# Insomnia34/charon

Hardware: AMD Instinct MI355X
Metric: verified BLS partial sigs/sec (node) + threshold aggregates/sec, 1/2/4/8 GPU (higher is better)
Workload: dtype u32

## Files before the change

charon_amd/csrc/hipbls.hip:

```cpp
#include <hip/hip_runtime.h>
#include <hsa/hsa.h>
#include <hsa/hsa_ext_amd.h>

#include <algorithm>
#include <array>
#include <atomic>
#include <chrono>
#include <condition_variable>
#include <cstdio>
#include <cstdlib>
#include <cstring>
#include <deque>
#include <map>
#include <memory>
#include <mutex>
#include <string>
#include <thread>
#include <unordered_map>
#include <vector>

#include <sys/random.h>

#include "fav_split.h"
#include "hcache_assign.h"
#include "kernels.h"
#include "ranges.h"

extern "C" {
__global__ void k_rlc_items(uint64_t i0, uint64_t i1, const uint8_t* pks, const uint8_t* sigs, const uint32_t* msg_idx,
                            uint64_t n, uint64_t n_msgs, bls::rlc_seed seed, uint32_t* rpk, uint32_t* rsig,
                            int32_t* status, const uint32_t* key_idx, uint64_t T, const int32_t* tcode,
                            const uint32_t* tab, bls::keycache kc);
__global__ void k_rlc_hash(const uint8_t* msgs, const uint64_t* offs, uint64_t n_hash, const uint32_t* mlist, uint32_t* H,
                           uint64_t hstride, const uint32_t* hslot);
__global__ void k_rlcb_items(uint64_t n, const uint8_t* pks, const uint8_t* sigs, const uint32_t* msg_idx,
                             uint64_t n_msgs, bls::rlc_seed seed, uint32_t* rpk, uint32_t* pts, uint32_t* sc,
                             int32_t* status, const uint32_t* key_idx, uint64_t T, const int32_t* tcode,
                             const uint32_t* tab, const uint32_t* g1pos, uint32_t* gpts, uint32_t* gsc,
                             bls::keycache kc);
}

extern "C" {
__global__ void k_sign_ct_hash(const uint8_t* msgs, const uint64_t* offs, uint64_t n, uint32_t* H);
__global__ void k_sign_ct_mul(const uint8_t* sks, const uint32_t* H, uint64_t n, uint8_t* out, int32_t* status);
__global__ void k_sk_to_pk_ct(const uint8_t* sks, uint64_t n, uint8_t* out, int32_t* status);
}

extern "C" {
__global__ void k_g1_comb_build(uint32_t* T);
__global__ void k_deal_ct(const uint8_t* secrets, const uint8_t* tails, uint32_t n, uint32_t total, uint32_t threshold,
                          const uint32_t* T, uint8_t* out_shares, int32_t* status, uint8_t* out_pubs,
                          int32_t* pub_status, uint8_t* sink);
__global__ void k_recover_plan(const uint64_t* offs, uint32_t n_groups, uint32_t* m_max);
__global__ void k_recover_ct(const uint8_t* shares, const int64_t* ids, const uint64_t* offs, uint32_t n_groups,
                             uint32_t n_parts, const uint32_t* m_max, const uint32_t* T, uint8_t* out_secrets,
                             int32_t* status, uint8_t* out_pubkeys, int32_t* pk_status, uint8_t* sink);
}

namespace bls_fp2p {
__global__ void k_verify_prep8(const uint8_t* pks, const uint8_t* msgs, const uint64_t* offs, const uint8_t* sigs,
                               uint64_t n, uint32_t* ws, int32_t* status, uint32_t replicas, uint32_t* race,
                               uint32_t epoch);
__global__ void k_verify_pair_lq8(const uint32_t* ws, uint64_t n, int32_t* status, uint32_t replicas, uint32_t* race,
                                  uint32_t epoch);
__global__ void k_rlcb_sfactor8(const uint32_t* W, uint32_t* Fs);
__global__ void k_rlcb_final8(const uint32_t* Ftot, const uint32_t* Fs, int32_t* flag);
__global__ void k_g1m_miller8(uint64_t nl_max, const uint32_t* meta, const uint32_t* lmsg, const uint32_t* Wv,
                              const uint32_t* H, uint64_t hstride, const uint32_t* hslot, uint32_t* F, uint64_t col0,
                              uint64_t fstride);
__global__ void k_fav_prep8(const uint8_t* pks, uint64_t nkeys, const uint8_t* sigs, const uint8_t* msgs,
                            const uint64_t* moffs, uint64_t G, uint32_t* pts, int32_t* kcode, uint32_t* ws);
__global__ void k_tv_prep8(const uint8_t* pks, const uint8_t* msgs, const uint64_t* moffs, uint64_t G,
                           const int64_t* ids, const uint64_t* goffs, uint32_t* ws, int32_t* vstatus,
                           const uint8_t* sigs, uint64_t n_parts, uint32_t* pts, int32_t* pstat, uint32_t with_keys);
__global__ void k_tagg_sum8(const uint32_t* pts, const int32_t* pstat, const int64_t* ids, const uint64_t* goffs,
                            uint64_t n_parts, uint8_t* out, int32_t* status);
__global__ void k_tv_prep8_keys(const uint32_t* key_idx, uint64_t T, const int32_t* tcode, const uint32_t* tab,
                                const uint8_t* msgs, const uint64_t* moffs, const uint32_t* mlist, uint64_t n_hash,
                                uint64_t n_msgs, uint32_t* Hc, uint64_t G, const int64_t* ids, const uint64_t* goffs,
                                uint32_t* ws, int32_t* vstatus, const uint8_t* sigs, uint64_t n_parts, uint32_t* pts,
                                int32_t* pstat);
__global__ void k_verify_prep8_keys(const uint8_t* msgs, const uint64_t* moffs, const uint32_t* mlist, uint64_t n_hash,
                                    const uint32_t* hslot, uint32_t* H, uint64_t hstride, const uint8_t* sigs,
                                    uint64_t n, uint32_t* ws);
__global__ void k_hcache_fill8(const uint8_t* msgs, const uint64_t* moffs, const uint32_t* mlist, uint64_t n_hash,
                               const uint32_t* hslot, uint32_t* H, uint64_t hstride);
}
namespace bls_hex {
__global__ void k_verify_pair_lq16(const uint32_t* ws, uint64_t n, int32_t* status, uint32_t replicas, uint32_t* race,
                                   uint32_t epoch);
__global__ void k_tv_pair_lq16(const uint32_t* pts, const int32_t* pstat, const int64_t* ids, const uint64_t* goffs,
                               uint64_t G, uint64_t n_parts, const uint32_t* ws, int32_t* astatus, int32_t* vstatus,
                               uint8_t* out);
}
namespace bls_hexw {
__global__ void k_fav_pair_lq16(const uint32_t* pts, const int32_t* kcode, uint64_t nkeys, const uint64_t* goff,
                                const uint32_t* ws, uint64_t G, int32_t* status);
__global__ void k_fav_pair_lq16_keys(const uint32_t* key_idx, uint64_t T, const int32_t* tcode, const uint32_t* tab,
                                     const uint64_t* poff, const uint32_t* parts, const int32_t* pflags,
                                     uint64_t n_slices, const uint64_t* goff, const uint32_t* hcol,
                                     const uint32_t* Hcache, uint64_t cstride, const uint32_t* Hc, uint64_t hstride,
                                     const uint32_t* ws, uint64_t G, int32_t* status);
}
namespace bls_fp2p {
constexpr uint32_t kSfactorLds = 36 * 1024;
}

namespace {

thread_local std::string g_last_error;

constexpr int kStreamsPerDevice = 4;

struct DevBuf {
  void* p = nullptr;
  size_t cap = 0;
  hipError_t ensure(size_t n) {
    if (n <= cap) return hipSuccess;
    if (p) (void)hipFree(p);
    p = nullptr;
    cap = 0;
    const size_t want = ((n < 4096 ? 4096 : n + n / 4) + 255) & ~(size_t)255;
    hipError_t e = hipMalloc(&p, want);
    if (e == hipSuccess) cap = want;
    return e;
  }
};

struct TimingSlot {
  std::vector<std::pair<hipEvent_t, hipEvent_t>> pending;
  double total_ms = 0;
  uint64_t launches = 0;
};

struct HCache : HCacheState {
  DevBuf table;
};

struct KeyCache {
  std::mutex mu;
  uint64_t slots = 0;
  uint32_t* entries = nullptr;
  uint32_t* claim = nullptr;
  unsigned long long* ctr = nullptr;
  bls::keycache dev() const {
    bls::keycache k{};
    if (slots) {
      k.entries = entries;
      k.claim = claim;
      k.ctr = ctr;
      k.mask = (uint32_t)(slots - 1);
    }
    return k;
  }
};
constexpr uint64_t kKeyCacheDefaultSlots = 65536;
constexpr uint64_t kKeyCacheMaxSlots = 1ull << 24;

struct RootCache {
  std::mutex mu;
  uint64_t slots = 0;
  uint32_t* entries = nullptr;
  uint32_t* claim = nullptr;
  unsigned long long* ctr = nullptr;
  unsigned long long* h_ins = nullptr;
  uint64_t gen_base = 0;
  uint64_t rollovers = 0;
  bool partition = true;
  bls::rootcache dev() const {
    bls::rootcache r{};
    if (slots) {
      r.entries = entries;
      r.claim = claim;
      r.ctr = ctr;
      r.mask = (uint32_t)(slots - 1);
    }
    return r;
  }
};
constexpr uint64_t kRootCacheDefaultSlots = 262144;
constexpr uint64_t kRootCacheMaxSlots = 1ull << 22;

struct VBatch {
  std::vector<uint8_t> pk, sig, msg;
  std::vector<uint64_t> off{0};
  std::vector<int32_t> status;
  int rc = HIPBLS_OK;
  bool done = false;
  uint64_t n() const { return off.size() - 1; }
};

struct QSlot {
  hipStream_t stream = nullptr;
  hipEvent_t done_ev = nullptr;
  DevBuf d_pk, d_sig, d_msg, d_off, d_st, d_ws;
  int32_t* h_st = nullptr;
  uint64_t h_cap = 0;
  std::shared_ptr<VBatch> b;
  int rc = HIPBLS_OK;
  std::chrono::steady_clock::time_point launched;
};

struct VerifyQueue {
  static constexpr int kSlots = 2;
  std::mutex mu;
  std::condition_variable cv_work, cv_done;
  std::deque<std::shared_ptr<VBatch>> open;
  std::unordered_map<uint64_t, std::pair<std::shared_ptr<VBatch>, uint32_t>> tickets;
  uint64_t next_ticket = 1;
  std::thread worker;
  bool started = false, stop = false;
  uint64_t batches = 0, items = 0, keyed = 0, overlapped = 0;
  uint64_t wakeups = 0;
  double batch_us[26] = {};
  double batch_mean = 2.0;
  hipStream_t stream = nullptr;
  QSlot slot[kSlots];
  std::deque<int> inflight;
  DevBuf d_pk, d_sig, d_msg, d_off, d_kidx, d_midx, d_slot, d_mlist, d_rlc_st;
  DevBuf d_vk_h, d_vk_ws;
  std::vector<uint32_t> kidx, midx, order, slotv, miss;
  std::vector<uint8_t> sig_sorted, umsg;
  std::vector<uint64_t> uoff;
  std::vector<int32_t> st_sorted;
};

struct Context {
  int device = -1;
  int slot = 0;
  hipStream_t stream = nullptr;
  std::mutex mu;
  DevBuf b_pk, b_msg, b_off, b_sig, b_st, b_out, b_ids, b_pts, b_pst, b_aux, b_part, b_bad;
  DevBuf r_pk, r_sig, r_h, r_win, r_midx, r_list, r_cnt, r_slot, r_mlist;
  DevBuf t_code, t_tab, b_kidx;
  DevBuf f_ws;
  DevBuf fk_h, fk_hcol, fk_mlist;
  DevBuf fk_slices, fk_poff, fk_parts, fk_pflags;
  DevBuf v_ws;
  DevBuf ct_h;
  DevBuf ct_comb, ct_sink, ct_plan, dl_pub, dl_pst;
  int comb_state = 0;
  hipEvent_t comb_ev = nullptr;
  DevBuf vk_midx, vk_slot, vk_mlist, vk_h, vk_ws;
  DevBuf pf_msg, pf_off, pf_slot, pf_mlist;
  DevBuf tv_pts[2], tv_pst[2], tv_ws[2], tv_aux[2];
  DevBuf tv_h[2];
  struct TvHostSlot {
    std::mutex mu;
    DevBuf sig, ids, off, pk, msg, moff, out, st;
    DevBuf kidx, midx, hsrc, mlist;
    uint8_t* h_out = nullptr;
    int32_t* h_st = nullptr;
    uint64_t h_groups = 0;
    hipEvent_t done = nullptr;
  } tvh[2];
  std::atomic<uint64_t> tvh_seq{0};
  hipEvent_t tv_done[2] = {}, tv_phase = nullptr;
  hipEvent_t tv_hread = nullptr;
  uint64_t tv_seq = 0;
  uint64_t t_size = 0;
  std::unordered_map<std::string, uint32_t> t_index;
  static constexpr int kSub = 2;
  hipStream_t sub[kSub] = {};
  hipEvent_t ev_fork = nullptr, ev_hash = nullptr, ev_join[kSub] = {};
  hipEvent_t ws_done = nullptr, ws_done_rlc = nullptr;
  hipEvent_t ev_join_in = nullptr, ev_join_out = nullptr;
  int stream_prio = 0;
  std::vector<uint32_t> cu_mask;
  uint64_t joined = 0;
  uint64_t r_windows = 0;
  uint64_t r_call = 0;
  DevBuf m_pts, m_sc, m_cnt, m_off, m_cur, m_list, m_B, m_P, m_Sg, m_Wp, m_W, m_F, m_F2, m_flag, m_Fs;
  DevBuf g1_ws;
  hipEvent_t rlcb_ev_sf = nullptr;
  uint64_t slots = 0;
  static constexpr int kRlcbSlots = 8;
  int32_t* rlcb_host_flag = nullptr;
  hipEvent_t rlcb_ev[kRlcbSlots] = {};
  hipEvent_t rlcb_ev_items = nullptr, rlcb_ev_msm = nullptr;
  bool rlcb_pending[kRlcbSlots] = {};
  uint64_t rlcb_seq[kRlcbSlots] = {};
  uint64_t rlcb_call[kRlcbSlots] = {};
  uint64_t rlcb_next_seq = 0, rlcb_last_seq = 0;
  int rlcb_last = -1;
  uint64_t rlcb_last_call = 0;
  int rlcb_skipped = 0;
  uint64_t rlcb_attempted = 0, rlcb_passed = 0;
  HCache hcache;
  KeyCache kcache;
  RootCache rcache;
  std::mutex tmu;
  std::map<std::string, TimingSlot> timing;
  VerifyQueue q;
};

std::vector<Context*> g_ctxs;
std::map<int, int> g_streams_per_device;
std::atomic<int> g_nctx{0};
std::mutex g_init_mu;
std::atomic<bool> g_timing{false};
std::atomic<uint64_t> g_rr{0};
std::atomic<uint64_t> g_call_seq{0};
constexpr int kMaxContexts = 64;

int set_err(const char* what, hipError_t e) {
  g_last_error = std::string(what) + ": " + hipGetErrorString(e);
  return HIPBLS_ERR_DEVICE;
}
int arg_err(const char* what) {
  g_last_error = what;
  return HIPBLS_ERR_ARG;
}

#define HIP_TRY(expr)                                \
  do {                                               \
    hipError_t _e = (expr);                          \
    if (_e != hipSuccess) return set_err(#expr, _e); \
  } while (0)

int keycache_setup(KeyCache& kc, uint64_t slots, hipStream_t s) {
  if (slots > kKeyCacheMaxSlots) return arg_err("key cache above 2^24 slots");
  uint64_t want = 0;
  if (slots) {
    want = bls::KC_MIN_SLOTS;
    while (want < slots) want <<= 1;
  }
  if (want != kc.slots) {
    if (kc.entries) (void)hipFree(kc.entries);
    if (kc.claim) (void)hipFree(kc.claim);
    kc.entries = kc.claim = nullptr;
    kc.slots = 0;
    if (want) {
      HIP_TRY(hipMalloc((void**)&kc.entries, want * bls::KC_WORDS * 4));
      HIP_TRY(hipMalloc((void**)&kc.claim, want * 4));
      kc.slots = want;
    }
  }
  if (!kc.ctr) HIP_TRY(hipMalloc((void**)&kc.ctr, 3 * sizeof(unsigned long long)));
  HIP_TRY(hipMemsetAsync(kc.ctr, 0, 3 * sizeof(unsigned long long), s));
  if (kc.slots) {
    HIP_TRY(hipMemsetAsync(kc.claim, 0, kc.slots * 4, s));
    HIP_TRY(hipMemsetAsync(kc.entries, 0, kc.slots * bls::KC_WORDS * 4, s));
  }
  HIP_TRY(hipStreamSynchronize(s));
  return HIPBLS_OK;
}
uint64_t keycache_default_slots() {
  const char* e = getenv("HIPBLS_KEYCACHE_SLOTS");
  if (!e || !e[0]) return kKeyCacheDefaultSlots;
  char* end = nullptr;
  const unsigned long long v = strtoull(e, &end, 10);
  if (end == e || *end || v > kKeyCacheMaxSlots) {
    fprintf(stderr, "hipbls: HIPBLS_KEYCACHE_SLOTS=%s ignored (expected 0 .. 2^24)\n", e);
    return kKeyCacheDefaultSlots;
  }
  return (uint64_t)v;
}

int rootcache_setup(RootCache& rc, uint64_t slots, hipStream_t s) {
  if (slots > kRootCacheMaxSlots) return arg_err("root cache above 2^22 slots");
  uint64_t want = 0;
  if (slots) {
    want = bls::KC_MIN_SLOTS;
    while (want < slots) want <<= 1;
  }
  if (want != rc.slots) {
    if (rc.entries) (void)hipFree(rc.entries);
    if (rc.claim) (void)hipFree(rc.claim);
    rc.entries = rc.claim = nullptr;
    rc.slots = 0;
    if (want) {
      HIP_TRY(hipMalloc((void**)&rc.entries, want * bls::RC_WORDS * 4));
      HIP_TRY(hipMalloc((void**)&rc.claim, want * 4));
      rc.slots = want;
    }
  }
  if (!rc.ctr) HIP_TRY(hipMalloc((void**)&rc.ctr, 3 * sizeof(unsigned long long)));
  if (!rc.h_ins) HIP_TRY(hipHostMalloc((void**)&rc.h_ins, sizeof(unsigned long long), hipHostMallocDefault));
  HIP_TRY(hipMemsetAsync(rc.ctr, 0, 3 * sizeof(unsigned long long), s));
  if (rc.slots) {
    HIP_TRY(hipMemsetAsync(rc.claim, 0, rc.slots * 4, s));
    HIP_TRY(hipMemsetAsync(rc.entries, 0, rc.slots * bls::RC_WORDS * 4, s));
  }
  HIP_TRY(hipStreamSynchronize(s));
  *rc.h_ins = 0;
  rc.gen_base = 0;
  rc.rollovers = 0;
  return HIPBLS_OK;
}
uint64_t rootcache_default_slots() {
  const char* e = getenv("HIPBLS_ROOTCACHE_SLOTS");
  if (!e || !e[0]) return kRootCacheDefaultSlots;
  char* end = nullptr;
  const unsigned long long v = strtoull(e, &end, 10);
  if (end == e || *end || v > kRootCacheMaxSlots) {
    fprintf(stderr, "hipbls: HIPBLS_ROOTCACHE_SLOTS=%s ignored (expected 0 .. 2^22)\n", e);
    return kRootCacheDefaultSlots;
  }
  return (uint64_t)v;
}

#define KC_LAUNCH_GUARD(c) std::lock_guard<std::mutex> _kcl((c).kcache.mu)

int nctx() { return g_nctx.load(std::memory_order_acquire); }
Context& ctx(int k) { return *g_ctxs[k]; }

constexpr uint32_t kCuMaskWords = 16;
constexpr uint64_t kScratchAlign = 2ull << 20;
constexpr uint32_t kLaneBytes = 64;

struct Scratch {
  uint64_t per_lane = 0;
  uint64_t per_queue = 0;
  uint64_t limit = 0;
  uint32_t slots = 0;
  uint32_t cus = 0;
  uint32_t queues = 0;
  std::string deepest;
};
std::map<int, Scratch> g_scratch;
std::atomic<bool> g_join_all{false};

template <int S>
__global__ void k_scratch_reserve(uint32_t* out, uint32_t n) {
  constexpr int W = (S - 16) / 4;
  volatile uint32_t frame[W];
  if (n) {
    frame[n % W] = n;
    out[threadIdx.x] = frame[(n * 7u) % W];
  }
}

struct KernelRef {
  const char* name;
  const void* fn;
};
#define KREF(k) {#k, reinterpret_cast<const void*>(&k)}
#define KREF8(k) {#k, reinterpret_cast<const void*>(&bls_fp2p::k)}
#define KREF16(k) {#k, reinterpret_cast<const void*>(&bls_hex::k)}
#define KREF16W(k) {#k, reinterpret_cast<const void*>(&bls_hexw::k)}
const KernelRef kKernels[] = {
    KREF(k_fav_batch), KREF(k_fp12_prod64), KREF(k_g1_decode), KREF(k_g1m_count), KREF(k_g1m_fix), KREF(k_g1m_fold),
    KREF(k_g1m_hist), KREF(k_g1m_plan), KREF(k_g1m_rank), KREF(k_g1m_run), KREF(k_g1m_scatter), KREF(k_g2_decode),
    KREF(k_g2_sum_final), KREF(k_g2_sum_partial), KREF(k_msm_fix), KREF(k_msm_hist), KREF(k_msm_run), KREF(k_msm_scan),
    KREF(k_msm_scatter), KREF(k_msm_segment), KREF(k_msm_window), KREF(k_msm_wsum), KREF(k_pubtab_load),
    KREF(k_rlc_fallback), KREF(k_rlc_fallback_lg2), KREF(k_rlc_hash), KREF(k_rlc_items),
    KREF(k_rlc_window), KREF(k_rlc_window_lg2), KREF(k_rlcb_chunks), KREF(k_rlcb_items), KREF(k_rlcb_mark),
    KREF(k_scan_apply), KREF(k_scan_part), KREF(k_scan_top), KREF(k_sign), KREF(k_signing_roots), KREF(k_sk_to_pk),
    KREF(k_tagg_scale), KREF(k_tagg_sum), KREF(k_tagg_sum_s), KREF(k_tagg_unscale),
    KREF(k_tv_check_unscale), KREF(k_tv_join), KREF(k_tv_phase_a), KREF(k_tv_prep_pk), KREF(k_tv_prep_pk2),
    KREF(k_verify_fused), KREF(k_verify_keys), KREF(k_verify_pair_lg2), KREF(k_verify_pair_lq4),
    KREF(k_verify_pair_single), KREF(k_verify_prep), KREF(k_zero_sig_status), KREF8(k_g1m_miller8),
    KREF8(k_rlcb_final8), KREF8(k_rlcb_sfactor8), KREF8(k_verify_pair_lq8), KREF8(k_verify_prep8),
    KREF16(k_verify_pair_lq16), KREF8(k_fav_prep8), KREF16W(k_fav_pair_lq16),
    KREF8(k_tv_prep8), KREF8(k_tagg_sum8), KREF16(k_tv_pair_lq16),
    KREF(k_tv_phase_a_keys), KREF(k_tv_join_keys), KREF(k_tv_gather_keys), KREF8(k_tv_prep8_keys),
    KREF(k_verify_gather_keys), KREF8(k_verify_prep8_keys), KREF8(k_hcache_fill8),
    KREF(k_fav_batch_keys), KREF16W(k_fav_pair_lq16_keys), KREF(k_fav_sum_keys),
    KREF(k_root_lookup),
    KREF(k_sign_ct_hash), KREF(k_sign_ct_mul), KREF(k_sk_to_pk_ct),
    KREF(k_g1_comb_build), KREF(k_deal_ct), KREF(k_recover_plan), KREF(k_recover_ct),
};
#define RES(s) reinterpret_cast<const void*>(&k_scratch_reserve<s>)
const void* const kReserve[] = {
    RES(8192), RES(8448), RES(8704), RES(8960), RES(9216), RES(9472), RES(9728), RES(9984), RES(10240), RES(10496),
    RES(10752), RES(11008), RES(11264), RES(11520), RES(11776), RES(12032), RES(12288), RES(12544), RES(12800),
    RES(13056), RES(13104),
};
#undef RES
#undef KREF
#undef KREF8
#undef KREF16
#undef KREF16W

std::string kernel_names() {
  std::string s;
  for (const KernelRef& k : kKernels) {
    if (!s.empty()) s += ' ';
    s += k.name;
  }
  return s;
}

uint64_t scratch_limit(int device) {
  int bus = -1, dev = -1, dom = -1;
  if (hipDeviceGetAttribute(&bus, hipDeviceAttributePciBusId, device) != hipSuccess ||
      hipDeviceGetAttribute(&dev, hipDeviceAttributePciDeviceId, device) != hipSuccess ||
      hipDeviceGetAttribute(&dom, hipDeviceAttributePciDomainId, device) != hipSuccess) {
    (void)hipGetLastError();
    return 0;
  }
  struct Find {
    uint32_t bdf, dom;
    hsa_agent_t agent;
    bool found;
  } f{(uint32_t)((bus << 8) | (dev << 3)), (uint32_t)dom, {}, false};
  if (hsa_init() != HSA_STATUS_SUCCESS) return 0;
  hsa_iterate_agents(
      [](hsa_agent_t a, void* p) -> hsa_status_t {
        Find& f = *(Find*)p;
        hsa_device_type_t t;
        uint32_t bdf = 0, dom = 0;
        if (hsa_agent_get_info(a, HSA_AGENT_INFO_DEVICE, &t) != HSA_STATUS_SUCCESS || t != HSA_DEVICE_TYPE_GPU)
          return HSA_STATUS_SUCCESS;
        if (hsa_agent_get_info(a, (hsa_agent_info_t)HSA_AMD_AGENT_INFO_BDFID, &bdf) != HSA_STATUS_SUCCESS ||
            hsa_agent_get_info(a, (hsa_agent_info_t)HSA_AMD_AGENT_INFO_DOMAIN, &dom) != HSA_STATUS_SUCCESS)
          return HSA_STATUS_SUCCESS;
        if ((bdf & ~7u) == f.bdf && dom == f.dom) {
          f.agent = a;
          f.found = true;
          return HSA_STATUS_INFO_BREAK;
        }
        return HSA_STATUS_SUCCESS;
      },
      &f);
  uint64_t lim = 0;
  if (!f.found ||
      hsa_agent_get_info(f.agent, (hsa_agent_info_t)HSA_AMD_AGENT_INFO_SCRATCH_LIMIT_MAX, &lim) != HSA_STATUS_SUCCESS)
    lim = 0;
  return lim;
}

int scratch_budget(int device, Scratch& s) {
  s = Scratch();
  for (const KernelRef& k : kKernels) {
    hipFuncAttributes fa;
    HIP_TRY(hipFuncGetAttributes(&fa, k.fn));
    if ((uint64_t)fa.localSizeBytes > s.per_lane) {
      s.per_lane = fa.localSizeBytes;
      s.deepest = k.name;
    }
  }
  int threads = 0, warp = 0, cus = 0;
  HIP_TRY(hipDeviceGetAttribute(&threads, hipDeviceAttributeMaxThreadsPerMultiProcessor, device));
  HIP_TRY(hipDeviceGetAttribute(&warp, hipDeviceAttributeWarpSize, device));
  HIP_TRY(hipDeviceGetAttribute(&cus, hipDeviceAttributeMultiprocessorCount, device));
  s.slots = warp > 0 ? (uint32_t)(threads / warp) : 32;
  s.cus = (uint32_t)cus;
  const uint64_t raw = s.per_lane * kLaneBytes * s.slots * s.cus;
  s.per_queue = (raw + kScratchAlign - 1) / kScratchAlign * kScratchAlign;
  const char* q = getenv("GPU_MAX_HW_QUEUES");
  s.queues = q && atoi(q) > 0 ? (uint32_t)atoi(q) : 4u;
  s.limit = scratch_limit(device);
  return HIPBLS_OK;
}

int scratch_reserve(const hipStream_t* ss, int n, uint64_t per_lane) {
  const void* fn = nullptr;
  for (const void* r : kReserve) {
    hipFuncAttributes fa;
    HIP_TRY(hipFuncGetAttributes(&fa, r));
    if ((uint64_t)fa.localSizeBytes >= per_lane) {
      fn = r;
      break;
    }
  }
  if (!fn) {
    g_last_error = "scratch: the deepest kernel needs " + std::to_string(per_lane) +
                   " B per lane, more than the largest reserve kernel";
    return HIPBLS_ERR_DEVICE;
  }
  void* args[2];
  uint32_t* none = nullptr;
  uint32_t zero = 0;
  args[0] = &none;
  args[1] = &zero;
  for (int k = 0; k < n; ++k) {
    HIP_TRY(hipLaunchKernel(fn, dim3(1), dim3(64), args, 0, ss[k]));
    HIP_TRY(hipStreamSynchronize(ss[k]));
  }
  return HIPBLS_OK;
}

int init_locked(const std::vector<int>& ids) {
  int ndev = 0;
  hipError_t e = hipGetDeviceCount(&ndev);
  if (e != hipSuccess || ndev == 0) return set_err("hipGetDeviceCount (no GPU)", e == hipSuccess ? hipErrorNoDevice : e);
  if (ids.empty() || ids.size() > (size_t)kMaxContexts) return arg_err("device list empty or longer than 64");
  for (int d : ids)
    if (d < 0 || d >= ndev) return arg_err("device index out of range");
  std::vector<Context*> made;
  std::map<int, std::array<hipStream_t, kStreamsPerDevice>> dev_streams;
  for (size_t k = 0; k < ids.size(); ++k) {
    Context* c = new Context();
    c->device = ids[k];
    c->slot = (int)k;
    HIP_TRY(hipSetDevice(c->device));
    auto it = dev_streams.find(c->device);
    if (it == dev_streams.end()) {
      std::array<hipStream_t, kStreamsPerDevice> ss{};
      for (auto& x : ss) HIP_TRY(hipStreamCreateWithFlags(&x, hipStreamNonBlocking));
      it = dev_streams.emplace(c->device, ss).first;
    }
    c->stream = it->second[0];
    c->sub[0] = it->second[1];
    c->sub[1] = it->second[2];
    c->q.stream = it->second[3];
    HIP_TRY(hipEventCreateWithFlags(&c->ws_done, hipEventDisableTiming));
    HIP_TRY(hipEventCreateWithFlags(&c->ws_done_rlc, hipEventDisableTiming));
    HIP_TRY(hipEventCreateWithFlags(&c->ev_join_in, hipEventDisableTiming));
    HIP_TRY(hipEventCreateWithFlags(&c->ev_join_out, hipEventDisableTiming));
    HIP_TRY(hipStreamGetPriority(c->stream, &c->stream_prio));
    c->cu_mask.assign(kCuMaskWords, 0);
    if (hipExtStreamGetCUMask(c->stream, kCuMaskWords, c->cu_mask.data()) != hipSuccess) {
      (void)hipGetLastError();
      c->cu_mask.clear();
    }
    {
      const int krc = keycache_setup(c->kcache, keycache_default_slots(), c->stream);
      if (krc) return krc;
      const char* part = getenv("HIPBLS_ROOTCACHE_PARTITION");
      c->rcache.partition = !(part && part[0] == '0');
      const int rrc = rootcache_setup(c->rcache, rootcache_default_slots(), c->stream);
      if (rrc) return rrc;
    }
    made.push_back(c);
  }
  for (auto& kv : dev_streams) {
    HIP_TRY(hipSetDevice(kv.first));
    Scratch sb;
    int rc = scratch_budget(kv.first, sb);
    if (rc) return rc;
    if (sb.limit && (uint64_t)kStreamsPerDevice * sb.per_queue > sb.limit) {
      g_last_error = "scratch: " + std::to_string(kStreamsPerDevice) + " hardware queues x " +
                     std::to_string(sb.per_queue) + " B (" + std::to_string(sb.per_lane) + " B per lane, " + sb.deepest +
                     ") exceed device " + std::to_string(kv.first) + "'s scratch limit of " + std::to_string(sb.limit) +
                     " B";
      return HIPBLS_ERR_DEVICE;
    }
    if (sb.limit && (uint64_t)sb.queues * sb.per_queue > sb.limit) g_join_all = true;
    if (!sb.limit) {
      g_join_all = true;
      g_last_error = "scratch: device " + std::to_string(kv.first) +
                     " reports no scratch limit; every *_device call runs on the library's streams";
      fprintf(stderr, "hipbls: %s\n", g_last_error.c_str());
    }
    const char* rs = getenv("HIPBLS_SCRATCH_RESERVE");
    if (!(rs && rs[0] == '0')) {
      rc = scratch_reserve(kv.second.data(), kStreamsPerDevice, sb.per_lane);
      if (rc) return rc;
    }
    g_scratch[kv.first] = sb;
  }
  const char* t = getenv("HIPBLS_TIMING");
  if (t && t[0] == '1') g_timing = true;
  for (auto& kv : dev_streams) g_streams_per_device[kv.first] = (int)kv.second.size();
  g_ctxs = made;
  g_nctx.store((int)made.size(), std::memory_order_release);
  return HIPBLS_OK;
}

int default_devices(std::vector<int>& ids) {
  int ndev = 0;
  if (hipGetDeviceCount(&ndev) != hipSuccess) ndev = 0;
  const char* env = getenv("HIPBLS_DEVICES");
  if (env && env[0]) {
    if (!strcmp(env, "all")) {
      for (int d = 0; d < ndev; ++d) ids.push_back(d);
    } else {
      const char* p = env;
      while (*p) {
        char* end = nullptr;
        const long v = strtol(p, &end, 10);
        if (end == p) return arg_err("HIPBLS_DEVICES: expected 'all' or a comma-separated device list");
        ids.push_back((int)v);
        p = *end == ',' ? end + 1 : end;
        if (*end && *end != ',') return arg_err("HIPBLS_DEVICES: expected 'all' or a comma-separated device list");
      }
    }
    return HIPBLS_OK;
  }
  int d = 0;
  HIP_TRY(hipGetDevice(&d));
  ids.push_back(d);
  return HIPBLS_OK;
}

int ensure_init() {
  if (nctx()) return HIPBLS_OK;
  std::lock_guard<std::mutex> lk(g_init_mu);
  if (nctx()) return HIPBLS_OK;
  std::vector<int> ids;
  const int rc = default_devices(ids);
  if (rc) return rc;
  return init_locked(ids);
}

int bind(Context& c) {
  HIP_TRY(hipSetDevice(c.device));
  return HIPBLS_OK;
}

#define ENTER_CTX(c)          \
  int _brc = bind(c);         \
  if (_brc) return _brc;      \
  std::lock_guard<std::mutex> _lk((c).mu)

#define ENSURE_INIT()              \
  do {                             \
    int _irc = ensure_init();      \
    if (_irc) return _irc;         \
  } while (0)

Context& ctx_of(const void* p) {
  const int n = nctx();
  if (n > 1 && p) {
    hipPointerAttribute_t a;
    if (hipPointerGetAttributes(&a, p) == hipSuccess)
      for (int k = 0; k < n; ++k)
        if (ctx(k).device == a.device) return ctx(k);
    (void)hipGetLastError();
  }
  return ctx(0);
}

bool shares_library_queues(Context& c, hipStream_t st) {
  if (g_join_all.load()) return false;
  int prio = 0;
  if (hipStreamGetPriority(st, &prio) != hipSuccess) {
    (void)hipGetLastError();
    return false;
  }
  if (prio != c.stream_prio) return false;
  if (c.cu_mask.empty()) return true;
  uint32_t m[kCuMaskWords] = {};
  if (hipExtStreamGetCUMask(st, kCuMaskWords, m) != hipSuccess) {
    (void)hipGetLastError();
    return false;
  }
  return std::equal(c.cu_mask.begin(), c.cu_mask.end(), m);
}

struct StreamJoin {
  Context& c;
  hipStream_t user = nullptr, s = nullptr;
  bool joined = false;
  StreamJoin(Context& cc, void* stream) : c(cc), user((hipStream_t)stream), s(stream ? (hipStream_t)stream : cc.stream) {}
  int begin() {
    if (!user || user == c.stream || shares_library_queues(c, user)) return HIPBLS_OK;
    HIP_TRY(hipEventRecord(c.ev_join_in, user));
    HIP_TRY(hipStreamWaitEvent(c.stream, c.ev_join_in, 0));
    s = c.stream;
    joined = true;
    c.joined += 1;
    return HIPBLS_OK;
  }
  ~StreamJoin() {
    if (joined && hipEventRecord(c.ev_join_out, c.stream) == hipSuccess) (void)hipStreamWaitEvent(user, c.ev_join_out, 0);
  }
};
#define ON_STREAM(c, stream, s)        \
  StreamJoin _sj((c), (stream));       \
  {                                    \
    const int _jrc = _sj.begin();      \
    if (_jrc) return _jrc;             \
  }                                    \
  const hipStream_t s = _sj.s

enum { WS_GEN = 0, WS_RLC = 1 };
int ws_begin(Context& c, hipStream_t s, int group = WS_GEN) {
  HIP_TRY(hipStreamWaitEvent(s, group == WS_RLC ? c.ws_done_rlc : c.ws_done, 0));
  return HIPBLS_OK;
}
int ws_end(Context& c, hipStream_t s, int group = WS_GEN) {
  HIP_TRY(hipEventRecord(group == WS_RLC ? c.ws_done_rlc : c.ws_done, s));
// ... 106 lines not shown
  return c.slots;
}
constexpr uint64_t kPairHashMaxVerify = 16384;

void drain_timing(TimingSlot& t, bool wait) {
  std::vector<std::pair<hipEvent_t, hipEvent_t>> keep;
  for (auto& pr : t.pending) {
    if (!wait && hipEventQuery(pr.second) != hipSuccess) {
      keep.push_back(pr);
      continue;
    }
    float ms = 0;
    if ((!wait || hipEventSynchronize(pr.second) == hipSuccess) &&
        hipEventElapsedTime(&ms, pr.first, pr.second) == hipSuccess) {
      t.total_ms += ms;
      t.launches += 1;
    }
    (void)hipEventDestroy(pr.first);
    (void)hipEventDestroy(pr.second);
  }
  t.pending.swap(keep);
}

template <class Launch>
int timed(Context& c, const char* name, hipStream_t s, Launch launch) {
  hipEvent_t e0 = nullptr, e1 = nullptr;
  const bool on = g_timing.load();
  if (on) {
    HIP_TRY(hipEventCreate(&e0));
    HIP_TRY(hipEventCreate(&e1));
    HIP_TRY(hipEventRecord(e0, s));
  }
  launch();
  HIP_TRY(hipGetLastError());
  if (on) {
    HIP_TRY(hipEventRecord(e1, s));
    std::lock_guard<std::mutex> lk(c.tmu);
    TimingSlot& t = c.timing[name];
    t.pending.emplace_back(e0, e1);
    if (t.pending.size() > 256) drain_timing(t, false);
  }
  return HIPBLS_OK;
}

int initial_pair_mode() {
  const char* pm = getenv("HIPBLS_PAIR_MODE");
  if (pm && pm[0] >= '0' && pm[0] <= '4' && pm[1] == 0) return pm[0] - '0';
  return HIPBLS_PAIR_AUTO;
}
std::atomic<int> g_pair_mode{initial_pair_mode()};
constexpr uint64_t kLg2MaxVerify = 32768;
constexpr uint64_t kLg2MaxWindows = 32768;

#ifndef BLS_LQ4_MAX_VERIFY
#define BLS_LQ4_MAX_VERIFY 16384
#endif
constexpr uint64_t kLq4MaxVerify = BLS_LQ4_MAX_VERIFY;

#ifndef BLS_LQ8_MAX_VERIFY
#define BLS_LQ8_MAX_VERIFY 4096
#endif
constexpr uint64_t kLq8MaxVerify = BLS_LQ8_MAX_VERIFY;

uint32_t initial_lat_replicas() {
  const char* r = getenv("HIPBLS_LAT_REPLICAS");
  const int v = r ? atoi(r) : 8;
  return v < 1 ? 1u : (v > 32 ? 32u : (uint32_t)v);
}
std::atomic<uint32_t> g_lat_replicas{initial_lat_replicas()};
std::atomic<uint32_t> g_race_epoch{0};

bool use_pairs(uint64_t units, uint64_t auto_max) {
  const int mode = g_pair_mode.load();
  if (mode == HIPBLS_PAIR_SINGLE) return false;
  if (mode == HIPBLS_PAIR_LANES || mode == HIPBLS_PAIR_QUADS || mode == HIPBLS_PAIR_OCTETS) return true;
  return units <= auto_max;
}
bool use_quads(uint64_t n) {
  const int mode = g_pair_mode.load();
  if (mode == HIPBLS_PAIR_QUADS || mode == HIPBLS_PAIR_OCTETS) return true;
  return mode == HIPBLS_PAIR_AUTO && n <= kLq4MaxVerify;
}
constexpr uint64_t kLq16MaxVerify = 4;
bool initial_lat_hex() {
  const char* e = getenv("HIPBLS_LAT_HEX");
  return !(e && e[0] == '0');
}
const bool g_lat_hex = initial_lat_hex();
bool use_hex(uint64_t n) { return g_lat_hex && g_pair_mode.load() == HIPBLS_PAIR_AUTO && n <= kLq16MaxVerify; }
bool use_octets(uint64_t n) {
  const int mode = g_pair_mode.load();
  if (mode == HIPBLS_PAIR_OCTETS) return true;
  return mode == HIPBLS_PAIR_AUTO && n <= kLq8MaxVerify;
}

int verify_ws_ensure_bytes(DevBuf& ws, uint64_t bytes, hipStream_t s) {
  void* const before = ws.p;
  HIP_TRY(ws.ensure(bytes + 128));
  if (ws.p != before) HIP_TRY(hipMemsetAsync((uint8_t*)ws.p + ws.cap - 64, 0, 64, s));
  return HIPBLS_OK;
}
int verify_ws_ensure(DevBuf& ws, uint64_t n, hipStream_t s) { return verify_ws_ensure_bytes(ws, n * 122 * 4, s); }

struct OctRace {
  unsigned g8;
  uint32_t* race;
  uint32_t reps, epoch;
};
OctRace oct_race(const DevBuf& ws, uint64_t n) {
  OctRace R;
  R.g8 = (unsigned)((8 * n + 63) / 64);
  R.race = (uint32_t*)((uint8_t*)ws.p + ws.cap - 64);
  R.reps = R.g8 == 1 && ((uintptr_t)R.race & 63) == 0 ? g_lat_replicas.load() : 1u;
  R.epoch = R.reps > 1 ? g_race_epoch.fetch_add(1) + 1u : 0u;
  if (R.reps > 1 && R.epoch == 0) R.epoch = g_race_epoch.fetch_add(1) + 1u;
  return R;
}

int launch_oct_check(Context& c, const DevBuf& ws, uint64_t n, int32_t* d_status, hipStream_t s, const OctRace& R) {
  return timed(c, use_hex(n) ? "verify_pair_lq16" : "verify_pair_lq8", s, [&] {
#if defined(BLS_LQ8_XCD_PROBE) && BLS_LQ8_XCD_PROBE
    hipLaunchKernelGGL(bls_fp2p::k_verify_pair_lq8, dim3(8 * R.g8), dim3(kBlock), 0, s, (const uint32_t*)ws.p, n,
                       d_status, 1u, R.race, 0u);
#else
    if (use_hex(n))
      hipLaunchKernelGGL(bls_hex::k_verify_pair_lq16, dim3(R.g8 * R.reps), dim3(kBlock), 0, s, (const uint32_t*)ws.p,
                         n, d_status, R.reps, R.race, R.epoch);
    else
      hipLaunchKernelGGL(bls_fp2p::k_verify_pair_lq8, dim3(R.g8 * R.reps), dim3(kBlock), 0, s, (const uint32_t*)ws.p,
                         n, d_status, R.reps, R.race, R.epoch);
#endif
  });
}

bool rootcache_due(const RootCache& R) {
  return R.slots && *(volatile unsigned long long*)R.h_ins - R.gen_base >= R.slots / 2;
}

int rootcache_roll_if_due(Context& c, bool ctx_locked) {
  RootCache& R = c.rcache;
  {
    std::lock_guard<std::mutex> g(R.mu);
    if (!rootcache_due(R)) return HIPBLS_OK;
  }
  std::unique_lock<std::mutex> cl(c.mu, std::defer_lock);
  if (!ctx_locked) cl.lock();
  std::lock_guard<std::mutex> g(R.mu);
  if (!rootcache_due(R)) return HIPBLS_OK;
  HIP_TRY(hipDeviceSynchronize());
  unsigned long long ins = 0;
  HIP_TRY(hipMemcpyAsync(&ins, R.ctr + 2, sizeof(ins), hipMemcpyDeviceToHost, c.stream));
  HIP_TRY(hipMemsetAsync(R.claim, 0, R.slots * 4, c.stream));
  HIP_TRY(hipMemsetAsync(R.entries, 0, R.slots * bls::RC_WORDS * 4, c.stream));
  HIP_TRY(hipStreamSynchronize(c.stream));
  *R.h_ins = ins;
  R.gen_base = ins;
  R.rollovers += 1;
  return HIPBLS_OK;
}

int launch_verify_fused(Context& c, const uint8_t* d_pks, const uint8_t* d_msgs, const uint64_t* d_offs,
                        const uint8_t* d_sigs, uint64_t n, int32_t* d_status, hipStream_t s, DevBuf& ws,
                        bool ctx_locked) {
  RootCache& R = c.rcache;
  int rc = rootcache_roll_if_due(c, ctx_locked);
  if (rc) return rc;
  std::lock_guard<std::mutex> rg(R.mu);
  const bls::rootcache rcd = n <= 0xffffffffull ? R.dev() : bls::rootcache{};
  uint32_t *perm = nullptr, *pslot = nullptr;
  if (rcd.entries) {
    rc = verify_ws_ensure_bytes(ws, (2 * n + 2) * 4, s);
    if (rc) return rc;
    perm = (uint32_t*)ws.p;
    pslot = perm + n;
    uint32_t* const cnt = pslot + n;
    HIP_TRY(hipMemsetAsync(cnt, 0, 2 * sizeof(uint32_t), s));
    rc = timed(c, "root_lookup", s, [&] {
      hipLaunchKernelGGL(k_root_lookup, dim3((unsigned)grid_for(n)), dim3(kBlock), 0, s, d_msgs, d_offs, n, rcd, perm,
                         pslot, cnt, R.partition ? 1 : 0);
    });
    if (rc) return rc;
  }
  rc = timed(c, "verify", s, [&] {
    KC_LAUNCH_GUARD(c);
    hipLaunchKernelGGL(k_verify_fused, dim3((unsigned)grid_for(n)), dim3(kBlock), 0, s, d_pks, d_msgs, d_offs, d_sigs,
                       n, d_status, c.kcache.dev(), rcd, (const uint32_t*)perm, (const uint32_t*)pslot);
  });
  if (rc) return rc;
  if (rcd.entries) HIP_TRY(hipMemcpyAsync(R.h_ins, rcd.ctr + 2, sizeof(unsigned long long), hipMemcpyDeviceToHost, s));
  return HIPBLS_OK;
}

int launch_verify(Context& c, const uint8_t* d_pks, const uint8_t* d_msgs, const uint64_t* d_offs,
                  const uint8_t* d_sigs, uint64_t n, int32_t* d_status, hipStream_t s, DevBuf& ws,
                  bool ctx_locked = true) {
  if (n == 0) return HIPBLS_OK;
  if (!use_pairs(n, kLg2MaxVerify))
    return launch_verify_fused(c, d_pks, d_msgs, d_offs, d_sigs, n, d_status, s, ws, ctx_locked);
  int rc = verify_ws_ensure(ws, n, s);
  if (rc) return rc;
  if (use_octets(n)) {
    const OctRace R = oct_race(ws, n);
    rc = timed(c, "verify_prep8", s, [&] {
      hipLaunchKernelGGL(bls_fp2p::k_verify_prep8, dim3(3 * R.g8 * R.reps), dim3(kBlock), 0, s, d_pks, d_msgs, d_offs,
                         d_sigs, n, (uint32_t*)ws.p, d_status, R.reps, R.race, R.epoch);
    });
    if (rc) return rc;
    return launch_oct_check(c, ws, n, d_status, s, R);
  }
  rc = timed(c, "verify_prep", s, [&] {
    const int pair_hash = n <= kPairHashMaxVerify ? 1 : 0;
    KC_LAUNCH_GUARD(c);
    hipLaunchKernelGGL(k_verify_prep, dim3((unsigned)((pair_hash ? 3 : 2) * grid_for(n))), dim3(kBlock), 0, s, d_pks,
                       d_msgs, d_offs, d_sigs, n, (uint32_t*)ws.p, d_status, pair_hash, c.kcache.dev());
  });
  if (rc) return rc;
  if (use_quads(n))
    return timed(c, "verify_pair_lq4", s, [&] {
      hipLaunchKernelGGL(k_verify_pair_lq4, dim3((unsigned)grid_for(4 * n)), dim3(kBlock), 0, s,
                         (const uint32_t*)ws.p, n, d_status);
    });
  return timed(c, "verify_pair_lg2", s, [&] {
    hipLaunchKernelGGL(k_verify_pair_lg2, dim3((unsigned)grid_for(2 * n)), dim3(kBlock), 0, s,
                       (const uint32_t*)ws.p, n, d_status);
  });
}

bool use_rlc_batch(Context& c, uint64_t n);
int launch_rlc_batch(Context& c, const uint8_t* d_pks, const uint8_t* d_sigs, const uint32_t* d_midx, uint64_t n,
                     const uint8_t* d_msgs, const uint64_t* d_offs, uint64_t n_msgs, const rlc_seed& seed,
                     int32_t* d_status, hipStream_t s, const uint32_t* d_kidx, uint32_t* d_H, uint64_t hstride,
                     const uint32_t* d_hslot, const uint32_t* d_mlist, uint64_t n_hash);

int ensure_rlc_streams(Context& c) {
  if (c.ev_fork) return HIPBLS_OK;
  HIP_TRY(hipEventCreateWithFlags(&c.ev_hash, hipEventDisableTiming));
  for (int k = 0; k < Context::kSub; ++k) HIP_TRY(hipEventCreateWithFlags(&c.ev_join[k], hipEventDisableTiming));
  HIP_TRY(hipEventCreateWithFlags(&c.ev_fork, hipEventDisableTiming));
  return HIPBLS_OK;
}

rlc_seed parse_seed(const uint8_t* seed32) {
  rlc_seed seed;
  for (int k = 0; k < 8; ++k)
    seed.w[k] = (uint32_t)seed32[4 * k] << 24 | (uint32_t)seed32[4 * k + 1] << 16 | (uint32_t)seed32[4 * k + 2] << 8 |
                (uint32_t)seed32[4 * k + 3];
  return seed;
}

constexpr uint64_t kLg2FallbackLanes = 32768;
int launch_fallback(Context& c, hipStream_t s, const uint32_t* list, const uint32_t* cnt, uint64_t cap,
                    uint64_t concurrent, const uint8_t* d_pks, const uint8_t* d_sigs, const uint32_t* d_midx,
                    const uint32_t* d_H, uint64_t hstride, const uint32_t* d_hslot, int32_t* d_status,
                    const uint32_t* d_kidx, uint64_t T, const uint32_t* tab, const uint32_t* rpk,
                    const uint32_t* rsig, uint64_t n) {
  const int mode = g_pair_mode.load();
  const uint64_t pair_upto = mode == HIPBLS_PAIR_SINGLE ? 0
                             : (mode == HIPBLS_PAIR_AUTO ? kLg2FallbackLanes / (concurrent ? concurrent : 1)
                                                         : ~(uint64_t)0);
  const uint64_t pairs = cap < pair_upto ? cap : pair_upto;
  int rc = HIPBLS_OK;
  if (pairs > 0)
    rc = timed(c, "rlc_fallback_lg2", s, [&] {
      hipLaunchKernelGGL(k_rlc_fallback_lg2, dim3((unsigned)grid_for(2 * pairs)), dim3(kBlock), 0, s, list, cnt, cap,
                         d_pks, d_sigs, d_midx, d_H, hstride, d_hslot, d_status, d_kidx, T, tab, pair_upto, rpk, rsig,
                         n);
    });
  if (rc) return rc;
  if (pair_upto < cap)
    rc = timed(c, "rlc_fallback", s, [&] {
      hipLaunchKernelGGL(k_rlc_fallback, dim3((unsigned)grid_for(cap)), dim3(kBlock), 0, s, list, cnt, cap, d_pks,
                         d_sigs, d_midx, d_H, hstride, d_hslot, d_status, d_kidx, T, tab, pair_upto, rpk, rsig, n);
    });
  return rc;
}

int launch_rlc(Context& c, const uint8_t* d_pks, const uint8_t* d_sigs, const uint32_t* d_midx, uint64_t n,
               const uint8_t* d_msgs, const uint64_t* d_offs, uint64_t n_msgs, const rlc_seed& seed,
               int32_t* d_status, hipStream_t s, uint64_t call, const uint32_t* d_kidx = nullptr,
               uint32_t* d_H = nullptr, uint64_t hstride = 0, const uint32_t* d_hslot = nullptr,
               const uint32_t* d_mlist = nullptr, uint64_t n_hash = 0) {
  const uint64_t T = c.t_size;
  const int32_t* tcode = (const int32_t*)c.t_code.p;
  const uint32_t* tab = (const uint32_t*)c.t_tab.p;
  c.r_windows = 0;
  c.r_call = call;
  if (n == 0) return HIPBLS_OK;
  if (n > 0xffffffffull) return arg_err("RLC batch larger than 2^32 items");
  int rc = ensure_rlc_streams(c);
  if (rc) return rc;
  const uint64_t n_win = (n + RLC_W - 1) / RLC_W;
  HIP_TRY(c.r_pk.ensure(n * 36 * 4));
  HIP_TRY(c.r_sig.ensure(n * 72 * 4));
  if (!d_H) {
    HIP_TRY(c.r_h.ensure((n_msgs ? n_msgs : 1) * 48 * 4));
    d_H = (uint32_t*)c.r_h.p;
    hstride = n_msgs;
    d_hslot = nullptr;
    d_mlist = nullptr;
    n_hash = n_msgs;
  }
  HIP_TRY(c.r_win.ensure(n_win * 4));
  HIP_TRY(c.r_list.ensure(n * 4));
  HIP_TRY(c.r_cnt.ensure(Context::kSub * 4));
  if (use_rlc_batch(c, n))
    return launch_rlc_batch(c, d_pks, d_sigs, d_midx, n, d_msgs, d_offs, n_msgs, seed, d_status, s, d_kidx, d_H,
                            hstride, d_hslot, d_mlist, n_hash);
  uint32_t* rpk = (uint32_t*)c.r_pk.p;
  uint32_t* rsig = (uint32_t*)c.r_sig.p;
  int32_t* win = (int32_t*)c.r_win.p;
  uint32_t* list = (uint32_t*)c.r_list.p;
  uint32_t* cnt = (uint32_t*)c.r_cnt.p;
  const uint64_t min_win = 2048;
  int nsub = (int)((n_win + min_win - 1) / min_win);
  if (nsub > Context::kSub) nsub = Context::kSub;
  if (nsub < 1) nsub = 1;
  const uint64_t win_per = (n_win + nsub - 1) / nsub;
  bool direct = false;
  {
    uint64_t full = 0, all = 0;
    for (int k = 0; k < nsub; ++k) {
      const uint64_t w0 = win_per * k, w1 = w0 + win_per < n_win ? w0 + win_per : n_win;
      if (w0 >= w1 || use_pairs(w1 - w0, kLg2MaxWindows)) continue;
      full += (w1 - w0) / kBlock;
      all += grid_for(w1 - w0);
    }
    const uint64_t S = wave_slots(c);
    direct = all > S && (full + S - 1) / S < (all + S - 1) / S;
  }

  rc = ws_begin(c, s, WS_RLC);
  if (rc) return rc;
  HIP_TRY(hipMemsetAsync(cnt, 0, Context::kSub * 4, s));
  HIP_TRY(hipEventRecord(c.ev_fork, s));
  if (n_hash) {
    rc = timed(c, "rlc_hash", s, [&] {
      hipLaunchKernelGGL(k_rlc_hash, dim3((unsigned)grid_for(n_hash)), dim3(kBlock), 0, s, d_msgs, d_offs, n_hash,
                         d_mlist, d_H, hstride, d_hslot);
    });
// ... 2545 lines not shown
}

int hipbls_kernel_timing(const char* name, double* avg_ms, uint64_t* launches) {
  if (!name || !avg_ms || !launches) return arg_err("null argument");
  ENSURE_INIT();
  double total = 0;
  uint64_t cnt = 0;
  const int n = nctx();
  for (int k = 0; k < n; ++k) {
    Context& c = ctx(k);
    int rc = bind(c);
    if (rc) return rc;
    std::lock_guard<std::mutex> lk(c.tmu);
    auto it = c.timing.find(name);
    if (it == c.timing.end()) continue;
    drain_timing(it->second, true);
    total += it->second.total_ms;
    cnt += it->second.launches;
  }
  *launches = cnt;
  *avg_ms = cnt ? total / cnt : 0.0;
  return HIPBLS_OK;
}

int hipbls_kernel_timing_reset(void) {
  ENSURE_INIT();
  const int n = nctx();
  for (int k = 0; k < n; ++k) {
    Context& c = ctx(k);
    int rc = bind(c);
    if (rc) return rc;
    std::lock_guard<std::mutex> lk(c.tmu);
    for (auto& kv : c.timing) {
      drain_timing(kv.second, true);
      kv.second.total_ms = 0;
      kv.second.launches = 0;
    }
  }
  return HIPBLS_OK;
}

int rlc_entry(const uint8_t* pks, const uint32_t* key_idx, const uint8_t* sigs, const uint32_t* msg_idx, uint64_t n,
              const uint8_t* msgs, const uint64_t* msg_offsets, uint64_t n_msgs, const uint8_t* seed32,
              int32_t* status) {
  const uint64_t call = g_call_seq.fetch_add(1) + 1;
  const std::vector<uint64_t> b = plan_ranges(n, parts_for(n, kSplitRlc), msg_idx);
  const bool whole = b.size() == 2;
  return run_ranges(b, [&](Context& c, uint64_t lo, uint64_t hi) {
    return rlc_range(c, pks, key_idx, sigs, msg_idx, lo, hi, msgs, msg_offsets, n_msgs, seed32, status, call, whole);
  });
}

int hipbls_batch_verify_rlc(const uint8_t* pks, const uint8_t* sigs, const uint32_t* msg_idx, uint64_t n,
                            const uint8_t* msgs, const uint64_t* msg_offsets, uint64_t n_msgs, const uint8_t* seed32,
                            int32_t* status) {
  if (n == 0) return HIPBLS_OK;
  if (!pks || !sigs || !msg_idx || !msg_offsets || !seed32 || !status || mul_overflows(n, 288))
    return arg_err("bad RLC arguments");
  for (uint64_t i = 0; i < n; ++i)
    if (msg_idx[i] >= n_msgs) return arg_err("message index out of range");
  if (!offsets_ok(msg_offsets, n_msgs)) return arg_err("bad message offsets");
  if (msg_offsets[n_msgs] && !msgs) return arg_err("null messages");
  ENSURE_INIT();
  return rlc_entry(pks, nullptr, sigs, msg_idx, n, msgs, msg_offsets, n_msgs, seed32, status);
}

int hipbls_batch_verify_rlc_device(const uint8_t* d_pks, const uint8_t* d_sigs, const uint32_t* d_msg_idx, uint64_t n,
                                   const uint8_t* d_msgs, const uint64_t* d_msg_offsets, uint64_t n_msgs,
                                   const uint8_t* seed32, int32_t* d_status, void* stream) {
  if (n == 0) return HIPBLS_OK;
  if (!seed32 || mul_overflows(n, 288)) return arg_err("bad RLC arguments");
  ENSURE_INIT();
  Context& c = ctx_of(d_status);
  ENTER_CTX(c);
  ON_STREAM(c, stream, s);
  return launch_rlc(c, d_pks, d_sigs, d_msg_idx, n, d_msgs, d_msg_offsets, n_msgs, parse_seed(seed32), d_status,
                    s, g_call_seq.fetch_add(1) + 1);
}

int hipbls_hcache_config(uint64_t capacity) {
  if (capacity > (1ull << 24)) return arg_err("H(m) cache capacity above 2^24");
  ENSURE_INIT();
  return run_all([&](Context& c) -> int {
    HCache& hc = c.hcache;
    HIP_TRY(hipDeviceSynchronize());
    hcache_reset(hc, capacity);
    if (capacity) HIP_TRY(hc.table.ensure(capacity * 48 * 4));
    return HIPBLS_OK;
  });
}

int hipbls_keycache_config(uint64_t slots) {
  if (slots > kKeyCacheMaxSlots) return arg_err("key cache above 2^24 slots");
  ENSURE_INIT();
  return run_all([&](Context& c) -> int {
    KC_LAUNCH_GUARD(c);
    HIP_TRY(hipDeviceSynchronize());
    return keycache_setup(c.kcache, slots, c.stream);
  });
}

int hipbls_keycache_stats(uint64_t* hits, uint64_t* misses, uint64_t* inserts) {
  if (!hits || !misses || !inserts) return arg_err("null output");
  *hits = *misses = *inserts = 0;
  ENSURE_INIT();
  const int n = nctx();
  for (int k = 0; k < n; ++k) {
    Context& c = ctx(k);
    ENTER_CTX(c);
    if (!c.kcache.ctr) continue;
    unsigned long long v[3] = {0, 0, 0};
    HIP_TRY(hipDeviceSynchronize());
    HIP_TRY(hipMemcpyAsync(v, c.kcache.ctr, sizeof(v), hipMemcpyDeviceToHost, c.stream));
    HIP_TRY(hipStreamSynchronize(c.stream));
    *hits += v[0];
    *misses += v[1];
    *inserts += v[2];
  }
  return HIPBLS_OK;
}

int hipbls_rootcache_config(uint64_t slots) {
  if (slots > kRootCacheMaxSlots) return arg_err("root cache above 2^22 slots");
  ENSURE_INIT();
  return run_all([&](Context& c) -> int {
    std::lock_guard<std::mutex> g(c.rcache.mu);
    HIP_TRY(hipDeviceSynchronize());
    return rootcache_setup(c.rcache, slots, c.stream);
  });
}

int hipbls_rootcache_stats(uint64_t* hits, uint64_t* misses, uint64_t* inserts, uint64_t* rollovers) {
  if (!hits || !misses || !inserts || !rollovers) return arg_err("null output");
  *hits = *misses = *inserts = *rollovers = 0;
  ENSURE_INIT();
  const int n = nctx();
  for (int k = 0; k < n; ++k) {
    Context& c = ctx(k);
    ENTER_CTX(c);
    std::lock_guard<std::mutex> g(c.rcache.mu);
    if (!c.rcache.ctr) continue;
    unsigned long long v[3] = {0, 0, 0};
    HIP_TRY(hipDeviceSynchronize());
    HIP_TRY(hipMemcpyAsync(v, c.rcache.ctr, sizeof(v), hipMemcpyDeviceToHost, c.stream));
    HIP_TRY(hipStreamSynchronize(c.stream));
    *hits += v[0];
    *misses += v[1];
    *inserts += v[2];
    *rollovers += c.rcache.rollovers;
  }
  return HIPBLS_OK;
}

int hipbls_hcache_stats(uint64_t* hits, uint64_t* misses, uint64_t* entries) {
  if (!hits || !misses || !entries) return arg_err("null output");
  *hits = *misses = *entries = 0;
  const int n = nctx();
  for (int k = 0; k < n; ++k) {
    Context& c = ctx(k);
    std::lock_guard<std::mutex> lk(c.mu);
    *hits += c.hcache.hits;
    *misses += c.hcache.misses;
    *entries += c.hcache.map.size();
  }
  return HIPBLS_OK;
}

int hipbls_hcache_prefetch(const uint8_t* msgs, const uint64_t* msg_offsets, uint64_t n_msgs, uint64_t* hashed,
                           uint64_t* present) {
  if (hashed) *hashed = 0;
  if (present) *present = 0;
  if (n_msgs == 0) return HIPBLS_OK;
  if (!msg_offsets || !offsets_ok(msg_offsets, n_msgs)) return arg_err("bad message offsets");
  if (msg_offsets[n_msgs] && !msgs) return arg_err("null messages");
  ENSURE_INIT();
  std::vector<uint8_t> umsg;
  std::vector<uint64_t> uoff;
  std::vector<uint32_t> mid;
  distinct_messages(msgs, msg_offsets, n_msgs, umsg, uoff, mid);
  const int nc = nctx();
  std::vector<uint64_t> h(nc, 0), p(nc, 0);
  int rc = run_all([&](Context& c) -> int {
    return hcache_prefetch_on(c, umsg.data(), uoff.data(), uoff.size() - 1, h[c.slot], p[c.slot]);
  });
  if (rc) return rc;
  for (int k = 0; k < nc; ++k) {
    if (hashed) *hashed += h[k];
    if (present) *present += p[k];
  }
  return HIPBLS_OK;
}

int hipbls_pubshare_table_load(const uint8_t* pks, uint64_t n, int32_t* status) {
  if ((n && (!pks || !status)) || mul_overflows(n, 240) || n > 0xffffffffull) return arg_err("bad table arguments");
  ENSURE_INIT();
  const int nc = nctx();
  std::vector<std::vector<int32_t>> st(nc, std::vector<int32_t>(n ? n : 1));
  int rc = run_all([&](Context& c) -> int { return table_load_host(c, pks, n, st[c.slot].data()); });
  if (rc) return rc;
  if (n) memcpy(status, st[0].data(), n * 4);
  return HIPBLS_OK;
}

int hipbls_pubshare_table_size(uint64_t* n) {
  if (!n) return arg_err("null output");
  ENSURE_INIT();
  Context& c = ctx(0);
  std::lock_guard<std::mutex> lk(c.mu);
  *n = c.t_size;
  return HIPBLS_OK;
}

int hipbls_verify_batch_keys(const uint32_t* key_idx, const uint8_t* msgs, const uint64_t* msg_offsets,
                             const uint8_t* sigs, uint64_t n, int32_t* status) {
  if (n == 0) return HIPBLS_OK;
  if (!key_idx || !msg_offsets || !sigs || !status || mul_overflows(n, 96)) return arg_err("bad arguments");
  if (!offsets_ok(msg_offsets, n)) return arg_err("bad message offsets");
  if (msg_offsets[n] && !msgs) return arg_err("null messages");
  ENSURE_INIT();
  uint64_t T = 0;
  {
    std::lock_guard<std::mutex> lk(ctx(0).mu);
    T = ctx(0).t_size;
  }
  for (uint64_t i = 0; i < n; ++i)
    if (key_idx[i] >= T) return arg_err("key index outside the pubshare table");
  return run_ranges(plan_ranges(n, parts_for(n, kSplitVerify), nullptr), [&](Context& c, uint64_t lo, uint64_t hi) {
    std::vector<uint64_t> tmp;
    return verify_keys_host(c, key_idx + lo, msgs ? msgs + msg_offsets[lo] : msgs, rebase(msg_offsets, lo, hi, tmp),
                            sigs + 96 * lo, hi - lo, status + lo);
  });
}

int hipbls_verify_batch_keys_device(const uint32_t* d_key_idx, const uint8_t* d_msgs, const uint64_t* d_msg_offsets,
                                    const uint8_t* d_sigs, uint64_t n, int32_t* d_status, void* stream) {
  if (n == 0) return HIPBLS_OK;
  ENSURE_INIT();
  Context& c = ctx_of(d_status);
  ENTER_CTX(c);
  ON_STREAM(c, stream, s);
  return timed(c, "verify_keys", s, [&] {
    hipLaunchKernelGGL(k_verify_keys, dim3((unsigned)grid_for(n)), dim3(kBlock), 0, s, d_key_idx, c.t_size,
                       (const int32_t*)c.t_code.p, (const uint32_t*)c.t_tab.p, d_msgs, d_msg_offsets, d_sigs, n,
                       d_status);
  });
}

int hipbls_batch_verify_rlc_keys(const uint32_t* key_idx, const uint8_t* sigs, const uint32_t* msg_idx, uint64_t n,
                                 const uint8_t* msgs, const uint64_t* msg_offsets, uint64_t n_msgs,
                                 const uint8_t* seed32, int32_t* status) {
  if (n == 0) return HIPBLS_OK;
  if (!key_idx || !sigs || !msg_idx || !msg_offsets || !seed32 || !status || mul_overflows(n, 288))
    return arg_err("bad RLC arguments");
  for (uint64_t i = 0; i < n; ++i)
    if (msg_idx[i] >= n_msgs) return arg_err("message index out of range");
  if (!offsets_ok(msg_offsets, n_msgs)) return arg_err("bad message offsets");
  if (msg_offsets[n_msgs] && !msgs) return arg_err("null messages");
  ENSURE_INIT();
  uint64_t T = 0;
  {
    std::lock_guard<std::mutex> lk(ctx(0).mu);
    T = ctx(0).t_size;
  }
  for (uint64_t i = 0; i < n; ++i)
    if (key_idx[i] >= T) return arg_err("key index outside the pubshare table");
  return rlc_entry(nullptr, key_idx, sigs, msg_idx, n, msgs, msg_offsets, n_msgs, seed32, status);
}

int hipbls_batch_verify_rlc_keys_device(const uint32_t* d_key_idx, const uint8_t* d_sigs, const uint32_t* d_msg_idx,
                                        uint64_t n, const uint8_t* d_msgs, const uint64_t* d_msg_offsets,
                                        uint64_t n_msgs, const uint8_t* seed32, int32_t* d_status, void* stream) {
  if (n == 0) return HIPBLS_OK;
  if (!seed32 || !d_key_idx || mul_overflows(n, 288)) return arg_err("bad RLC arguments");
  ENSURE_INIT();
  Context& c = ctx_of(d_status);
  ENTER_CTX(c);
  ON_STREAM(c, stream, s);
  return launch_rlc(c, nullptr, d_sigs, d_msg_idx, n, d_msgs, d_msg_offsets, n_msgs, parse_seed(seed32), d_status,
                    s, g_call_seq.fetch_add(1) + 1, d_key_idx);
}

int hipbls_rlc_stats(uint64_t* windows, uint64_t* windows_failed, uint64_t* items_fallback) {
  if (!windows || !windows_failed || !items_fallback) return arg_err("null output");
  ENSURE_INIT();
  *windows = *windows_failed = *items_fallback = 0;
  const int n = nctx();
  uint64_t newest = 0;
  for (int k = 0; k < n; ++k) {
    std::lock_guard<std::mutex> lk(ctx(k).mu);
    if (ctx(k).r_call > newest) newest = ctx(k).r_call;
  }
  for (int k = 0; k < n; ++k) {
    Context& c = ctx(k);
    ENTER_CTX(c);
    if (c.r_call != newest || c.r_windows == 0) continue;
    std::vector<int32_t> v(c.r_windows);
    HIP_TRY(hipDeviceSynchronize());
    HIP_TRY(hipMemcpy(v.data(), c.r_win.p, v.size() * 4, hipMemcpyDeviceToHost));
    *windows += c.r_windows;
    for (int32_t x : v)
      if (x > 0) {
        *windows_failed += 1;
        *items_fallback += (uint64_t)x;
      } else if (x < 0) {
        *items_fallback += (uint64_t)-x;
      }
// ... 6 lines not shown
```

charon_amd/csrc/kernels.h:

```cpp
#pragma once
#include <hip/hip_runtime.h>

#include "fav_keys.h"
#include "lg2.h"
#include "ops.h"
#include "rlc.h"
#include "rlcb.h"

using namespace bls;

namespace {

#ifndef BLS_VERIFY_LDS
#define BLS_VERIFY_LDS 1
#endif
constexpr int kBlock = 64;
#define BLS_LANE_F12(F)                      \
  __shared__ u32x4 s_f12_[36 * kBlock];      \
  const f12l<kBlock> F { (BLS_LDS u32x4*)&s_f12_[threadIdx.x] }

__global__ void __launch_bounds__(kBlock) k_verify_fused(const uint8_t* __restrict__ pks,
                                                         const uint8_t* __restrict__ msgs,
                                                         const uint64_t* __restrict__ offs,
                                                         const uint8_t* __restrict__ sigs, uint64_t n,
                                                         int32_t* __restrict__ status, keycache kc, rootcache rc,
                                                         const uint32_t* __restrict__ perm,
                                                         const uint32_t* __restrict__ pslot) {
  const uint64_t j = blockIdx.x * (uint64_t)blockDim.x + threadIdx.x;
  if (j >= n) return;
  const uint64_t i = perm ? perm[j] : j;
  if (i >= n) return;
  const uint64_t o0 = offs[i], o1 = offs[i + 1];
#if BLS_VERIFY_LDS
  BLS_LANE_F12(F);
  if (!perm) rc.entries = nullptr;
  status[i] = op_verify_l_kernel_rc(pks + 48 * i, msgs + o0, (uint32_t)(o1 - o0), sigs + 96 * i, F, kc, rc,
                                    perm ? pslot[j] : RC_NONE);
#else
  status[i] = op_verify(pks + 48 * i, msgs + o0, (uint32_t)(o1 - o0), sigs + 96 * i);
#endif
}

__global__ void __launch_bounds__(kBlock) k_root_lookup(const uint8_t* __restrict__ msgs,
                                                        const uint64_t* __restrict__ offs, uint64_t n, rootcache rc,
                                                        uint32_t* __restrict__ perm, uint32_t* __restrict__ pslot,
                                                        uint32_t* __restrict__ cnt, int partition) {
  const uint64_t i = blockIdx.x * (uint64_t)blockDim.x + threadIdx.x;
  if (i >= n) return;
  const uint64_t o0 = offs[i], o1 = offs[i + 1];
  const bool eligible = o1 - o0 == RC_MSG_BYTES;
  uint32_t slot = RC_NONE;
  if (eligible) {
    uint32_t tag[8];
    rc_tag_from_msg(tag, msgs + o0);
    slot = rc_find(rc, tag);
  }
  const bool hit = slot != RC_NONE;
  rc_count(rc, 0, hit);
  rc_count(rc, 1, eligible && !hit);
  uint64_t pos = i;
  if (partition) {
    const uint64_t act = __ballot(1), mh = __ballot(hit), mr = act & ~mh;
    const uint32_t lane = __builtin_amdgcn_mbcnt_hi(~0u, __builtin_amdgcn_mbcnt_lo(~0u, 0u));
    uint32_t bh = 0, br = 0;
    if (lane == (uint32_t)(__ffsll((unsigned long long)act) - 1)) {
      if (mh) bh = atomicAdd(cnt + 0, (uint32_t)__popcll(mh));
      if (mr) br = atomicAdd(cnt + 1, (uint32_t)__popcll(mr));
    }
    bh = __builtin_amdgcn_readfirstlane(bh);
    br = __builtin_amdgcn_readfirstlane(br);
    const uint64_t below = ((uint64_t)1 << lane) - 1;
    pos = hit ? (uint64_t)bh + __popcll(mh & below) : n - 1 - ((uint64_t)br + __popcll(mr & below));
  }
  if (pos >= n) return;
  perm[pos] = (uint32_t)i;
  pslot[pos] = slot;
}

__global__ void __launch_bounds__(kBlock) k_verify_prep(const uint8_t* __restrict__ pks,
                                                        const uint8_t* __restrict__ msgs,
                                                        const uint64_t* __restrict__ offs,
                                                        const uint8_t* __restrict__ sigs, uint64_t n,
                                                        uint32_t* __restrict__ ws, int32_t* __restrict__ status,
                                                        int pair_hash, keycache kc) {
  const uint64_t nb = (n + kBlock - 1) / kBlock;
  const bool hash_role = blockIdx.x >= nb;
  if (hash_role && pair_hash) {
    const uint64_t t = (blockIdx.x - nb) * (uint64_t)blockDim.x + threadIdx.x;
    const uint64_t i = t >> 1;
    if (i >= n) return;
    const uint32_t m = (t & 1) ? ~0u : 0u;
    const uint64_t o0 = offs[i], o1 = offs[i + 1];
    g2j hj;
    hash_to_g2_pair(hj, msgs + o0, (uint32_t)(o1 - o0), DST_POP, 43, m);
    if (!m) {
      g2a hm;
      jac_to_aff(hm, hj);
      soa_store<48>(ws + 24 * n, n, i, &hm.x.c0.v[0]);
    }
    return;
  }
  const uint64_t i = (blockIdx.x - (hash_role ? nb : 0)) * (uint64_t)blockDim.x + threadIdx.x;
  if (i >= n) return;
  if (hash_role) {
    const uint64_t o0 = offs[i], o1 = offs[i + 1];
    g2j hj;
    hash_to_g2(hj, msgs + o0, (uint32_t)(o1 - o0), DST_POP, 43);
    g2a hm;
    jac_to_aff(hm, hj);
    soa_store<48>(ws + 24 * n, n, i, &hm.x.c0.v[0]);
    return;
  }
  g1a pk;
  g2a sig;
  int st = RLC_PENDING;
  const int dp = g1_decode_kc_pk(pk, pks + 48 * i, kc);
  if (dp == DEC_BAD) {
    st = HIPBLS_ERR_PUBKEY;
  } else {
    const int ds = g2_decompress(sig, sigs + 96 * i, false);
    if (ds == DEC_BAD)
      st = HIPBLS_ERR_SIGNATURE;
    else if (dp == DEC_INF || ds == DEC_INF)
      st = verify_inf_status(ds, sig);
  }
  if (st == RLC_PENDING) {
    soa_store<24>(ws, n, i, &pk.x.v[0]);
    soa_store<48>(ws + 72 * n, n, i, &sig.x.c0.v[0]);
  }
  status[i] = st;
}

__global__ void __launch_bounds__(kBlock) k_verify_pair_lg2(const uint32_t* __restrict__ ws, uint64_t n,
                                                            int32_t* __restrict__ status) {
  const uint64_t t = blockIdx.x * (uint64_t)blockDim.x + threadIdx.x;
  const uint64_t i = t >> 1;
  const uint32_t m = (t & 1) ? ~0u : 0u;
  if (i >= n || status[i] != RLC_PENDING) return;
  g1a P[1];
  g2a Q[1];
  if (!m) {
    soa_load<24>(&P[0].x.v[0], ws, n, i);
    soa_load<48>(&Q[0].x.c0.v[0], ws + 24 * n, n, i);
  } else {
    P[0].x = G1_GEN_X;
    P[0].y = G1_NEG_GEN_Y;
    soa_load<48>(&Q[0].x.c0.v[0], ws + 72 * n, n, i);
  }
  fp12 f;
  g2j T;
  miller_loop_multi<1>(f, P, Q, 1, &T);
  const uint32_t in_g2 = g2_subgroup_from_miller(T, Q[0]) ? 1u : 0u;
  const uint32_t other = pair_swap(in_g2);
  const uint32_t sig_in_g2 = m ? in_g2 : other;
  const bool ok = lg2_finish(f, m);
  if (!m) status[i] = !sig_in_g2 ? HIPBLS_ERR_SIGNATURE : (ok ? HIPBLS_OK : HIPBLS_ERR_VERIFY);
}

__device__ __forceinline__ void verify_pair_lq4_lane(uint64_t t, const uint32_t* __restrict__ ws, uint64_t n,
                                                     int32_t* __restrict__ status) {
  const uint64_t i = t >> 2;
  const int q = (int)(t & 3);
  if (i >= n || status[i] != RLC_PENDING) return;
  g1a pk;
  g2a hm, sig;
  soa_load<24>(&pk.x.v[0], ws, n, i);
  soa_load<48>(&hm.x.c0.v[0], ws + 24 * n, n, i);
  soa_load<48>(&sig.x.c0.v[0], ws + 72 * n, n, i);
  const int st = lq4_verify(pk, hm, sig, q);
  if (q == 0) status[i] = st;
}
__global__ void __launch_bounds__(kBlock) k_verify_pair_lq4(const uint32_t* __restrict__ ws, uint64_t n,
                                                            int32_t* __restrict__ status) {
  verify_pair_lq4_lane(blockIdx.x * (uint64_t)blockDim.x + threadIdx.x, ws, n, status);
}

__global__ void __launch_bounds__(kBlock) k_sign(const uint8_t* __restrict__ sks, const uint8_t* __restrict__ msgs,
                                                 const uint64_t* __restrict__ offs, uint64_t n,
                                                 uint8_t* __restrict__ out, int32_t* __restrict__ status) {
  const uint64_t i = blockIdx.x * (uint64_t)blockDim.x + threadIdx.x;
  if (i >= n) return;
  const uint64_t o0 = offs[i], o1 = offs[i + 1];
  uint8_t sig[96];
  const int st = op_sign(sig, sks + 32 * i, msgs + o0, (uint32_t)(o1 - o0));
  for (int k = 0; k < 96; ++k) out[96 * i + k] = st == HIPBLS_OK ? sig[k] : (uint8_t)0;
  status[i] = st;
}

__global__ void __launch_bounds__(kBlock) k_sk_to_pk(const uint8_t* __restrict__ sks, uint64_t n,
                                                     uint8_t* __restrict__ out, int32_t* __restrict__ status) {
  const uint64_t i = blockIdx.x * (uint64_t)blockDim.x + threadIdx.x;
  if (i >= n) return;
  uint8_t pk[48];
  const int st = op_sk_to_pk(pk, sks + 32 * i);
  for (int k = 0; k < 48; ++k) out[48 * i + k] = st == HIPBLS_OK ? pk[k] : (uint8_t)0;
  status[i] = st;
}

#ifndef BLS_TAGG_WAVES
#define BLS_TAGG_WAVES 1
#endif
__device__ __forceinline__ void tagg_scale_lane(uint64_t k, const uint8_t* __restrict__ sigs,
                                                const int64_t* __restrict__ ids, const uint64_t* __restrict__ goffs,
                                                uint64_t n_groups, uint64_t n_parts, uint32_t* __restrict__ pts,
                                                int32_t* __restrict__ pstat) {
  if (k >= n_parts) return;
  uint64_t lo = 0, hi = n_groups;
  while (hi - lo > 1) {
    const uint64_t mid = (lo + hi) / 2;
    if (goffs[mid] <= k)
      lo = mid;
    else
      hi = mid;
  }
  const uint64_t g0 = goffs[lo], g1 = goffs[lo + 1];
  const int t = (int)(g1 - g0);
  const int me = (int)(k - g0);
  g2j acc;
  jac_set_inf(acc);
  int st = HIPBLS_OK;
  for (int a = 0; a < t; ++a) {
    if (ids[g0 + a] == 0) st = HIPBLS_ERR_COMBINE;
    for (int b = a + 1; b < t; ++b)
      if (ids[g0 + a] == ids[g0 + b]) st = HIPBLS_ERR_COMBINE;
  }
// ... 1101 lines not shown
```

charon_amd/csrc/ops.h:

```cpp
#pragma once
#include "../../include/hipbls.h"
#include "fr.h"
#include "h2c.h"
#include "pairing.h"
#include "pairing_lds.h"

namespace bls {

BLS_HD BLS_CALL bool pairing_check_verify(const g1a& pk, const g2a& hm, const g2a& sig) {
  g1a P[2];
  g2a Q[2];
  bool skip[2] = {false, false};
  P[0] = pk;
  Q[0] = hm;
  P[1].x = G1_GEN_X;
  P[1].y = G1_NEG_GEN_Y;
  Q[1] = sig;
  fp12 f, e;
  miller_loop_n(f, P, Q, skip, 2);
  final_exponentiation(e, f);
  return fp12_is_one(e);
}

BLS_HD BLS_CALL int pairing_check_verify_sig(const g1a& pk, const g2a& hm, const g2a& sig) {
  g1a P1;
  P1.x = G1_GEN_X;
  P1.y = G1_NEG_GEN_Y;
  fp12 f, e;
  g2j T1;
  miller_loop_2(f, pk, hm, P1, sig, &T1);
  const bool in_g2 = g2_subgroup_from_miller(T1, sig);
  final_exponentiation(e, f);
  if (!in_g2) return HIPBLS_ERR_SIGNATURE;
  return fp12_is_one(e) ? HIPBLS_OK : HIPBLS_ERR_VERIFY;
}

#ifndef BLS_VERIFY_L_CALL
#define BLS_VERIFY_L_CALL BLS_CALL
#endif
template <int S, bool INL>
BLS_HD BLS_INLINE int pairing_check_verify_sig_l_body(const g1a& pk, const g2a& hm, const g2a& sig, const f12l<S> F) {
  g1a P1;
  P1.x = G1_GEN_X;
  P1.y = G1_NEG_GEN_Y;
  fp12 f;
  bool in_g2;
  {
    g2j T1;
    if (INL)
      miller_loop_2_l_body<S, true>(f, F, pk, hm, P1, sig, &T1);
    else
      miller_loop_2_l<S, true>(f, F, pk, hm, P1, sig, &T1);
    in_g2 = g2_subgroup_from_miller(T1, sig);
  }
  final_exp_l(f, f, F);
  if (!in_g2) return HIPBLS_ERR_SIGNATURE;
  return fp12_is_one(f) ? HIPBLS_OK : HIPBLS_ERR_VERIFY;
}
template <int S>
BLS_HD BLS_VERIFY_L_CALL int pairing_check_verify_sig_l(const g1a& pk, const g2a& hm, const g2a& sig, const f12l<S> F) {
  return pairing_check_verify_sig_l_body<S, false>(pk, hm, sig, F);
}

BLS_HD BLS_INLINE int verify_inf_status(int ds, const g2a& sig) {
  if (ds == DEC_OK) {
    g2j sj;
    jac_from_aff(sj, sig);
    if (!g2_in_subgroup(sj)) return HIPBLS_ERR_SIGNATURE;
  }
  return HIPBLS_ERR_VERIFY;
}




BLS_HD BLS_CALL void lagrange_at_zero(fr& out_plain, const int64_t* ids, int n, int i) {
  fr num, den, t, xi, xj;
  fr_from_u32(num, 1);
  fr_from_u32(den, 1);
  fr_from_i64(xi, ids[i]);
  for (int j = 0; j < n; ++j) {
    if (j == i) continue;
    fr_from_i64(xj, ids[j]);
    fr_mul(num, num, xj);
    fr_sub(t, xj, xi);
    fr_mul(den, den, t);
  }
  fr_inv(den, den);
  fr_mul(t, num, den);
  fr_to_plain(out_plain, t);
}

BLS_HD BLS_INLINE uint64_t gcd_u64(uint64_t a, uint64_t b) {
  while (b) {
    const uint64_t t = a % b;
    a = b;
    b = t;
  }
  return a;
}
BLS_HD BLS_CALL bool lagrange_small(const int64_t* ids, int t, int me, int64_t& c_me, uint64_t& L) {
  if (t < 1 || t > 16) return false;
  for (int a = 0; a < t; ++a)
    if (ids[a] > (1 << 20) || ids[a] < -(1 << 20) || ids[a] == 0) return false;
  int64_t D[16];
  uint64_t l = 1;
  for (int k = 0; k < t; ++k) {
    int64_t d = 1;
    for (int j = 0; j < t; ++j) {
      if (j == k) continue;
      if (__builtin_mul_overflow(d, ids[j] - ids[k], &d)) return false;
    }
    if (d == 0 || d == INT64_MIN) return false;
    D[k] = d;
    const uint64_t ad = d < 0 ? (uint64_t)(-d) : (uint64_t)d;
    if (__builtin_mul_overflow(l, ad / gcd_u64(l, ad), &l) || l > (uint64_t)INT64_MAX) return false;
  }
  for (int k = 0; k < t; ++k) {
    int64_t n = 1;
    for (int j = 0; j < t; ++j)
      if (j != k && __builtin_mul_overflow(n, ids[j], &n)) return false;
    const uint64_t ad = D[k] < 0 ? (uint64_t)(-D[k]) : (uint64_t)D[k];
    const int64_t f = D[k] < 0 ? -(int64_t)(l / ad) : (int64_t)(l / ad);
    int64_t c;
    if (__builtin_mul_overflow(n, f, &c) || c == INT64_MIN) return false;
    if (k == me) c_me = c;
  }
  L = l;
  return true;
}

BLS_HD BLS_INLINE void g2_mul_i64(g2j& r, const g2j& p, int64_t c) {
  jac_mul_u64(r, p, c < 0 ? (uint64_t)0 - (uint64_t)c : (uint64_t)c);
  if (c < 0) {
    g2j t = r;
    jac_neg(r, t);
  }
}

BLS_HD BLS_CALL void tagg_scale_point(g2j& out, const g2j& sj, const int64_t* ids, int t, int me) {
  int64_t c;
  uint64_t L;
  if (lagrange_small(ids, t, me, c, L)) {
    g2_mul_i64(out, sj, c);
  } else {
    fr lam;
    lagrange_at_zero(lam, ids, t, me);
    g2_mul_glv4(out, sj, lam.v);
  }
}

BLS_HD BLS_CALL bool g2_subgroup_and_mul_i64(g2j& out, const g2j& sj, int64_t c) {
  const uint64_t k = c < 0 ? (uint64_t)0 - (uint64_t)c : (uint64_t)c;
  g2j pw = sj, ax, ac;
  jac_set_inf(ax);
  jac_set_inf(ac);
  for (int i = 0; i < 64; ++i) {
    if ((X_ABS >> i) & 1ull) {
      g2j t = ax;
      jac_add(ax, t, pw);
    }
    if ((k >> i) & 1ull) {
      g2j t = ac;
      jac_add_body(ac, t, pw);
    }
    if (i < 63 && ((X_ABS | k) >> (i + 1)) != 0) {
      g2j t;
      jac_dbl_body(t, pw);
      pw = t;
    }
  }
  if (c < 0) {
    g2j t = ac;
    jac_neg(ac, t);
  }
  out = ac;
  g2j q, ps;
  jac_neg(q, ax);
  g2_psi(ps, sj);
  return jac_eq(q, ps);
}

BLS_HD BLS_CALL void tagg_unscale(g2j& acc, const int64_t* ids, int t) {
  int64_t c;
  uint64_t L;
  if (!lagrange_small(ids, t, 0, c, L) || jac_is_inf(acc)) return;
  fr lf, li, plain;
  fr_from_i64(lf, (int64_t)L);
  fr_inv(li, lf);
  fr_to_plain(plain, li);
  g2j x = acc;
  g2_mul_glv4(acc, x, plain.v);
}

BLS_HD BLS_INLINE uint64_t tagg_group_L(const int64_t* ids, int t) {
  int64_t c;
  uint64_t L;
  return lagrange_small(ids, t, 0, c, L) ? L : 1;
}
BLS_HD BLS_CALL void g1_scale_affine(g1a& pk, uint64_t L) {
  if (L <= 1) return;
  g1j pj, q;
// ... 103 lines not shown
```

charon_amd/csrc/pairing.h:

```cpp
#pragma once
#include "curve.h"

namespace bls {

struct g1_pair_in {
  fp x, y;
  bool is_inf;
};




BLS_HD BLS_INLINE void miller_dbl_step_inl(g2j& T_in, fp2& g0, fp2& g1, fp2& h1, const fp& xp_in, const fp& yp_in) {
  const fp xp = xp_in;
  const fp yp = yp_in;
  g2j T = T_in;
  fp2 A, B, C, E, H, t;
  fp2_sqr(t, T.x);
  {
    fp2 J3;
    fp2_add(J3, t, t);
    fp2_add(J3, J3, t);
    fp2_mul_fp(g1, J3, xp);
  }
  fp2_mul(A, T.x, T.y);
  fp2_half(A, A);
  fp2_sqr(C, T.z);
  fp2_mul_3b2(E, C);
  fp2_add(H, T.y, T.z);
  fp2_sqr(H, H);
  fp2_sqr(B, T.y);
  fp2_sub(H, H, B);
  fp2_sub(H, H, C);
  fp2_sub(g0, E, B);
  fp2_mul_fp(h1, H, yp);
  fp2_neg(h1, h1);
  fp2_mul(T.z, B, H);
  fp2 F;
  fp2_add(F, E, E);
  fp2_add(F, F, E);
  fp2_sub(t, B, F);
  fp2_mul(T.x, A, t);
  fp2_add(t, B, F);
  fp2_half(t, t);
  fp2_sqr(t, t);
  fp2 E2;
  fp2_sqr(E2, E);
  fp2_add(C, E2, E2);
  fp2_add(C, C, E2);
  fp2_sub(T.y, t, C);
  T_in = T;
}
BLS_HD BLS_MILLER_CALL void miller_dbl_step(g2j& T_in, fp2& g0, fp2& g1, fp2& h1, const fp& xp_in, const fp& yp_in) { miller_dbl_step_inl(T_in, g0, g1, h1, xp_in, yp_in); }

BLS_HD BLS_INLINE void miller_add_step_inl(g2j& T_in, fp2& g0, fp2& g1, fp2& h1, const g2a& Q_in, const fp& xp_in,
                                         const fp& yp_in) {
  const fp xp = xp_in;
  const fp yp = yp_in;
  g2j T = T_in;
  fp2 theta, lambda, t, u;
  fp2_mul(t, Q_in.y, T.z);
  fp2_sub(theta, T.y, t);
  fp2_mul(t, Q_in.x, T.z);
  fp2_sub(lambda, T.x, t);
  fp2_mul(t, theta, Q_in.x);
  fp2_mul(u, lambda, Q_in.y);
  fp2_sub(g0, t, u);
  fp2_mul_fp(g1, theta, xp);
  fp2_neg(g1, g1);
  fp2_mul_fp(h1, lambda, yp);
  fp2 C, D, E, G;
  fp2_sqr(C, theta);
  fp2_mul(C, T.z, C);
  fp2_sqr(D, lambda);
  fp2_mul(G, T.x, D);
  fp2_mul(E, lambda, D);
  fp2_mul(T.z, T.z, E);
  fp2_mul(t, T.y, E);
  fp2_add(u, E, C);
  fp2_sub(u, u, G);
  fp2_sub(u, u, G);
  fp2_mul(T.x, lambda, u);
  fp2_sub(u, G, u);
  fp2_mul(u, theta, u);
  fp2_sub(T.y, u, t);
  T_in = T;
}
BLS_HD BLS_MILLER_CALL void miller_add_step(g2j& T_in, fp2& g0, fp2& g1, fp2& h1, const g2a& Q_in, const fp& xp_in,
                                         const fp& yp_in) { miller_add_step_inl(T_in, g0, g1, h1, Q_in, xp_in, yp_in); }

#ifndef BLS_MILLER_FUSE
#define BLS_MILLER_FUSE 0
#endif
BLS_HD BLS_CALL void miller_dbl2_line2(fp12& f_io, g2j& T0_io, g2j& T1_io, const g1a& P0_in, const g1a& P1_in,
                                       bool square) {
  fp12 f = f_io;
  g2j T0 = T0_io, T1 = T1_io;
  const g1a P0 = P0_in, P1 = P1_in;
  if (square) {
    fp12 s;
    fp12_sqr_inl(s, f);
    f = s;
  }
  fp2 a0, a1, ah, g0, g1, h1;
  miller_dbl_step_inl(T0, a0, a1, ah, P0.x, P0.y);
  miller_dbl_step_inl(T1, g0, g1, h1, P1.x, P1.y);
  fp12_mul_line2_inl(f, a0, a1, ah, g0, g1, h1);
  f_io = f;
  T0_io = T0;
  T1_io = T1;
}

BLS_HD BLS_CALL void miller_loop_2(fp12& f_out, const g1a& P0_in, const g2a& Q0, const g1a& P1_in, const g2a& Q1,
                                   g2j* T1_out = nullptr) {
  const g1a P0 = P0_in, P1 = P1_in;
  g2j T0, T1;
  T0.x = Q0.x;
  T0.y = Q0.y;
  fp2_set_one(T0.z);
  T1.x = Q1.x;
  T1.y = Q1.y;
  fp2_set_one(T1.z);
  fp12 f;
  {
    fp2 a0, a1, ah, g0, g1, h1;
    miller_dbl_step_inl(T0, a0, a1, ah, P0.x, P0.y);
    miller_dbl_step_inl(T1, g0, g1, h1, P1.x, P1.y);
    fp12_line_pair(f, a0, a1, ah, g0, g1, h1);
    miller_add_step_inl(T0, a0, a1, ah, Q0, P0.x, P0.y);
    miller_add_step_inl(T1, g0, g1, h1, Q1, P1.x, P1.y);
    fp12_mul_line2_inl(f, a0, a1, ah, g0, g1, h1);
  }
  for (int bit = 61; bit >= 0; --bit) {
    fp12_sqr_inl(f, f);
    fp2 a0, a1, ah, g0, g1, h1;
    miller_dbl_step_inl(T0, a0, a1, ah, P0.x, P0.y);
    miller_dbl_step_inl(T1, g0, g1, h1, P1.x, P1.y);
    fp12_mul_line2_inl(f, a0, a1, ah, g0, g1, h1);
    if ((X_ABS >> bit) & 1ull) {
      miller_add_step_inl(T0, a0, a1, ah, Q0, P0.x, P0.y);
      miller_add_step_inl(T1, g0, g1, h1, Q1, P1.x, P1.y);
      fp12_mul_line2_inl(f, a0, a1, ah, g0, g1, h1);
    }
  }
  fp12_conj(f_out, f);
  if (T1_out) *T1_out = T1;
}

BLS_HD BLS_INLINE bool g2_subgroup_from_miller(const g2j& T, const g2a& Q) {
  g2j q, ps;
  jac_from_aff(q, Q);
  g2_psi(ps, q);
  fp2 t;
  bool ok = !fp2_is_zero(T.z);
  fp2_mul(t, ps.x, T.z);
  ok = ok && fp2_eq(t, T.x);
  fp2_mul(t, ps.y, T.z);
  fp2_add(t, t, T.y);
  return ok && fp2_is_zero(t);
}

BLS_HD BLS_CALL void miller_loop_n(fp12& f, const g1a* P, const g2a* Q, const bool* skip, int n) {
  static_assert((X_ABS >> 62) & 1ull, "miller_loop_2 folds the top bit below |x|'s leading one into its first step");
  if (n == 2 && !skip[0] && !skip[1]) {
    miller_loop_2(f, P[0], Q[0], P[1], Q[1]);
    return;
  }
  constexpr int MAXN = 2;
  g2j T[MAXN];
  for (int i = 0; i < n; ++i) {
    T[i].x = Q[i].x;
    T[i].y = Q[i].y;
    fp2_set_one(T[i].z);
  }
  fp12_set_one(f);
  fp2 g0, g1, h1;
  bool first = true;
  for (int bit = 62; bit >= 0; --bit) {
    if (n == 2 && !skip[0] && !skip[1]) {
      fp2 a0, a1, ah;
#if BLS_MILLER_FUSE == 1
      miller_dbl2_line2(f, T[0], T[1], P[0], P[1], !first);
#elif BLS_MILLER_FUSE == 2
      if (!first) fp12_sqr(f, f);
      miller_dbl2_line2(f, T[0], T[1], P[0], P[1], false);
#else
      if (!first) fp12_sqr(f, f);
      miller_dbl_step(T[0], a0, a1, ah, P[0].x, P[0].y);
      miller_dbl_step(T[1], g0, g1, h1, P[1].x, P[1].y);
      fp12_mul_line2(f, a0, a1, ah, g0, g1, h1);
#endif
      first = false;
      if ((X_ABS >> bit) & 1ull) {
        miller_add_step(T[0], a0, a1, ah, Q[0], P[0].x, P[0].y);
        miller_add_step(T[1], g0, g1, h1, Q[1], P[1].x, P[1].y);
        fp12_mul_line2(f, a0, a1, ah, g0, g1, h1);
      }
      continue;
    }
    if (!first) fp12_sqr(f, f);
    first = false;
    for (int i = 0; i < n; ++i) {
      miller_dbl_step(T[i], g0, g1, h1, P[i].x, P[i].y);
      if (!skip[i]) fp12_mul_line(f, g0, g1, h1);
    }
    if ((X_ABS >> bit) & 1ull) {
      for (int i = 0; i < n; ++i) {
        miller_add_step(T[i], g0, g1, h1, Q[i], P[i].x, P[i].y);
        if (!skip[i]) fp12_mul_line(f, g0, g1, h1);
      }
    }
  }
  fp12_conj(f, f);
}

#ifndef BLS_EXP_MUL
#define BLS_EXP_MUL fp12_mul
#endif

struct cyc_c {
// ... 223 lines not shown
```

charon_amd/csrc/pairing_lds.h:

```cpp
#pragma once
#include "pairing.h"

namespace bls {

#if defined(__HIP_DEVICE_COMPILE__)
#define BLS_LDS __attribute__((address_space(3)))
#else
#define BLS_LDS
#endif

typedef uint32_t u32x4 __attribute__((vector_size(16)));

#if defined(__HIPCC__)
#define BLS_MEMBER __forceinline__
#else
#define BLS_MEMBER inline
#endif

template <int S>
struct f12l {
  BLS_LDS u32x4* p;

  BLS_HD BLS_MEMBER void ld_fp(fp& r, int g) const {
    for (int j = 0; j < 3; ++j) {
      const u32x4 q = p[(g + j) * S];
      r.v[4 * j] = q[0];
      r.v[4 * j + 1] = q[1];
      r.v[4 * j + 2] = q[2];
      r.v[4 * j + 3] = q[3];
    }
  }
  BLS_HD BLS_MEMBER void st_fp(int g, const fp& a) const {
    for (int j = 0; j < 3; ++j) {
      const u32x4 q = {a.v[4 * j], a.v[4 * j + 1], a.v[4 * j + 2], a.v[4 * j + 3]};
      p[(g + j) * S] = q;
    }
  }
  BLS_HD BLS_MEMBER fp2 ld(int k) const {
    fp2 r;
    ld_fp(r.c0, 6 * k);
    ld_fp(r.c1, 6 * k + 3);
    return r;
  }
  BLS_HD BLS_MEMBER void st(int k, const fp2& a) const {
    st_fp(6 * k, a.c0);
    st_fp(6 * k + 3, a.c1);
  }
  BLS_HD BLS_MEMBER void ld12(fp12& r) const {
    r.c0.c0 = ld(0);
    r.c0.c1 = ld(1);
    r.c0.c2 = ld(2);
    r.c1.c0 = ld(3);
    r.c1.c1 = ld(4);
    r.c1.c2 = ld(5);
  }
  BLS_HD BLS_MEMBER void st12(const fp12& a) const {
    st(0, a.c0.c0);
    st(1, a.c0.c1);
    st(2, a.c0.c2);
    st(3, a.c1.c0);
    st(4, a.c1.c1);
    st(5, a.c1.c2);
  }
};

#if BLS_LAZY_FP6
template <class A, class B>
BLS_HD BLS_INLINE void fp6_mul_fetch(fp6& r, const A& a, const B& b) {
  fp2 xa1, xa2, c0, c1, c2;
  fp2_mul_xi(xa1, a(1));
  fp2_mul_xi(xa2, a(2));
  fp2_mul3(c0, a(0), b(0), xa1, b(2), xa2, b(1));
  fp2_mul3(c1, a(0), b(1), a(1), b(0), xa2, b(2));
  fp2_mul3(c2, a(0), b(2), a(1), b(1), a(2), b(0));
  r.c0 = c0;
  r.c1 = c1;
  r.c2 = c2;
}
#else
template <class A, class B>
BLS_HD BLS_INLINE void fp6_mul_fetch(fp6& r, const A& a, const B& b) {
  fp2 t0, t1, t2, s0, s1, u0, u1, u2;
  fp2_mul(t0, a(0), b(0));
  fp2_mul(t1, a(1), b(1));
  fp2_mul(t2, a(2), b(2));
  fp2_add_lazy(s0, a(1), a(2));
  fp2_add_lazy(s1, b(1), b(2));
  fp2_mul(u0, s0, s1);
  fp2_sub(u0, u0, t1);
  fp2_sub(u0, u0, t2);
  fp2_mul_xi(u0, u0);
  fp2_add(u0, u0, t0);
  fp2_add_lazy(s0, a(0), a(1));
  fp2_add_lazy(s1, b(0), b(1));
  fp2_mul(u1, s0, s1);
  fp2_sub(u1, u1, t0);
  fp2_sub(u1, u1, t1);
  fp2 x2;
  fp2_mul_xi(x2, t2);
  fp2_add(u1, u1, x2);
  fp2_add_lazy(s0, a(0), a(2));
  fp2_add_lazy(s1, b(0), b(2));
  fp2_mul(u2, s0, s1);
  fp2_sub(u2, u2, t0);
  fp2_sub(u2, u2, t2);
  fp2_add(u2, u2, t1);
  r.c0 = u0;
  r.c1 = u1;
  r.c2 = u2;
}
#endif

template <int S>
BLS_HD BLS_INLINE void fp12_sqr_l(const f12l<S>& F) {
  fp6 t;
  fp6_mul_fetch(t, [&](int i) { return F.ld(i); }, [&](int i) { return F.ld(3 + i); });
  {
    const fp2 b0 = F.ld(3), b1 = F.ld(4), b2 = F.ld(5);
    fp2 vb0, s, u;
    fp2_mul_xi(vb0, b2);
    fp2 a = F.ld(0);
    fp2_add(s, a, b0);
    fp2_add(u, a, vb0);
    F.st(0, s);
    F.st(3, u);
    a = F.ld(1);
    fp2_add(s, a, b1);
    fp2_add(u, a, b0);
    F.st(1, s);
    F.st(4, u);
    a = F.ld(2);
    fp2_add(s, a, b2);
    fp2_add(u, a, b1);
    F.st(2, s);
    F.st(5, u);
  }
  fp6 s;
  fp6_mul_fetch(s, [&](int i) { return F.ld(i); }, [&](int i) { return F.ld(3 + i); });
  fp6 vt;
  fp6_mul_v(vt, t);
  fp2 c;
  fp2_sub(c, s.c0, t.c0);
  fp2_sub(c, c, vt.c0);
  F.st(0, c);
  fp2_sub(c, s.c1, t.c1);
  fp2_sub(c, c, vt.c1);
  F.st(1, c);
  fp2_sub(c, s.c2, t.c2);
  fp2_sub(c, c, vt.c2);
  F.st(2, c);
  fp2_add(c, t.c0, t.c0);
  F.st(3, c);
  fp2_add(c, t.c1, t.c1);
  F.st(4, c);
  fp2_add(c, t.c2, t.c2);
  F.st(5, c);
}

template <int S>
BLS_HD BLS_INLINE void fp12_mul_line2_l(const f12l<S>& F, const fp2& ga0_in, const fp2& ga1_in, const fp2& ha1_in,
                                        const fp2& gb0_in, const fp2& gb1_in, const fp2& hb1_in) {
  const fp2 ga0 = ga0_in;
  const fp2 ga1 = ga1_in;
  const fp2 ha1 = ha1_in;
  const fp2 gb0 = gb0_in;
  const fp2 gb1 = gb1_in;
  const fp2 hb1 = hb1_in;
  fp2 p00, p11, phh, sa, sb, t;
  fp6 L0;
  fp2 x, y;
// ... 21 lines not shown
  fp6 t0, t1;
  fp6_mul_fetch(t0, [&](int i) { return F.ld(i); }, [&](int i) { return i == 0 ? L0.c0 : (i == 1 ? L0.c1 : L0.c2); });
#if BLS_LAZY_FP6
  {
    fp2 u, xa2;
    fp2_mul2(u, F.ld(4), y, F.ld(5), x);
    fp2_mul_xi(t1.c0, u);
    fp2_mul_xi(xa2, F.ld(5));
    fp2_mul2(t1.c1, F.ld(3), x, xa2, y);
    fp2_mul2(t1.c2, F.ld(3), y, F.ld(4), x);
  }
#else
  {
    fp2 m1, m2, m0, u, w2;
    fp2_mul(m1, F.ld(4), x);
    fp2_mul(m2, F.ld(5), y);
    fp2_mul(m0, F.ld(3), x);
    fp2_add_lazy(u, F.ld(4), F.ld(5));
    fp2_add_lazy(w2, x, y);
    fp2_mul(u, u, w2);
    fp2_sub(u, u, m1);
    fp2_sub(u, u, m2);
    fp2_mul_xi(t1.c0, u);
    fp2_mul_xi(u, m2);
    fp2_add(t1.c1, m0, u);
    fp2_mul(u, F.ld(3), y);
    fp2_add(t1.c2, u, m1);
  }
#endif
  fp2 c;
  for (int i = 0; i < 3; ++i) {
    fp2_add(c, F.ld(i), F.ld(3 + i));
    F.st(3 + i, c);
  }
  fp6 d;
  {
    fp6 vt1;
    fp6_mul_v(vt1, t1);
    fp2_add(c, t0.c0, vt1.c0);
    F.st(0, c);
    fp2_add(c, t0.c1, vt1.c1);
    F.st(1, c);
    fp2_add(c, t0.c2, vt1.c2);
    F.st(2, c);
    fp6_add(d, t0, t1);
  }
  fp6 l, s;
  l.c0 = L0.c0;
  fp2_add(l.c1, L0.c1, x);
  fp2_add(l.c2, L0.c2, y);
  fp6_mul_fetch(s, [&](int i) { return F.ld(3 + i); }, [&](int i) { return i == 0 ? l.c0 : (i == 1 ? l.c1 : l.c2); });
  fp2_sub(c, s.c0, d.c0);
  F.st(3, c);
  fp2_sub(c, s.c1, d.c1);
  F.st(4, c);
  fp2_sub(c, s.c2, d.c2);
  F.st(5, c);
}

template <class A>
BLS_HD BLS_INLINE void fp6_mul_01_fetch(fp6& r, const A& a, const fp2& b0, const fp2& b1) {
#if BLS_LAZY_FP6
  fp2 xa2, c0, c1, c2;
  fp2_mul_xi(xa2, a(2));
  fp2_mul2(c0, a(0), b0, xa2, b1);
  fp2_mul2(c1, a(0), b1, a(1), b0);
  fp2_mul2(c2, a(2), b0, a(1), b1);
  r.c0 = c0;
  r.c1 = c1;
  r.c2 = c2;
#else
  fp2 t0, t1, s0, s1, u, c0, c1, c2;
  fp2_mul(t0, a(0), b0);
  fp2_mul(t1, a(1), b1);
  fp2_mul(u, a(2), b1);
  fp2_mul_xi(u, u);
  fp2_add(c0, u, t0);
  fp2_add_lazy(s0, a(0), a(1));
  fp2_add(s1, b0, b1);
  fp2_mul(c1, s0, s1);
  fp2_sub(c1, c1, t0);
  fp2_sub(c1, c1, t1);
  fp2_mul(c2, a(2), b0);
  fp2_add(c2, c2, t1);
  r.c0 = c0;
  r.c1 = c1;
  r.c2 = c2;
#endif
}
template <class A>
BLS_HD BLS_INLINE void fp6_mul_1_fetch(fp6& r, const A& a, const fp2& b1) {
  fp2 c0;
  fp2_mul(c0, a(2), b1);
  fp2_mul_xi(r.c0, c0);
  fp2_mul(r.c1, a(0), b1);
  fp2_mul(r.c2, a(1), b1);
}

template <int S>
BLS_HD BLS_INLINE void fp12_mul_line_l(const f12l<S>& F, const fp2& g0_in, const fp2& g1_in, const fp2& h1_in) {
  const fp2 g0 = g0_in;
  const fp2 g1 = g1_in;
  const fp2 h1 = h1_in;
  fp6 t0, t1;
  fp6_mul_01_fetch(t0, [&](int i) { return F.ld(i); }, g0, g1);
  fp6_mul_1_fetch(t1, [&](int i) { return F.ld(3 + i); }, h1);
  fp2 c;
  for (int i = 0; i < 3; ++i) {
    fp2_add(c, F.ld(i), F.ld(3 + i));
    F.st(3 + i, c);
  }
  fp6 d;
  {
    fp6 vt1;
    fp6_mul_v(vt1, t1);
    fp2_add(c, t0.c0, vt1.c0);
    F.st(0, c);
    fp2_add(c, t0.c1, vt1.c1);
    F.st(1, c);
    fp2_add(c, t0.c2, vt1.c2);
    F.st(2, c);
    fp6_add(d, t0, t1);
  }
  fp2 gh1;
  fp2_add(gh1, g1, h1);
  fp6 s;
  fp6_mul_01_fetch(s, [&](int i) { return F.ld(3 + i); }, g0, gh1);
  fp2_sub(c, s.c0, d.c0);
  F.st(3, c);
  fp2_sub(c, s.c1, d.c1);
  F.st(4, c);
  fp2_sub(c, s.c2, d.c2);
  F.st(5, c);
}

#ifndef BLS_ML_PARK
#define BLS_ML_PARK 6
#endif
template <class T>
BLS_HD BLS_INLINE void park_agpr(T& x) {
#if defined(__HIP_DEVICE_COMPILE__)
  uint32_t* w = reinterpret_cast<uint32_t*>(&x);
#pragma unroll
  for (int i = 0; i < (int)(sizeof(T) / 4); ++i) asm("" : "+a"(w[i]));
#endif
}

#ifndef BLS_ML_DBL
#define BLS_ML_DBL miller_dbl_step_inl
#endif
#ifndef BLS_MILLER_L_CALL
#define BLS_MILLER_L_CALL BLS_CALL
#endif
template <int S, bool P1_NEG_GEN = false>
BLS_HD BLS_INLINE void miller_loop_2_l_body(fp12& f_out, const f12l<S> F, const g1a& P0_in, const g2a& Q0,
                                          const g1a& P1_in, const g2a& Q1, g2j* T1_out) {
  g1a P0 = P0_in;
  g1a P1;
  if (P1_NEG_GEN) {
    P1.x = G1_GEN_X;
    P1.y = G1_NEG_GEN_Y;
  } else {
    P1 = P1_in;
  }
  g2j T0, T1;
  T0.x = Q0.x;
  T0.y = Q0.y;
  fp2_set_one(T0.z);
  T1.x = Q1.x;
  T1.y = Q1.y;
  fp2_set_one(T1.z);
  {
    fp12 f;
    fp2 a0, a1, ah, g0, g1, h1;
    miller_dbl_step_inl(T0, a0, a1, ah, P0.x, P0.y);
    miller_dbl_step_inl(T1, g0, g1, h1, P1.x, P1.y);
    fp12_line_pair(f, a0, a1, ah, g0, g1, h1);
    F.st12(f);
    miller_add_step_inl(T0, a0, a1, ah, Q0, P0.x, P0.y);
    miller_add_step_inl(T1, g0, g1, h1, Q1, P1.x, P1.y);
    fp12_mul_line2_l(F, a0, a1, ah, g0, g1, h1);
  }
  for (int bit = 61; bit >= 0; --bit) {
#if BLS_ML_PARK & 1
    park_agpr(T0);
    park_agpr(T1);
#endif
#if BLS_ML_PARK & 4
    park_agpr(P0);
#endif
    fp12_sqr_l(F);
    fp2 a0, a1, ah, g0, g1, h1;
    BLS_ML_DBL(T0, a0, a1, ah, P0.x, P0.y);
#if BLS_ML_PARK & 2
    park_agpr(T0);
    park_agpr(a0);
    park_agpr(a1);
    park_agpr(ah);
#endif
    BLS_ML_DBL(T1, g0, g1, h1, P1.x, P1.y);
    fp12_mul_line2_l(F, a0, a1, ah, g0, g1, h1);
    if ((X_ABS >> bit) & 1ull) {
      miller_add_step_inl(T0, a0, a1, ah, Q0, P0.x, P0.y);
      miller_add_step_inl(T1, g0, g1, h1, Q1, P1.x, P1.y);
      fp12_mul_line2_l(F, a0, a1, ah, g0, g1, h1);
    }
  }
  fp12 f;
  F.ld12(f);
  fp12_conj(f_out, f);
  if (T1_out) *T1_out = T1;
}
template <int S, bool P1_NEG_GEN = false>
BLS_HD BLS_MILLER_L_CALL void miller_loop_2_l(fp12& f_out, const f12l<S> F, const g1a& P0_in, const g2a& Q0, const g1a& P1_in,
                                     const g2a& Q1, g2j* T1_out) {
  miller_loop_2_l_body<S, P1_NEG_GEN>(f_out, F, P0_in, Q0, P1_in, Q1, T1_out);
}

template <int S>
BLS_HD BLS_INLINE void fp12_mul_l(const f12l<S>& F, const fp12& b) {
  fp6 t0, t1;
  fp6_mul_fetch(t0, [&](int i) { return F.ld(i); }, [&](int i) { return i == 0 ? b.c0.c0 : (i == 1 ? b.c0.c1 : b.c0.c2); });
  fp6_mul_fetch(t1, [&](int i) { return F.ld(3 + i); }, [&](int i) { return i == 0 ? b.c1.c0 : (i == 1 ? b.c1.c1 : b.c1.c2); });
  fp2 c;
  for (int i = 0; i < 3; ++i) {
    fp2_add(c, F.ld(i), F.ld(3 + i));
    F.st(3 + i, c);
  }
  fp6 d, sb;
  {
    fp6 vt1;
    fp6_mul_v(vt1, t1);
    fp2_add(c, t0.c0, vt1.c0);
    F.st(0, c);
    fp2_add(c, t0.c1, vt1.c1);
    F.st(1, c);
    fp2_add(c, t0.c2, vt1.c2);
    F.st(2, c);
    fp6_add(d, t0, t1);
  }
  fp6_add(sb, b.c0, b.c1);
  fp6 s;
  fp6_mul_fetch(s, [&](int i) { return F.ld(3 + i); }, [&](int i) { return i == 0 ? sb.c0 : (i == 1 ? sb.c1 : sb.c2); });
  fp2_sub(c, s.c0, d.c0);
  F.st(3, c);
  fp2_sub(c, s.c1, d.c1);
  F.st(4, c);
  fp2_sub(c, s.c2, d.c2);
  F.st(5, c);
}

template <int S>
BLS_HD BLS_CALL bool fp12_cyc_exp_xabs_karabina_l(fp12& r, const fp12& a_in, const f12l<S> F) {
  static_assert(X_ABS == 0xd201000000010000ull, "the squaring counts below are |x|'s set bits");
  cyc_c st[6];
  cyc_c c;
  c.z2 = a_in.c1.c0;
  c.z3 = a_in.c0.c2;
  c.z4 = a_in.c0.c1;
  c.z5 = a_in.c1.c2;
  cyc_sqr_run(c, 16);
  st[0] = c;
  cyc_sqr_run(c, 32);
  st[1] = c;
  cyc_sqr_run(c, 9);
  st[2] = c;
  cyc_sqr_run(c, 3);
  st[3] = c;
  cyc_sqr_run(c, 2);
  st[4] = c;
  cyc_sqr_run(c, 1);
  st[5] = c;
  fp2 num[6], den[6], pre[6];
  int s;
#pragma unroll 1
  for (s = 0; s < 6; ++s) cyc_z1_parts(num[s], den[s], st[s]);
  pre[0] = den[0];
#pragma unroll 1
  for (s = 1; s < 6; ++s) fp2_mul(pre[s], pre[s - 1], den[s]);
  if (fp2_is_zero(pre[5])) return true;
  fp2 inv;
  fp2_inv(inv, pre[5]);
#pragma unroll 1
  for (s = 5; s >= 0; --s) {
    fp2 is, z1;
    if (s > 0) {
      fp2_mul(is, inv, pre[s - 1]);
      fp2_mul(inv, inv, den[s]);
    } else {
      is = inv;
    }
    fp2_mul(z1, num[s], is);
    fp12 d;
    cyc_decompress(d, st[s], z1);
    if (s == 5)
      F.st12(d);
    else
      fp12_mul_l(F, d);
  }
  F.ld12(r);
  return false;
}
template <int S>
BLS_HD BLS_INLINE void fp12_cyc_exp_xabs_l(fp12& r, const fp12& a_in, const f12l<S>& F) {
  if (fp12_cyc_exp_xabs_karabina_l(r, a_in, F)) fp12_cyc_exp_xabs_gs(r, a_in);
}

template <int S>
BLS_HD BLS_CALL void final_exponentiation_l(fp12& r, const fp12& f_in, const f12l<S> F) {
  fp12 m;
  {
    fp12 t, fi;
    fp12_conj(t, f_in);
    fp12_inv(fi, f_in);
    BLS_FE_MUL(m, t, fi);
    fp12_frobenius(t, m, 2);
    BLS_FE_MUL(m, t, m);
  }
  fp12 t1;
  {
    fp12 t0, u;
    fp12_cyc_exp_xabs_l(t0, m, F);
    BLS_FE_MUL(t0, t0, m);
    fp12_conj(t0, t0);
    fp12_cyc_exp_xabs_l(u, t0, F);
    BLS_FE_MUL(u, u, t0);
    fp12_conj(t0, u);
    fp12_cyc_exp_xabs_l(u, t0, F);
    fp12_conj(u, u);
    fp12_frobenius(t1, t0, 1);
    BLS_FE_MUL(t1, t1, u);
  }
  fp12 t2;
  {
    fp12 u;
    fp12_cyc_exp_xabs_l(u, t1, F);
    fp12_cyc_exp_xabs_l(u, u, F);
    fp12_frobenius(t2, t1, 2);
    BLS_FE_MUL(t2, t2, u);
    fp12_conj(u, t1);
    BLS_FE_MUL(t2, t2, u);
  }
  {
    fp12 u;
    fp12_cyclotomic_sqr(u, m);
    BLS_FE_MUL(u, u, m);
    BLS_FE_MUL(r, t2, u);
  }
}
#ifndef BLS_FE_LDS
#define BLS_FE_LDS 1
#endif
template <int S>
BLS_HD BLS_INLINE void final_exp_l(fp12& r, const fp12& f, const f12l<S>& F) {
#if BLS_FE_LDS
  final_exponentiation_l(r, f, F);
#else
  final_exponentiation(r, f);
#endif
}

template <int S>
BLS_HD BLS_CALL bool pairing_check_verify_l(const g1a& pk, const g2a& hm, const g2a& sig, const f12l<S> F) {
  g1a P1;
// ... 10 lines not shown
```

charon_amd/csrc/rlc.h:

```cpp
#pragma once
#include "keycache.h"
#include "rootcache.h"
#include "ops.h"

namespace bls {

#ifndef RLC_W
#define RLC_W 8
#endif
constexpr int RLC_PENDING = -1;

struct rlc_seed {
  uint32_t w[8];
};

BLS_HD BLS_INLINE void rlc_scalars(uint32_t& a, uint32_t& b, const rlc_seed& seed, uint64_t i) {
  uint32_t w[16];
  for (int k = 0; k < 8; ++k) w[k] = seed.w[k];
  w[8] = (uint32_t)(i >> 32);
  w[9] = (uint32_t)i;
  w[10] = 0x80000000u;
  for (int k = 11; k < 15; ++k) w[k] = 0;
  w[15] = 40 * 8;
  sha256_state s;
// ... 69 lines not shown
    jac_from_aff(pj, P);
    jac_add_aff(pq, pj, Q);
    jac_to_aff(PQ, pq);
  }
  jac<F> acc;
  jac_set_inf(acc);
  for (int bit = 31; bit >= 0; --bit) {
    jac<F> t;
    jac_dbl_body(t, acc);
    acc = t;
    const uint32_t d = ((a >> bit) & 1u) | (((b >> bit) & 1u) << 1);
    const aff<F> addend = d == 1 ? P : (d == 2 ? Q : PQ);
    if (d) {
      jac<F> x = acc, y;
      jac_add_aff_body(y, x, addend);
      acc = y;
    }
  }
  r = acc;
}

BLS_HD BLS_CALL int g1_decompress_keep_x(g1a& out, g1j& xP, const uint8_t* b) {
  const int st = g1_decompress(out, b, false);
  if (st != DEC_OK) return st;
  g1j p, q, q2, phi;
  jac_from_aff(p, out);
  jac_mul_u64(q, p, X_ABS);
  jac_mul_u64(q2, q, X_ABS);
  fp_mul(phi.x, p.x, FP_BETA);
  fp_neg(phi.y, p.y);
  phi.z = p.z;
  if (!jac_eq(q2, phi)) return DEC_BAD;
  jac_neg(xP, q);
  return DEC_OK;
}

template <bool WANT_X>
BLS_HD BLS_INLINE int g1_decode_kc_body(g1a& out, g1j& xP, const uint8_t* b, const keycache& kc) {
  uint32_t tag[12];
  kc_tag_from_wire(tag, b);
  int st;
  bool ins = false;
  const bool hit = kc_lookup(kc, tag, out.y.v, WANT_X ? &xP.x.v[0] : nullptr);
  if (hit) {
    uint8_t buf[48];
    for (int i = 0; i < 48; ++i) buf[i] = b[i];
    buf[0] &= 0x1f;
    fp_plain_from_be48(out.x, buf);
    fp_to_mont(out.x, out.x);
    st = DEC_OK;
  } else {
    st = g1_decompress_keep_x(out, xP, b);
    if (st == DEC_OK) ins = kc_insert(kc, tag, out.y.v, &xP.x.v[0]);
  }
  kc_count(kc, hit, ins);
  return st;
}
BLS_HD BLS_CALL int g1_decode_kc_x(g1a& out, g1j& xP, const uint8_t* b, const keycache& kc) {
  if (!kc.entries) return g1_decompress_keep_x(out, xP, b);
  return g1_decode_kc_body<true>(out, xP, b, kc);
}
BLS_HD BLS_CALL int g1_decode_kc_pk(g1a& out, const uint8_t* b, const keycache& kc) {
  if (!kc.entries) return g1_decompress(out, b, true);
  g1j xP;
  return g1_decode_kc_body<false>(out, xP, b, kc);
}

BLS_HD BLS_CALL int rlc_item_decoded(int dp, const g1a& pk, const g1j& xpk, const uint8_t* sig96, const rlc_seed& seed,
                                     uint64_t i, uint32_t* rpk36, uint32_t* rsig72) {
  g1j rp;
  g2j rs;
  jac_set_inf(rp);
  jac_set_inf(rs);
  int st = RLC_PENDING;
  if (dp == DEC_BAD) st = HIPBLS_ERR_PUBKEY;
  g2a sig;
  if (st == RLC_PENDING) {
    const int ds = g2_decompress(sig, sig96, true);
    if (ds == DEC_BAD)
      st = HIPBLS_ERR_SIGNATURE;
    else if (dp == DEC_INF || ds == DEC_INF)
      st = HIPBLS_ERR_VERIFY;
  }
  if (st == RLC_PENDING) {
    uint32_t a, b;
    rlc_scalars(a, b, seed, i);
    g1j pj;
    jac_from_aff(pj, pk);
    jac_mul2_u32(rp, pj, xpk, a, b);
    g2j sj, psj;
    jac_from_aff(sj, sig);
    g2_psi(psj, sj);
    g2a psa;
    psa.x = psj.x;
    psa.y = psj.y;
    jac_mul2_u32_aff(rs, sig, psa, a, b);
  }
  const uint32_t* p = &rp.x.v[0];
  for (int k = 0; k < 36; ++k) rpk36[k] = p[k];
  const uint32_t* s = &rs.x.c0.v[0];
  for (int k = 0; k < 72; ++k) rsig72[k] = s[k];
  return st;
}

BLS_HD BLS_CALL int rlc_item(const uint8_t* pk48, const uint8_t* sig96, const rlc_seed& seed, uint64_t i,
                             uint32_t* rpk36, uint32_t* rsig72) {
  g1a pk;
  g1j xpk;
  const int dp = g1_decompress_keep_x(pk, xpk, pk48);
  return rlc_item_decoded(dp, pk, xpk, sig96, seed, i, rpk36, rsig72);
}
BLS_HD BLS_CALL int rlc_item_kc(const uint8_t* pk48, const uint8_t* sig96, const rlc_seed& seed, uint64_t i,
                                uint32_t* rpk36, uint32_t* rsig72, const keycache& kc) {
  g1a pk;
  g1j xpk;
  const int dp = g1_decode_kc_x(pk, xpk, pk48, kc);
  return rlc_item_decoded(dp, pk, xpk, sig96, seed, i, rpk36, rsig72);
}

constexpr int PUBTAB_WORDS = 24 + 36;

BLS_HD BLS_INLINE int pubtab_load_lane(uint64_t k, const uint8_t* pks, uint64_t T, int32_t* code, uint32_t* tab) {
  g1a pk;
  g1j xpk;
  const int dp = g1_decompress_keep_x(pk, xpk, pks + 48 * k);
  if (dp != DEC_OK) {
    fp_set_zero(pk.x);
    fp_set_zero(pk.y);
    jac_set_inf(xpk);
  }
  soa_store<24>(tab, T, k, &pk.x.v[0]);
  soa_store<36>(tab + 24 * T, T, k, &xpk.x.v[0]);
  code[k] = dp;
  return dp == DEC_BAD ? HIPBLS_ERR_PUBKEY : HIPBLS_OK;
}

BLS_HD BLS_INLINE int pubtab_get(g1a& pk, g1j& xpk, uint64_t k, uint64_t T, const int32_t* code, const uint32_t* tab) {
  soa_load<24>(&pk.x.v[0], tab, T, k);
  soa_load<36>(&xpk.x.v[0], tab + 24 * T, T, k);
  return code[k];
}

BLS_HD BLS_INLINE int tv_key_lane(g1a& lpk, uint64_t k, uint64_t T, const int32_t* code, const uint32_t* tab,
                                  const int64_t* ids, int t) {
  if (k >= T) return HIPBLS_ERR_ARG;
  g1j xpk;
  const int dp = pubtab_get(lpk, xpk, k, T, code, tab);
  if (dp == DEC_BAD) return HIPBLS_ERR_PUBKEY;
  if (dp == DEC_INF) return HIPBLS_ERR_VERIFY;
  g1_scale_affine(lpk, tagg_group_L(ids, t));
  return RLC_PENDING;
}

BLS_HD BLS_CALL void verify_hm_rc(g2a& hm, const uint8_t* msg, uint32_t msg_len, const rootcache& rc, uint32_t slot) {
  const bool eligible = rc.entries && msg_len == RC_MSG_BYTES;
  uint32_t tag[8];
  if (eligible) rc_tag_from_msg(tag, msg);
  bool ins = false;
  if (!(eligible && slot != RC_NONE && rc_get_slot(rc, slot, tag, &hm.x.c0.v[0]))) {
    g2j hj;
    hash_to_g2(hj, msg, msg_len, DST_POP, 43);
    const bool inf = jac_is_inf(hj);
    jac_to_aff(hm, hj);
    if (eligible && !inf) ins = rc_insert(rc, tag, &hm.x.c0.v[0]);
  }
  if (rc.entries) rc_count(rc, 2, ins);
}

template <int S>
BLS_HD BLS_INLINE int op_verify_l_kernel_rc(const uint8_t* pk48, const uint8_t* msg, uint32_t msg_len,
                                            const uint8_t* sig96, const f12l<S> F, const keycache& kc,
                                            const rootcache& rc, uint32_t slot) {
  g1a pk;
  const int dp = g1_decode_kc_pk(pk, pk48, kc);
  if (dp == DEC_BAD) return HIPBLS_ERR_PUBKEY;
  g2a sig;
  const int ds = g2_decompress(sig, sig96, false);
  if (ds == DEC_BAD) return HIPBLS_ERR_SIGNATURE;
  if (dp == DEC_INF || ds == DEC_INF) return verify_inf_status(ds, sig);
  g2a hm;
  verify_hm_rc(hm, msg, msg_len, rc, slot);
  return pairing_check_verify_sig_l_body<S, true>(pk, hm, sig, F);
}

template <int S>
BLS_HD BLS_CALL int op_verify_decoded_pk(int dp, const g1a& pk, const uint8_t* msg, uint32_t msg_len,
                                         const uint8_t* sig96, const f12l<S> F) {
  if (dp == DEC_BAD) return HIPBLS_ERR_PUBKEY;
  g2a sig;
  const int ds = g2_decompress(sig, sig96, false);
  if (ds == DEC_BAD) return HIPBLS_ERR_SIGNATURE;
  if (dp == DEC_INF || ds == DEC_INF) return verify_inf_status(ds, sig);
  g2j hj;
  hash_to_g2(hj, msg, msg_len, DST_POP, 43);
  g2a hm;
  jac_to_aff(hm, hj);
  return pairing_check_verify_sig_l(pk, hm, sig, F);
}

template <int MAXN>
BLS_HD BLS_CALL void miller_loop_multi(fp12& f, const g1a* P, const g2a* Q, int n, g2j* T0_out = nullptr) {
  g2j T[MAXN];
  for (int k = 0; k < n; ++k) {
    T[k].x = Q[k].x;
    T[k].y = Q[k].y;
    fp2_set_one(T[k].z);
  }
  fp12_set_one(f);
  fp2 g0, g1, h1;
  for (int bit = 62; bit >= 0; --bit) {
    if (bit != 62) fp12_sqr(f, f);
    for (int k = 0; k < n; k += 2) {
      if (k + 1 < n) {
        fp2 a0, a1, ah;
        miller_dbl_step(T[k], a0, a1, ah, P[k].x, P[k].y);
        miller_dbl_step(T[k + 1], g0, g1, h1, P[k + 1].x, P[k + 1].y);
        fp12_mul_line2(f, a0, a1, ah, g0, g1, h1);
      } else {
        miller_dbl_step(T[k], g0, g1, h1, P[k].x, P[k].y);
        fp12_mul_line(f, g0, g1, h1);
      }
    }
    if ((X_ABS >> bit) & 1ull) {
      for (int k = 0; k < n; k += 2) {
        if (k + 1 < n) {
          fp2 a0, a1, ah;
          miller_add_step(T[k], a0, a1, ah, Q[k], P[k].x, P[k].y);
          miller_add_step(T[k + 1], g0, g1, h1, Q[k + 1], P[k + 1].x, P[k + 1].y);
          fp12_mul_line2(f, a0, a1, ah, g0, g1, h1);
        } else {
          miller_add_step(T[k], g0, g1, h1, Q[k], P[k].x, P[k].y);
          fp12_mul_line(f, g0, g1, h1);
        }
      }
    }
  }
  fp12_conj(f, f);
  if (T0_out) *T0_out = T[0];
}

template <int MAXN, int S>
BLS_HD BLS_CALL void miller_loop_multi_l(fp12& f_out, const f12l<S> F, const g1a* P, const g2a* Q, int n) {
  g2j T[MAXN];
  for (int k = 0; k < n; ++k) {
    T[k].x = Q[k].x;
    T[k].y = Q[k].y;
    fp2_set_one(T[k].z);
  }
  {
    fp12 one;
    fp12_set_one(one);
    F.st12(one);
  }
  fp2 g0, g1, h1;
  for (int bit = 62; bit >= 0; --bit) {
    if (bit != 62) fp12_sqr_l(F);
    for (int k = 0; k < n; k += 2) {
      if (k + 1 < n) {
        fp2 a0, a1, ah;
        miller_dbl_step(T[k], a0, a1, ah, P[k].x, P[k].y);
        miller_dbl_step(T[k + 1], g0, g1, h1, P[k + 1].x, P[k + 1].y);
        fp12_mul_line2_l(F, a0, a1, ah, g0, g1, h1);
      } else {
        miller_dbl_step(T[k], g0, g1, h1, P[k].x, P[k].y);
        fp12_mul_line_l(F, g0, g1, h1);
      }
    }
    if ((X_ABS >> bit) & 1ull) {
      for (int k = 0; k < n; k += 2) {
        if (k + 1 < n) {
          fp2 a0, a1, ah;
          miller_add_step(T[k], a0, a1, ah, Q[k], P[k].x, P[k].y);
          miller_add_step(T[k + 1], g0, g1, h1, Q[k + 1], P[k + 1].x, P[k + 1].y);
          fp12_mul_line2_l(F, a0, a1, ah, g0, g1, h1);
        } else {
          miller_add_step(T[k], g0, g1, h1, Q[k], P[k].x, P[k].y);
          fp12_mul_line_l(F, g0, g1, h1);
        }
      }
    }
  }
  fp12 f;
  F.ld12(f);
  fp12_conj(f_out, f);
}

template <int LS, class LoadPk, class LoadSig, class LoadH>
BLS_HD BLS_INLINE bool rlc_window(const f12l<LS>& F, uint64_t i0, uint64_t i1, const int32_t* status, const uint32_t* msg_idx,
                                  LoadPk load_pk, LoadSig load_sig, LoadH load_h) {
  g1a P[RLC_W + 1];
  g2a Q[RLC_W + 1];
  int np = 0;
  g2j S;
  jac_set_inf(S);
  g1j run;
  uint32_t run_msg = 0xffffffffu;
  bool any = false;
  for (uint64_t i = i0; i < i1; ++i) {
    if (status[i] != RLC_PENDING) continue;
    any = true;
    g1j qp;
    g2j qs;
    load_pk(qp, i);
    load_sig(qs, i);
    jac_add(S, S, qs);
    const uint32_t m = msg_idx[i];
    if (m != run_msg) {
      if (run_msg != 0xffffffffu && !jac_is_inf(run)) {
        jac_to_aff(P[np], run);
        load_h(Q[np], run_msg);
        ++np;
      }
      run = qp;
      run_msg = m;
    } else {
      jac_add(run, run, qp);
    }
  }
  if (!any) return true;
  if (!jac_is_inf(run)) {
    jac_to_aff(P[np], run);
    load_h(Q[np], run_msg);
    ++np;
  }
  if (!jac_is_inf(S)) {
    P[np].x = G1_GEN_X;
    P[np].y = G1_NEG_GEN_Y;
    jac_to_aff(Q[np], S);
    ++np;
  }
  if (np == 0) return true;
  fp12 f;
  miller_loop_multi_l<RLC_W + 1>(f, F, P, Q, np);
  final_exp_l(f, f, F);
  return fp12_is_one(f);
// ... 100 lines not shown
```

charon_amd/csrc/rootcache.h:

```cpp
#pragma once
#include "keycache.h"

namespace bls {

constexpr int RC_WORDS = 64;
constexpr int RC_TAG = 0, RC_H = 8, RC_CHK = 56, RC_USED = 60;
constexpr uint32_t RC_MSG_BYTES = 32;
constexpr uint32_t RC_NONE = 0xffffffffu;

struct rootcache {
  uint32_t* entries;
  uint32_t* claim;
  unsigned long long* ctr;
  uint32_t mask;
  uint32_t pad_;
};

KC_HD void rc_tag_from_msg(uint32_t tag[8], const uint8_t* m32) {
  for (int k = 0; k < 8; ++k)
    tag[k] = (uint32_t)m32[4 * k] | ((uint32_t)m32[4 * k + 1] << 8) | ((uint32_t)m32[4 * k + 2] << 16) |
             ((uint32_t)m32[4 * k + 3] << 24);
}
KC_HD uint64_t rc_tag_hash(const uint32_t tag[8]) { return kc_fold(0x452821E638D01377ull, tag, 8); }
KC_HD uint64_t rc_check(uint64_t tag_hash, const uint32_t h[48]) {
  return kc_check_final(kc_fold(tag_hash ^ 0xBE5466CF34E90C6Cull, h, 48));
}

KC_HD void rc_pack(uint32_t e[RC_WORDS], const uint32_t tag[8], const uint32_t h[48]) {
  for (int k = 0; k < 8; ++k) e[RC_TAG + k] = tag[k];
  for (int k = 0; k < 48; ++k) e[RC_H + k] = h[k];
  const uint64_t c = rc_check(rc_tag_hash(tag), h);
  e[RC_CHK] = (uint32_t)c;
  e[RC_CHK + 1] = (uint32_t)(c >> 32);
  for (int k = RC_CHK + 2; k < RC_WORDS; ++k) e[k] = 0;
}

KC_HD bool rc_entry_get(const uint32_t* e, const uint32_t tag[8], uint32_t* h ) {
  uint32_t diff = 0;
  for (int k = 0; k < 8; ++k) diff |= e[RC_TAG + k] ^ tag[k];
  if (diff) return false;
  const uint64_t c = rc_check(rc_tag_hash(tag), e + RC_H);
  if (e[RC_CHK] != (uint32_t)c || e[RC_CHK + 1] != (uint32_t)(c >> 32)) return false;
  if (h)
    for (int k = 0; k < 48; ++k) h[k] = e[RC_H + k];
  return true;
}

constexpr int RC_PROBES = 4;
constexpr int RC_SEQ = RC_PROBES * KC_WINDOW;
KC_HD uint32_t rc_seq_slot(uint64_t tag_hash, int j, uint32_t mask) {
  const int p = j / KC_WINDOW;
  const uint32_t home = p ? (uint32_t)(kc_mix(tag_hash, (uint32_t)p) >> 20) : kc_home(tag_hash, mask);
  return (home + (uint32_t)(j % KC_WINDOW)) & mask;
}

KC_HD uint32_t rc_find(const rootcache& rc, const uint32_t tag[8]) {
  const uint64_t th = rc_tag_hash(tag);
  const uint32_t fpr = kc_fingerprint(th);
  for (int j = 0; j < RC_SEQ; ++j) {
    const uint32_t s = rc_seq_slot(th, j, rc.mask);
    const uint32_t c = kc_load_claim(rc.claim + s);
    if (!c) return RC_NONE;
    if (c != fpr) continue;
    uint32_t e[RC_WORDS];
    kc_load_words(e, rc.entries + (uint64_t)s * RC_WORDS, 0, RC_USED);
    if (rc_entry_get(e, tag, nullptr)) return s;
  }
  return RC_NONE;
}

KC_HD bool rc_get_slot(const rootcache& rc, uint32_t slot, const uint32_t tag[8], uint32_t h[48]) {
  uint32_t e[RC_WORDS];
  kc_load_words(e, rc.entries + (uint64_t)(slot & rc.mask) * RC_WORDS, 0, RC_USED);
  return rc_entry_get(e, tag, h);
}

KC_HD bool rc_insert(const rootcache& rc, const uint32_t tag[8], const uint32_t h[48]) {
  const uint64_t th = rc_tag_hash(tag);
  const uint32_t fpr = kc_fingerprint(th);
  for (int j = 0; j < RC_SEQ; ++j) {
    const uint32_t s = rc_seq_slot(th, j, rc.mask);
    uint32_t c = kc_load_claim(rc.claim + s);
    if (!c) c = kc_cas_claim(rc.claim + s, fpr);
    if (c == fpr) return false;
    if (c) continue;
    uint32_t e[RC_WORDS];
    rc_pack(e, tag, h);
    kc_store_entry(rc.entries + (uint64_t)s * RC_WORDS, e);
    return true;
  }
  return false;
}

#if defined(__HIP_DEVICE_COMPILE__)
KC_HD void rc_count(const rootcache& rc, int which, bool flag) {
  const uint64_t act = __ballot(1), m = __ballot(flag);
  if (!m) return;
  const uint32_t lane = __builtin_amdgcn_mbcnt_hi(~0u, __builtin_amdgcn_mbcnt_lo(~0u, 0u));
  if (lane != (uint32_t)(__ffsll((unsigned long long)act) - 1)) return;
  __hip_atomic_fetch_add((kc_gu64*)rc.ctr + which, (unsigned long long)__popcll(m), __ATOMIC_RELAXED,
                         __HIP_MEMORY_SCOPE_AGENT);
}
#else
KC_HD void rc_count(const rootcache& rc, int which, bool flag) {
  if (flag) rc.ctr[which] += 1;
}
#endif

}
```

charon_amd/tbls.py:

```python

from __future__ import annotations

import ctypes
import os
import secrets
from typing import Dict, List, Mapping, Optional, Sequence, Tuple

R = 0x73EDA753299D7D483339D80809A1D80553BDA402FFFE5BFEFFFFFFFF00000001

OK, ERR_PUBKEY, ERR_SIGNATURE, ERR_VERIFY, ERR_SECRET, ERR_COMBINE, ERR_ZERO_SIG = 0, 1, 2, 3, 4, 5, 6
INFINITY_G2 = b"\xc0" + bytes(95)
ERR_ARG, ERR_DEVICE = 16, 17
PAIR_AUTO, PAIR_SINGLE, PAIR_LANES, PAIR_QUADS, PAIR_OCTETS = 0, 1, 2, 3, 4
RLC_AUTO, RLC_WINDOWS, RLC_BATCH = 0, 1, 2

VERIFY_ERRORS = {
    ERR_PUBKEY: "cannot set compressed public key in Herumi format",
    ERR_SIGNATURE: "cannot unmarshal signature into Herumi signature",
    ERR_VERIFY: "signature not verified",
}


class TBLSError(Exception):
    """A tbls error: message is the string tbls.Herumi returns for the same input."""


class DeviceError(RuntimeError):
    """HIP runtime failure.  Never converted into a 'verified' result."""


_LIB_PATH = os.environ.get("HIPBLS_LIB") or os.path.join(os.path.dirname(os.path.abspath(__file__)), "libhipbls.so")
_lib = None


def load_library(path: str = _LIB_PATH) -> ctypes.CDLL:
    global _lib
    if _lib is not None:
        return _lib
    if not os.path.exists(path):
        raise RuntimeError("hipbls native library not built: %s (run __graft_entry__.build())" % path)
    lib = ctypes.CDLL(path)
    u8p = ctypes.c_char_p
    u64 = ctypes.c_uint64
    i32p = ctypes.POINTER(ctypes.c_int32)
    u64p = ctypes.POINTER(ctypes.c_uint64)
    u32p = ctypes.POINTER(ctypes.c_uint32)
    i64p = ctypes.POINTER(ctypes.c_int64)
    vp = ctypes.c_void_p
    sig = {
        "hipbls_current_device": ([], ctypes.c_int),
        "hipbls_init_devices": ([ctypes.POINTER(ctypes.c_int32), ctypes.c_uint32], ctypes.c_int),
        "hipbls_device_slots": ([ctypes.POINTER(ctypes.c_int32), ctypes.c_uint32], ctypes.c_int),
        "hipbls_plan_ranges": ([u64, ctypes.c_uint32, u32p, u64p], ctypes.c_int),
        "hipbls_queue_keyed_batches": ([u64p], ctypes.c_int),
        "hipbls_deserialize_status": ([u8p, u64, ctypes.c_int32, i32p], ctypes.c_int),
        "hipbls_set_timing": ([ctypes.c_int], ctypes.c_int),
        "hipbls_set_pair_mode": ([ctypes.c_int], ctypes.c_int),
        "hipbls_rlc_set_mode": ([ctypes.c_int], ctypes.c_int),
        "hipbls_rlc_set_g1_msm_min": ([ctypes.c_uint32], ctypes.c_int),
        "hipbls_threshold_aggregate_verify_batch": ([u8p, i64p, u64p, u64, u8p, u8p, u64p, u8p, i32p, i32p],
                                                    ctypes.c_int),
        "hipbls_threshold_aggregate_verify_batch_device": ([vp, vp, vp, u64, u64, vp, vp, vp, vp, vp, vp, vp],
                                                           ctypes.c_int),
        "hipbls_threshold_aggregate_verify_batch_keys": ([u8p, i64p, u64p, u64, u32p, u32p, u8p, u64p, u64, u8p, i32p,
                                                          i32p], ctypes.c_int),
        "hipbls_threshold_aggregate_verify_batch_keys_device": ([vp, vp, vp, u64, u64, vp, vp, vp, vp, u64, vp, vp,
                                                                 vp, vp], ctypes.c_int),
        "hipbls_rlc_batch_stats": ([u64p, u64p, i32p], ctypes.c_int),
        "hipbls_verify": ([u8p, u8p, u64, u8p, i32p], ctypes.c_int),
        "hipbls_verify_submit": ([u8p, u8p, u64, u8p, u64p], ctypes.c_int),
        "hipbls_verify_wait": ([u64, i32p], ctypes.c_int),
        "hipbls_queue_config": ([u64, ctypes.c_uint32], ctypes.c_int),
        "hipbls_queue_stats": ([u64p, u64p], ctypes.c_int),
        "hipbls_verify_signed_data_batch": ([u8p, u8p, u8p, u8p, u64, i32p], ctypes.c_int),
        "hipbls_aggregate_device": ([vp, u64, vp, vp, vp], ctypes.c_int),
        "hipbls_hcache_config": ([u64], ctypes.c_int),
        "hipbls_hcache_stats": ([u64p, u64p, u64p], ctypes.c_int),
        "hipbls_hcache_prefetch": ([u8p, u64p, u64, u64p, u64p], ctypes.c_int),
        "hipbls_keycache_config": ([u64], ctypes.c_int),
        "hipbls_keycache_stats": ([u64p, u64p, u64p], ctypes.c_int),
        "hipbls_rootcache_config": ([u64], ctypes.c_int),
        "hipbls_rootcache_stats": ([u64p, u64p, u64p, u64p], ctypes.c_int),
        "hipbls_abi_version": ([], ctypes.c_int),
        "hipbls_init": ([ctypes.c_int], ctypes.c_int),
        "hipbls_device_count": ([], ctypes.c_int),
        "hipbls_device_streams": ([ctypes.c_int], ctypes.c_int),
        "hipbls_last_error": ([], ctypes.c_char_p),
        "hipbls_verify_batch": ([u8p, u8p, u64p, u8p, u64, i32p], ctypes.c_int),
        "hipbls_threshold_aggregate_batch": ([u8p, i64p, u64p, u64, u8p, i32p], ctypes.c_int),
        "hipbls_sign_batch": ([u8p, u8p, u64p, u64, u8p, i32p], ctypes.c_int),
        "hipbls_secret_to_public_key_batch": ([u8p, u64, u8p, i32p], ctypes.c_int),
        "hipbls_verify_aggregate": ([u8p, u64, u8p, u8p, u64, i32p], ctypes.c_int),
        "hipbls_aggregate": ([u8p, u64, u8p, i32p], ctypes.c_int),
        "hipbls_threshold_split": ([u8p, u8p, ctypes.c_uint32, ctypes.c_uint32, u8p, i32p], ctypes.c_int),
        "hipbls_recover_secret": ([u8p, i64p, ctypes.c_uint32, u8p, i32p], ctypes.c_int),
        "hipbls_verify_batch_device": ([vp, vp, vp, vp, u64, vp, vp], ctypes.c_int),
        "hipbls_threshold_aggregate_batch_device": ([vp, vp, vp, u64, u64, vp, vp, vp], ctypes.c_int),
        "hipbls_sign_batch_device": ([vp, vp, vp, u64, vp, vp, vp], ctypes.c_int),
        "hipbls_secret_to_public_key_batch_device": ([vp, u64, vp, vp, vp], ctypes.c_int),
        "hipbls_sign_batch_ct": ([u8p, u8p, u64p, u64, u8p, i32p], ctypes.c_int),
        "hipbls_secret_to_public_key_batch_ct": ([u8p, u64, u8p, i32p], ctypes.c_int),
        "hipbls_sign_batch_ct_device": ([vp, vp, vp, u64, vp, vp, vp], ctypes.c_int),
        "hipbls_secret_to_public_key_batch_ct_device": ([vp, u64, vp, vp, vp], ctypes.c_int),
        "hipbls_threshold_split_batch_ct": ([u8p, u8p, u64, ctypes.c_uint32, ctypes.c_uint32, u8p, i32p, u8p, i32p],
                                            ctypes.c_int),
        "hipbls_recover_secret_batch_ct": ([u8p, i64p, u64p, u64, u8p, i32p, u8p, i32p], ctypes.c_int),
        "hipbls_threshold_split_batch_ct_device": ([vp, vp, u64, ctypes.c_uint32, ctypes.c_uint32, vp, vp, vp, vp, vp],
                                                   ctypes.c_int),
        "hipbls_recover_secret_batch_ct_device": ([vp, vp, vp, u64, u64, vp, vp, vp, vp, vp], ctypes.c_int),
        "hipbls_batch_verify_rlc": ([u8p, u8p, u32p, u64, u8p, u64p, u64, u8p, i32p], ctypes.c_int),
        "hipbls_batch_verify_rlc_device": ([vp, vp, vp, u64, vp, vp, u64, u8p, vp, vp], ctypes.c_int),
        "hipbls_rlc_stats": ([u64p, u64p, u64p], ctypes.c_int),
        "hipbls_pubshare_table_load": ([u8p, u64, i32p], ctypes.c_int),
        "hipbls_verify_aggregate_batch": ([u8p, u64p, u64, u8p, u8p, u64p, i32p], ctypes.c_int),
        "hipbls_verify_aggregate_batch_device": ([vp, u64, vp, u64, vp, vp, vp, vp, vp], ctypes.c_int),
        "hipbls_verify_aggregate_batch_keys": ([u32p, u64p, u64, u8p, u8p, u64p, i32p], ctypes.c_int),
        "hipbls_verify_aggregate_batch_keys_device": ([vp, u64, vp, u64, vp, vp, vp, vp, vp], ctypes.c_int),
        "hipbls_pubshare_table_size": ([u64p], ctypes.c_int),
        "hipbls_verify_batch_keys": ([u32p, u8p, u64p, u8p, u64, i32p], ctypes.c_int),
        "hipbls_batch_verify_rlc_keys": ([u32p, u8p, u32p, u64, u8p, u64p, u64, u8p, i32p], ctypes.c_int),
        "hipbls_verify_batch_keys_device": ([vp, vp, vp, vp, u64, vp, vp], ctypes.c_int),
        "hipbls_batch_verify_rlc_keys_device": ([vp, vp, vp, u64, vp, vp, u64, u8p, vp, vp], ctypes.c_int),
        "hipbls_kernel_timing": ([ctypes.c_char_p, ctypes.POINTER(ctypes.c_double), u64p], ctypes.c_int),
        "hipbls_kernel_timing_reset": ([], ctypes.c_int),
        "hipbls_scratch_budget": ([ctypes.c_int, u64p, u64p, u64p, ctypes.POINTER(ctypes.c_uint32)], ctypes.c_int),
        "hipbls_stream_joins": ([u64p], ctypes.c_int),
        "hipbls_kernel_names": ([], ctypes.c_char_p),
        "hipbls_queue_worker_stats": ([u64p, u64p], ctypes.c_int),
        "hipbls_set_latency_replicas": ([ctypes.c_uint32], ctypes.c_int),
        "hipbls_build_id": ([], ctypes.c_char_p),
    }
    for name, (args, res) in sig.items():
        fn = getattr(lib, name)
        fn.argtypes = args
        fn.restype = res
    _lib = lib
    return lib


def exported_symbols() -> List[str]:
    return [
        "hipbls_abi_version", "hipbls_init", "hipbls_device_count", "hipbls_last_error",
        "hipbls_verify_batch", "hipbls_threshold_aggregate_batch", "hipbls_sign_batch",
        "hipbls_secret_to_public_key_batch", "hipbls_verify_aggregate", "hipbls_aggregate",
        "hipbls_threshold_split", "hipbls_recover_secret", "hipbls_verify_batch_device",
        "hipbls_threshold_aggregate_batch_device", "hipbls_sign_batch_device",
        "hipbls_secret_to_public_key_batch_device", "hipbls_kernel_timing", "hipbls_kernel_timing_reset",
        "hipbls_batch_verify_rlc", "hipbls_batch_verify_rlc_device", "hipbls_rlc_stats",
        "hipbls_pubshare_table_load", "hipbls_pubshare_table_size", "hipbls_verify_aggregate_batch",
        "hipbls_verify_aggregate_batch_device", "hipbls_verify_batch_keys",
        "hipbls_batch_verify_rlc_keys", "hipbls_verify_batch_keys_device", "hipbls_batch_verify_rlc_keys_device",
        "hipbls_current_device", "hipbls_set_timing", "hipbls_verify", "hipbls_verify_submit", "hipbls_verify_wait",
        "hipbls_queue_config", "hipbls_queue_stats", "hipbls_verify_signed_data_batch", "hipbls_aggregate_device",
        "hipbls_hcache_config", "hipbls_hcache_stats", "hipbls_set_pair_mode",
        "hipbls_rlc_set_mode", "hipbls_rlc_batch_stats", "hipbls_threshold_aggregate_verify_batch",
        "hipbls_threshold_aggregate_verify_batch_device", "hipbls_init_devices", "hipbls_device_slots",
        "hipbls_plan_ranges", "hipbls_queue_keyed_batches", "hipbls_deserialize_status", "hipbls_device_streams",
        "hipbls_rlc_set_g1_msm_min", "hipbls_scratch_budget", "hipbls_stream_joins", "hipbls_kernel_names",
        "hipbls_queue_worker_stats", "hipbls_set_latency_replicas", "hipbls_build_id",
        "hipbls_threshold_aggregate_verify_batch_keys", "hipbls_threshold_aggregate_verify_batch_keys_device",
        "hipbls_keycache_config", "hipbls_keycache_stats", "hipbls_hcache_prefetch",
        "hipbls_verify_aggregate_batch_keys", "hipbls_verify_aggregate_batch_keys_device",
        "hipbls_rootcache_config", "hipbls_rootcache_stats",
        "hipbls_sign_batch_ct", "hipbls_secret_to_public_key_batch_ct", "hipbls_sign_batch_ct_device",
        "hipbls_secret_to_public_key_batch_ct_device",
        "hipbls_threshold_split_batch_ct", "hipbls_recover_secret_batch_ct",
        "hipbls_threshold_split_batch_ct_device", "hipbls_recover_secret_batch_ct_device",
    ]


def build_id() -> dict:
    raw = load_library().hipbls_build_id().decode()
    return dict(kv.split("=", 1) for kv in raw.split())


def plan_ranges(n: int, parts: int, run_keys: Optional[Sequence[int]] = None) -> List[int]:
    lib = load_library()
    b = (ctypes.c_uint64 * (parts + 1))()
    keys = (ctypes.c_uint32 * max(n, 1))(*run_keys) if run_keys is not None else None
    _check(lib.hipbls_plan_ranges(n, parts, keys, b), lib)
    return list(b)


def _check(rc: int, lib) -> None:
    if rc == OK:
        return
    msg = lib.hipbls_last_error()
    msg = msg.decode() if msg else ""
    if rc == ERR_DEVICE:
        raise DeviceError("hipbls device error: " + msg)
    raise ValueError("hipbls invalid argument (rc=%d) %s" % (rc, msg))


def _offsets(msgs: Sequence[bytes]):
    offs = (ctypes.c_uint64 * (len(msgs) + 1))()
    acc = 0
    for i, m in enumerate(msgs):
        offs[i] = acc
        acc += len(m)
    offs[len(msgs)] = acc
    return b"".join(msgs), offs


def _status_array(n: int):
    return (ctypes.c_int32 * max(n, 1))()


def _go_int(idx) -> int:
    v = int(idx)
    if not -(1 << 63) <= v < (1 << 63):
        raise ValueError("share index outside Go's int range")
    return v


def _check_lengths(name: str, items: Sequence[bytes], size: int) -> None:
    if any(len(x) != size for x in items):
        raise ValueError("%s must be %d bytes each" % (name, size))


class HipBLS:

    def __init__(self, device: Optional[int] = None, devices: Optional[Sequence[int]] = None):
        self.lib = load_library()
        if devices is not None:
            arr = (ctypes.c_int32 * len(devices))(*devices)
            _check(self.lib.hipbls_init_devices(arr, len(devices)), self.lib)
            return
        if device is None:
            device = int(os.environ.get("LOCAL_RANK", "0"))
        _check(self.lib.hipbls_init(device), self.lib)

    def device_slots(self) -> List[int]:
        arr = (ctypes.c_int32 * 64)()
        n = self.lib.hipbls_device_slots(arr, 64)
        return list(arr)[:n]

    def generate_secret_key(self) -> bytes:
        while True:
            v = int.from_bytes(secrets.token_bytes(32), "big") & ((1 << 255) - 1)
            if v < R:
                return v.to_bytes(32, "big")

    def generate_insecure_key(self, random) -> bytes:
        for _ in range(100):
            b = random.read(32)
            if int.from_bytes(b, "big") < R:
                return bytes(b)
        raise TBLSError("cannot generate insecure key")

    def secret_to_public_key(self, secret: bytes) -> bytes:
        pk, st = self.secret_to_public_key_batch_ct([secret])
        if st[0] != OK:
            v = int.from_bytes(secret, "big")
            if v >= R:
                raise TBLSError("cannot unmarshal secret into Herumi secret key")
            raise TBLSError("cannot obtain public key from secret")
        return pk[0]

    def secret_to_public_key_batch(self, secrets_: Sequence[bytes]) -> Tuple[List[bytes], List[int]]:
        n = len(secrets_)
        _check_lengths("secret keys", secrets_, 32)
        out = ctypes.create_string_buffer(48 * max(n, 1))
        st = _status_array(n)
        _check(self.lib.hipbls_secret_to_public_key_batch(b"".join(secrets_), n, out, st), self.lib)
        raw = out.raw
        return [raw[48 * i:48 * i + 48] for i in range(n)], list(st)[:n]

    def secret_to_public_key_batch_ct(self, secrets_: Sequence[bytes]) -> Tuple[List[bytes], List[int]]:
        n = len(secrets_)
        _check_lengths("secret keys", secrets_, 32)
        out = ctypes.create_string_buffer(48 * max(n, 1))
        st = _status_array(n)
        _check(self.lib.hipbls_secret_to_public_key_batch_ct(b"".join(secrets_), n, out, st), self.lib)
        raw = out.raw
        return [raw[48 * i:48 * i + 48] for i in range(n)], list(st)[:n]

    def threshold_split_batch_ct(self, secrets_: Sequence[bytes], tails: Sequence[Sequence[bytes]], total: int,
                                 threshold: int, with_pubs: bool = True):
        n = len(secrets_)
        if len(tails) != n:
            raise ValueError("one polynomial tail per secret")
        _check_lengths("secret keys", secrets_, 32)
        for t in tails:
            if len(t) != max(threshold, 1) - 1:
                raise ValueError("a polynomial tail has threshold - 1 coefficients")
            _check_lengths("polynomial coefficients", t, 32)
        row = total + 1
        out = ctypes.create_string_buffer(32 * max(n * total, 1))
        st = _status_array(n)
        pubs = ctypes.create_string_buffer(48 * max(n * row, 1)) if with_pubs else None
        pst = _status_array(n * row) if with_pubs else None
        _check(self.lib.hipbls_threshold_split_batch_ct(b"".join(secrets_), b"".join(b"".join(t) for t in tails), n,
                                                        total, threshold, out, st, pubs, pst), self.lib)
        raw = out.raw
        shares = [{i + 1: raw[32 * (total * v + i):32 * (total * v + i) + 32] for i in range(total)} for v in range(n)]
        if not with_pubs:
            return shares, list(st)[:n], None, None
        praw, plist = pubs.raw, list(pst)
        return (shares, list(st)[:n],
                [[praw[48 * (row * v + k):48 * (row * v + k) + 48] for k in range(row)] for v in range(n)],
                [plist[row * v:row * v + row] for v in range(n)])

    def recover_secret_batch_ct(self, groups: Sequence[Mapping[int, bytes]], with_pubkeys: bool = True):
        n = len(groups)
        ids, shares, offs = [], [], (ctypes.c_uint64 * (n + 1))()
        for g, grp in enumerate(groups):
            offs[g] = len(ids)
            for i, sh in grp.items():
                ids.append(_go_int(i))
                shares.append(sh)
        offs[n] = len(ids)
        _check_lengths("shares", shares, 32)
        arr = (ctypes.c_int64 * max(len(ids), 1))(*ids)
        out = ctypes.create_string_buffer(32 * max(n, 1))
        st = _status_array(n)
        pks = ctypes.create_string_buffer(48 * max(n, 1)) if with_pubkeys else None
# ... 270 lines not shown

    def verify_aggregate(self, shares: Sequence[bytes], signature: bytes, data: bytes) -> None:
        _check_lengths("public keys", shares, 48)
        _check_lengths("signature", [signature], 96)
        st = _status_array(1)
        _check(self.lib.hipbls_verify_aggregate(b"".join(shares), len(shares), signature, data, len(data), st),
               self.lib)
        if st[0] == ERR_SIGNATURE:
            raise TBLSError("cannot unmarshal signature into Herumi signature")
        if st[0] == ERR_PUBKEY:
            raise TBLSError("cannot set compressed public key in Herumi format")
        if st[0] != OK:
            raise TBLSError("signature verification failed")

    def batch_verify_aggregate_status(self, groups: Sequence[Tuple[Sequence[bytes], bytes, bytes]]) -> List[int]:
        g = len(groups)
        for shares, sig, _ in groups:
            _check_lengths("public keys", shares, 48)
            _check_lengths("signature", [sig], 96)
        koffs = (ctypes.c_uint64 * (g + 1))()
        keys: List[bytes] = []
        for j, (shares, _, _) in enumerate(groups):
            koffs[j] = len(keys)
            keys.extend(bytes(s) for s in shares)
        koffs[g] = len(keys)
        blob, moffs = _offsets([bytes(d) for _, _, d in groups])
        st = _status_array(g)
        _check(self.lib.hipbls_verify_aggregate_batch(b"".join(keys), koffs, g, b"".join(bytes(s) for _, s, _ in groups),
                                                      blob, moffs, st), self.lib)
        return list(st)[:g]

    def batch_verify_aggregate_keys_status(self, groups: Sequence[Tuple[Sequence[int], bytes, bytes]]) -> List[int]:
        g = len(groups)
        for _, sig, _ in groups:
            _check_lengths("signature", [sig], 96)
        koffs = (ctypes.c_uint64 * (g + 1))()
        idx: List[int] = []
        for j, (key_idx, _, _) in enumerate(groups):
            koffs[j] = len(idx)
            idx.extend(int(k) for k in key_idx)
        koffs[g] = len(idx)
        blob, moffs = _offsets([bytes(d) for _, _, d in groups])
        st = _status_array(g)
        arr = (ctypes.c_uint32 * max(len(idx), 1))(*idx)
        _check(self.lib.hipbls_verify_aggregate_batch_keys(arr, koffs, g, b"".join(bytes(s) for _, s, _ in groups),
                                                           blob, moffs, st), self.lib)
        return list(st)[:g]

    def verify_aggregate_keys(self, key_idx: Sequence[int], signature: bytes, data: bytes) -> None:
        st = self.batch_verify_aggregate_keys_status([(key_idx, signature, data)])[0]
        if st == ERR_SIGNATURE:
            raise TBLSError("cannot unmarshal signature into Herumi signature")
        if st == ERR_PUBKEY:
            raise TBLSError("cannot set compressed public key in Herumi format")
        if st != OK:
            raise TBLSError("signature verification failed")

    def aggregate(self, signs: Sequence[bytes]) -> bytes:
        _check_lengths("signatures", signs, 96)
        out = ctypes.create_string_buffer(96)
        st = _status_array(1)
        _check(self.lib.hipbls_aggregate(b"".join(signs), len(signs), out, st), self.lib)
        if st[0] == ERR_SIGNATURE:
            raise TBLSError("cannot unmarshal signature into Herumi signature")
        if st[0] != OK:
            raise DeviceError("unexpected aggregate status %d" % st[0])
        return out.raw

    def deserialize_status(self, points: Sequence[bytes], kind: int) -> List[int]:
        size = 48 if kind == 1 else 96
        _check_lengths("points", points, size)
        st = _status_array(len(points))
        _check(self.lib.hipbls_deserialize_status(b"".join(points), len(points), kind, st), self.lib)
        return list(st)[:len(points)]

    def verify_queued(self, compressed_public_key: bytes, data: bytes, signature: bytes) -> int:
        _check_lengths("public key", [compressed_public_key], 48)
        _check_lengths("signature", [signature], 96)
        st = ctypes.c_int32(-1)
        _check(self.lib.hipbls_verify(compressed_public_key, data, len(data), signature, ctypes.byref(st)), self.lib)
        return st.value

    def verify_submit(self, compressed_public_key: bytes, data: bytes, signature: bytes) -> int:
        _check_lengths("public key", [compressed_public_key], 48)
        _check_lengths("signature", [signature], 96)
        t = ctypes.c_uint64()
        _check(self.lib.hipbls_verify_submit(compressed_public_key, data, len(data), signature, ctypes.byref(t)),
               self.lib)
        return t.value

    def verify_wait(self, ticket: int) -> int:
        st = ctypes.c_int32(-1)
        _check(self.lib.hipbls_verify_wait(ticket, ctypes.byref(st)), self.lib)
        return st.value

    def queue_config(self, max_batch: int = 65536, gather_us: int = 200) -> None:
        _check(self.lib.hipbls_queue_config(max_batch, gather_us), self.lib)

    def queue_keyed_batches(self) -> int:
        b = ctypes.c_uint64()
        _check(self.lib.hipbls_queue_keyed_batches(ctypes.byref(b)), self.lib)
        return b.value

    def queue_stats(self) -> Tuple[int, int]:
        b, i = ctypes.c_uint64(), ctypes.c_uint64()
        _check(self.lib.hipbls_queue_stats(ctypes.byref(b), ctypes.byref(i)), self.lib)
        return b.value, i.value

    def verify_signed_data_status(self, pks: Sequence[bytes], object_roots: Sequence[bytes],
                                  domains: Sequence[bytes], sigs: Sequence[bytes]) -> List[int]:
        n = len(pks)
        if not (len(object_roots) == len(domains) == len(sigs) == n):
            raise ValueError("mismatching lengths")
        _check_lengths("public keys", pks, 48)
        _check_lengths("object roots", object_roots, 32)
        _check_lengths("domains", domains, 32)
        _check_lengths("signatures", sigs, 96)
        st = _status_array(n)
        _check(self.lib.hipbls_verify_signed_data_batch(b"".join(pks), b"".join(object_roots), b"".join(domains),
                                                        b"".join(sigs), n, st), self.lib)
        return list(st)[:n]

    def hcache_config(self, capacity: int) -> None:
        _check(self.lib.hipbls_hcache_config(capacity), self.lib)

    def hcache_stats(self) -> Tuple[int, int, int]:
        a, b, c = ctypes.c_uint64(), ctypes.c_uint64(), ctypes.c_uint64()
        _check(self.lib.hipbls_hcache_stats(ctypes.byref(a), ctypes.byref(b), ctypes.byref(c)), self.lib)
        return a.value, b.value, c.value

    def hcache_prefetch(self, msgs: Sequence[bytes]) -> Tuple[int, int]:
        blob, offs = _offsets(msgs)
        h, p = ctypes.c_uint64(), ctypes.c_uint64()
        _check(self.lib.hipbls_hcache_prefetch(blob, offs, len(msgs), ctypes.byref(h), ctypes.byref(p)), self.lib)
        return h.value, p.value

    def keycache_config(self, slots: int) -> None:
        _check(self.lib.hipbls_keycache_config(slots), self.lib)

    def keycache_stats(self) -> Tuple[int, int, int]:
        a, b, c = ctypes.c_uint64(), ctypes.c_uint64(), ctypes.c_uint64()
        _check(self.lib.hipbls_keycache_stats(ctypes.byref(a), ctypes.byref(b), ctypes.byref(c)), self.lib)
        return a.value, b.value, c.value

    def rootcache_config(self, slots: int) -> None:
        _check(self.lib.hipbls_rootcache_config(slots), self.lib)

    def rootcache_stats(self) -> Tuple[int, int, int, int]:
        a, b, c, d = ctypes.c_uint64(), ctypes.c_uint64(), ctypes.c_uint64(), ctypes.c_uint64()
        _check(self.lib.hipbls_rootcache_stats(ctypes.byref(a), ctypes.byref(b), ctypes.byref(c), ctypes.byref(d)),
               self.lib)
        return a.value, b.value, c.value, d.value

    def set_pair_mode(self, mode: int) -> int:
        rc = self.lib.hipbls_set_pair_mode(mode)
        if rc not in (PAIR_AUTO, PAIR_SINGLE, PAIR_LANES, PAIR_QUADS, PAIR_OCTETS):
            _check(rc, self.lib)
        return rc

    def set_rlc_mode(self, mode: int) -> int:
        rc = self.lib.hipbls_rlc_set_mode(mode)
        if rc not in (RLC_AUTO, RLC_WINDOWS, RLC_BATCH):
            _check(rc, self.lib)
        return rc

    def set_rlc_g1_msm_min(self, min_items: int) -> int:
        if not 0 <= min_items < 1 << 31:
            raise ValueError("min_items out of range")
        return self.lib.hipbls_rlc_set_g1_msm_min(min_items)

    def rlc_batch_stats(self) -> Tuple[int, int, int]:
        a, b, c = ctypes.c_uint64(), ctypes.c_uint64(), ctypes.c_int32()
        _check(self.lib.hipbls_rlc_batch_stats(ctypes.byref(a), ctypes.byref(b), ctypes.byref(c)), self.lib)
        return a.value, b.value, c.value
```

include/hipbls.h:

```cpp
#ifndef HIPBLS_H
#define HIPBLS_H

#include <stddef.h>
#include <stdint.h>

#ifdef __cplusplus
extern "C" {
#endif

enum {
  HIPBLS_OK = 0,
  HIPBLS_ERR_PUBKEY = 1,
  HIPBLS_ERR_SIGNATURE = 2,
  HIPBLS_ERR_VERIFY = 3,
  HIPBLS_ERR_SECRET = 4,
  HIPBLS_ERR_COMBINE = 5,
  HIPBLS_ERR_ZERO_SIG = 6,
  HIPBLS_ERR_ARG = 16,
  HIPBLS_ERR_DEVICE = 17
};

#define HIPBLS_ABI_VERSION 12
int hipbls_abi_version(void);

int hipbls_init_devices(const int32_t* ids, uint32_t n);
int hipbls_init(int device);
int hipbls_device_slots(int32_t* ids, uint32_t cap);
int hipbls_plan_ranges(uint64_t n, uint32_t parts, const uint32_t* run_keys, uint64_t* bounds);
int hipbls_device_count(void);
int hipbls_device_streams(int device);
int hipbls_scratch_budget(int device, uint64_t* per_lane, uint64_t* per_queue, uint64_t* limit, uint32_t* queues);
int hipbls_stream_joins(uint64_t* calls);
const char* hipbls_kernel_names(void);
const char* hipbls_last_error(void);
const char* hipbls_build_id(void);
int hipbls_current_device(void);
int hipbls_set_timing(int enabled);
enum { HIPBLS_PAIR_AUTO = 0, HIPBLS_PAIR_SINGLE = 1, HIPBLS_PAIR_LANES = 2, HIPBLS_PAIR_QUADS = 3,
       HIPBLS_PAIR_OCTETS = 4 };
int hipbls_set_pair_mode(int mode);
int hipbls_set_latency_replicas(uint32_t replicas);

int hipbls_verify(const uint8_t* pk48, const uint8_t* msg, uint64_t msg_len, const uint8_t* sig96, int32_t* status);
int hipbls_verify_submit(const uint8_t* pk48, const uint8_t* msg, uint64_t msg_len, const uint8_t* sig96,
                         uint64_t* ticket);
int hipbls_verify_wait(uint64_t ticket, int32_t* status);
int hipbls_queue_config(uint64_t max_batch, uint32_t gather_us);
int hipbls_queue_stats(uint64_t* batches, uint64_t* items);
int hipbls_queue_keyed_batches(uint64_t* batches);
int hipbls_queue_worker_stats(uint64_t* wakeups, uint64_t* batches);


int hipbls_verify_batch(const uint8_t* pks, const uint8_t* msgs, const uint64_t* msg_offsets,
                        const uint8_t* sigs, uint64_t n, int32_t* status);

int hipbls_verify_signed_data_batch(const uint8_t* pks, const uint8_t* object_roots, const uint8_t* domains,
                                    const uint8_t* sigs, uint64_t n, int32_t* status);

int hipbls_threshold_aggregate_batch(const uint8_t* sigs, const int64_t* share_idx,
                                     const uint64_t* group_offsets, uint64_t n_groups,
                                     uint8_t* out_sigs, int32_t* status);

int hipbls_sign_batch(const uint8_t* sks, const uint8_t* msgs, const uint64_t* msg_offsets, uint64_t n,
                      uint8_t* out_sigs, int32_t* status);

int hipbls_secret_to_public_key_batch(const uint8_t* sks, uint64_t n, uint8_t* out_pks, int32_t* status);

int hipbls_sign_batch_ct(const uint8_t* sks, const uint8_t* msgs, const uint64_t* msg_offsets, uint64_t n,
                         uint8_t* out_sigs, int32_t* status);

int hipbls_secret_to_public_key_batch_ct(const uint8_t* sks, uint64_t n, uint8_t* out_pks, int32_t* status);

int hipbls_verify_aggregate(const uint8_t* pks, uint64_t n, const uint8_t* sig, const uint8_t* msg,
                            uint64_t msg_len, int32_t* status);

int hipbls_verify_aggregate_batch(const uint8_t* pks, const uint64_t* key_offsets, uint64_t n_groups,
                                  const uint8_t* sigs, const uint8_t* msgs, const uint64_t* msg_offsets,
                                  int32_t* status);

int hipbls_verify_aggregate_batch_keys(const uint32_t* key_idx, const uint64_t* key_offsets, uint64_t n_groups,
                                       const uint8_t* sigs, const uint8_t* msgs, const uint64_t* msg_offsets,
                                       int32_t* status);

int hipbls_deserialize_status(const uint8_t* data, uint64_t n, int32_t kind, int32_t* status);

int hipbls_aggregate(const uint8_t* sigs, uint64_t n, uint8_t* out_sig, int32_t* status);

int hipbls_threshold_split(const uint8_t* secret, const uint8_t* poly_tail, uint32_t total, uint32_t threshold,
                           uint8_t* out_shares, int32_t* status);

int hipbls_recover_secret(const uint8_t* shares, const int64_t* ids, uint32_t n, uint8_t* out_secret,
                          int32_t* status);

int hipbls_threshold_split_batch_ct(const uint8_t* secrets, const uint8_t* poly_tails, uint64_t n_val,
                                    uint32_t total, uint32_t threshold, uint8_t* out_shares, int32_t* status,
                                    uint8_t* out_pubs, int32_t* pub_status);

int hipbls_recover_secret_batch_ct(const uint8_t* shares, const int64_t* ids, const uint64_t* group_offsets,
                                   uint64_t n_groups, uint8_t* out_secrets, int32_t* status,
                                   uint8_t* out_pubkeys, int32_t* pk_status);

int hipbls_batch_verify_rlc(const uint8_t* pks, const uint8_t* sigs, const uint32_t* msg_idx, uint64_t n,
                            const uint8_t* msgs, const uint64_t* msg_offsets, uint64_t n_msgs, const uint8_t* seed32,
                            int32_t* status);
int hipbls_pubshare_table_load(const uint8_t* pks, uint64_t n, int32_t* status);
int hipbls_pubshare_table_size(uint64_t* n);
int hipbls_verify_batch_keys(const uint32_t* key_idx, const uint8_t* msgs, const uint64_t* msg_offsets,
                             const uint8_t* sigs, uint64_t n, int32_t* status);
int hipbls_batch_verify_rlc_keys(const uint32_t* key_idx, const uint8_t* sigs, const uint32_t* msg_idx, uint64_t n,
                                 const uint8_t* msgs, const uint64_t* msg_offsets, uint64_t n_msgs,
                                 const uint8_t* seed32, int32_t* status);

int hipbls_rlc_stats(uint64_t* windows, uint64_t* windows_failed, uint64_t* items_fallback);
enum { HIPBLS_RLC_AUTO = 0, HIPBLS_RLC_WINDOWS = 1, HIPBLS_RLC_BATCH = 2 };
int hipbls_rlc_set_mode(int mode);
int hipbls_rlc_set_g1_msm_min(uint32_t min);
int hipbls_rlc_batch_stats(uint64_t* attempted, uint64_t* passed, int32_t* last);

int hipbls_hcache_config(uint64_t capacity);
int hipbls_hcache_stats(uint64_t* hits, uint64_t* misses, uint64_t* entries);
int hipbls_hcache_prefetch(const uint8_t* msgs, const uint64_t* msg_offsets, uint64_t n_msgs, uint64_t* hashed,
                           uint64_t* present);

int hipbls_keycache_config(uint64_t slots);
int hipbls_keycache_stats(uint64_t* hits, uint64_t* misses, uint64_t* inserts);

int hipbls_rootcache_config(uint64_t slots);
int hipbls_rootcache_stats(uint64_t* hits, uint64_t* misses, uint64_t* inserts, uint64_t* rollovers);

int hipbls_verify_batch_device(const uint8_t* d_pks, const uint8_t* d_msgs, const uint64_t* d_msg_offsets,
                               const uint8_t* d_sigs, uint64_t n, int32_t* d_status, void* stream);
int hipbls_threshold_aggregate_verify_batch(const uint8_t* sigs, const int64_t* share_idx,
                                            const uint64_t* group_offsets, uint64_t n_groups, const uint8_t* dv_pks,
                                            const uint8_t* msgs, const uint64_t* msg_offsets, uint8_t* out_sigs,
                                            int32_t* agg_status, int32_t* verify_status);
int hipbls_threshold_aggregate_verify_batch_device(const uint8_t* d_sigs, const int64_t* d_share_idx,
                                                   const uint64_t* d_group_offsets, uint64_t n_groups,
                                                   uint64_t n_parts, const uint8_t* d_dv_pks, const uint8_t* d_msgs,
                                                   const uint64_t* d_msg_offsets, uint8_t* d_out_sigs,
                                                   int32_t* d_agg_status, int32_t* d_verify_status, void* stream);
int hipbls_threshold_aggregate_batch_device(const uint8_t* d_sigs, const int64_t* d_share_idx,
                                            const uint64_t* d_group_offsets, uint64_t n_groups, uint64_t n_parts,
                                            uint8_t* d_out_sigs, int32_t* d_status, void* stream);
int hipbls_threshold_aggregate_verify_batch_keys(const uint8_t* sigs, const int64_t* share_idx,
                                                 const uint64_t* group_offsets, uint64_t n_groups,
                                                 const uint32_t* dv_key_idx, const uint32_t* msg_idx,
                                                 const uint8_t* msgs, const uint64_t* msg_offsets, uint64_t n_msgs,
                                                 uint8_t* out_sigs, int32_t* agg_status, int32_t* verify_status);
int hipbls_threshold_aggregate_verify_batch_keys_device(
    const uint8_t* d_sigs, const int64_t* d_share_idx, const uint64_t* d_group_offsets, uint64_t n_groups,
    uint64_t n_parts, const uint32_t* d_dv_key_idx, const uint32_t* d_msg_idx, const uint8_t* d_msgs,
    const uint64_t* d_msg_offsets, uint64_t n_msgs, uint8_t* d_out_sigs, int32_t* d_agg_status,
    int32_t* d_verify_status, void* stream);
int hipbls_aggregate_device(const uint8_t* d_sigs, uint64_t n, uint8_t* d_out_sig, int32_t* d_status, void* stream);
int hipbls_sign_batch_device(const uint8_t* d_sks, const uint8_t* d_msgs, const uint64_t* d_msg_offsets,
                             uint64_t n, uint8_t* d_out_sigs, int32_t* d_status, void* stream);
int hipbls_secret_to_public_key_batch_device(const uint8_t* d_sks, uint64_t n, uint8_t* d_out_pks,
                                             int32_t* d_status, void* stream);
int hipbls_sign_batch_ct_device(const uint8_t* d_sks, const uint8_t* d_msgs, const uint64_t* d_msg_offsets,
                                uint64_t n, uint8_t* d_out_sigs, int32_t* d_status, void* stream);
int hipbls_secret_to_public_key_batch_ct_device(const uint8_t* d_sks, uint64_t n, uint8_t* d_out_pks,
                                                int32_t* d_status, void* stream);

int hipbls_threshold_split_batch_ct_device(const uint8_t* d_secrets, const uint8_t* d_poly_tails, uint64_t n_val,
                                           uint32_t total, uint32_t threshold, uint8_t* d_out_shares,
                                           int32_t* d_status, uint8_t* d_out_pubs, int32_t* d_pub_status,
                                           void* stream);
int hipbls_recover_secret_batch_ct_device(const uint8_t* d_shares, const int64_t* d_ids,
                                          const uint64_t* d_group_offsets, uint64_t n_groups, uint64_t n_parts,
                                          uint8_t* d_out_secrets, int32_t* d_status, uint8_t* d_out_pubkeys,
                                          int32_t* d_pk_status, void* stream);

int hipbls_batch_verify_rlc_device(const uint8_t* d_pks, const uint8_t* d_sigs, const uint32_t* d_msg_idx, uint64_t n,
                                   const uint8_t* d_msgs, const uint64_t* d_msg_offsets, uint64_t n_msgs,
                                   const uint8_t* seed32, int32_t* d_status, void* stream);

int hipbls_verify_aggregate_batch_device(const uint8_t* d_pks, uint64_t nkeys, const uint64_t* d_key_offsets,
                                         uint64_t n_groups, const uint8_t* d_sigs, const uint8_t* d_msgs,
                                         const uint64_t* d_msg_offsets, int32_t* d_status, void* stream);

int hipbls_verify_aggregate_batch_keys_device(const uint32_t* d_key_idx, uint64_t nkeys, const uint64_t* d_key_offsets,
                                              uint64_t n_groups, const uint8_t* d_sigs, const uint8_t* d_msgs,
                                              const uint64_t* d_msg_offsets, int32_t* d_status, void* stream);

int hipbls_verify_batch_keys_device(const uint32_t* d_key_idx, const uint8_t* d_msgs, const uint64_t* d_msg_offsets,
                                    const uint8_t* d_sigs, uint64_t n, int32_t* d_status, void* stream);
int hipbls_batch_verify_rlc_keys_device(const uint32_t* d_key_idx, const uint8_t* d_sigs, const uint32_t* d_msg_idx,
                                        uint64_t n, const uint8_t* d_msgs, const uint64_t* d_msg_offsets,
                                        uint64_t n_msgs, const uint8_t* seed32, int32_t* d_status, void* stream);

int hipbls_kernel_timing(const char* name, double* avg_ms, uint64_t* launches);
int hipbls_kernel_timing_reset(void);

#ifdef __cplusplus
}
#endif

#endif
```

Measured before the change: 2.709 million.

## Cache Miller-loop line coefficients per signing root and replay them on hits

Adds a device-side line-coefficient pool attached to the root cache. On a root-cache insert, the Miller loop records the G2 line coefficients (which depend only on the hashed message) into a block guarded by a checksum. On later hits, a wave whose lanes all have replay blocks replays the stored lines instead of recomputing the G2 doubling and addition steps. The root lookup partitions items by line availability so waves stay uniform. The cost is extra global memory traffic, a large pool allocation (slots/2 blocks of about 20KB each), checksum hashing, and a separate kernel variant whose register pressure may differ.

```diff
diff --git a/charon_amd/csrc/hipbls.hip b/charon_amd/csrc/hipbls.hip
--- a/charon_amd/csrc/hipbls.hip
+++ b/charon_amd/csrc/hipbls.hip
@@ -167,6 +167,12 @@
   uint64_t gen_base = 0;
   uint64_t rollovers = 0;
   bool partition = true;
+  uint64_t lines_want = kLinesDefault;
+  uint64_t line_blocks = 0;
+  uint32_t* lines = nullptr;
+  unsigned long long* lctr = nullptr;
+  static constexpr uint64_t kLinesDefault = ~0ull;
+  uint64_t lines_target() const { return !slots ? 0 : (lines_want == kLinesDefault ? slots / 2 : lines_want); }
   bls::rootcache dev() const {
     bls::rootcache r{};
     if (slots) {
@@ -174,12 +180,18 @@
       r.claim = claim;
       r.ctr = ctr;
       r.mask = (uint32_t)(slots - 1);
+      if (lines && lctr) {
+        r.lines = lines;
+        r.lctr = lctr;
+        r.blocks = (uint32_t)line_blocks;
+      }
     }
     return r;
   }
 };
 constexpr uint64_t kRootCacheDefaultSlots = 262144;
 constexpr uint64_t kRootCacheMaxSlots = 1ull << 22;
+constexpr uint64_t kRootCacheMaxLines = 1ull << 22;
 
 struct VBatch {
   std::vector<uint8_t> pk, sig, msg;
@@ -378,6 +390,12 @@
   if (!rc.ctr) HIP_TRY(hipMalloc((void**)&rc.ctr, 3 * sizeof(unsigned long long)));
   if (!rc.h_ins) HIP_TRY(hipHostMalloc((void**)&rc.h_ins, sizeof(unsigned long long), hipHostMallocDefault));
   HIP_TRY(hipMemsetAsync(rc.ctr, 0, 3 * sizeof(unsigned long long), s));
+  if (rc.lines && rc.line_blocks != rc.lines_target()) {
+    (void)hipFree(rc.lines);
+    rc.lines = nullptr;
+    rc.line_blocks = 0;
+  }
+  if (rc.lctr) HIP_TRY(hipMemsetAsync(rc.lctr, 0, bls::RL_CTRS * sizeof(unsigned long long), s));
   if (rc.slots) {
     HIP_TRY(hipMemsetAsync(rc.claim, 0, rc.slots * 4, s));
     HIP_TRY(hipMemsetAsync(rc.entries, 0, rc.slots * bls::RC_WORDS * 4, s));
@@ -398,6 +416,45 @@
     return kRootCacheDefaultSlots;
   }
   return (uint64_t)v;
+}
+
+uint64_t rootcache_default_lines() {
+  const char* e = getenv("HIPBLS_ROOTCACHE_LINES");
+  if (!e || !e[0]) return RootCache::kLinesDefault;
+  char* end = nullptr;
+  const unsigned long long v = strtoull(e, &end, 10);
+  if (end == e || *end || v > kRootCacheMaxLines) {
+    fprintf(stderr, "hipbls: HIPBLS_ROOTCACHE_LINES=%s ignored (expected 0 .. 2^22)\n", e);
+    return RootCache::kLinesDefault;
+  }
+  return (uint64_t)v;
+}
+
+void rootcache_lines_ensure(RootCache& rc, hipStream_t s) {
+  const uint64_t want = rc.lines_target();
+  if (!want || rc.lines) return;
+  if (!rc.lctr) {
+    if (hipMalloc((void**)&rc.lctr, bls::RL_CTRS * sizeof(unsigned long long)) != hipSuccess) {
+      (void)hipGetLastError();
+      rc.lctr = nullptr;
+      rc.lines_want = 0;
+      return;
+    }
+    if (hipMemsetAsync(rc.lctr, 0, bls::RL_CTRS * sizeof(unsigned long long), s) != hipSuccess ||
+        hipStreamSynchronize(s) != hipSuccess) {
+      (void)hipGetLastError();
+      rc.lines_want = 0;
+      return;
+    }
+  }
+  if (hipMalloc((void**)&rc.lines, want * bls::RL_BLOCK_WORDS * 4) != hipSuccess) {
+    (void)hipGetLastError();
+    fprintf(stderr, "hipbls: no memory for %llu line blocks of the root cache; lines off\n", (unsigned long long)want);
+    rc.lines = nullptr;
+    rc.lines_want = 0;
+    return;
+  }
+  rc.line_blocks = want;
 }
 
 #define KC_LAUNCH_GUARD(c) std::lock_guard<std::mutex> _kcl((c).kcache.mu)
@@ -449,7 +506,7 @@
     KREF(k_scan_apply), KREF(k_scan_part), KREF(k_scan_top), KREF(k_sign), KREF(k_signing_roots), KREF(k_sk_to_pk),
     KREF(k_tagg_scale), KREF(k_tagg_sum), KREF(k_tagg_sum_s), KREF(k_tagg_unscale),
     KREF(k_tv_check_unscale), KREF(k_tv_join), KREF(k_tv_phase_a), KREF(k_tv_prep_pk), KREF(k_tv_prep_pk2),
-    KREF(k_verify_fused), KREF(k_verify_keys), KREF(k_verify_pair_lg2), KREF(k_verify_pair_lq4),
+    KREF(k_verify_fused), KREF(k_verify_fused_lines), KREF(k_verify_keys), KREF(k_verify_pair_lg2), KREF(k_verify_pair_lq4),
     KREF(k_verify_pair_single), KREF(k_verify_prep), KREF(k_zero_sig_status), KREF8(k_g1m_miller8),
     KREF8(k_rlcb_final8), KREF8(k_rlcb_sfactor8), KREF8(k_verify_pair_lq8), KREF8(k_verify_prep8),
     KREF16(k_verify_pair_lq16), KREF8(k_fav_prep8), KREF16W(k_fav_pair_lq16),
@@ -611,6 +668,7 @@
       if (krc) return krc;
       const char* part = getenv("HIPBLS_ROOTCACHE_PARTITION");
       c->rcache.partition = !(part && part[0] == '0');
+      c->rcache.lines_want = rootcache_default_lines();
       const int rrc = rootcache_setup(c->rcache, rootcache_default_slots(), c->stream);
       if (rrc) return rrc;
     }
@@ -1023,6 +1081,7 @@
   HIP_TRY(hipMemcpyAsync(&ins, R.ctr + 2, sizeof(ins), hipMemcpyDeviceToHost, c.stream));
   HIP_TRY(hipMemsetAsync(R.claim, 0, R.slots * 4, c.stream));
   HIP_TRY(hipMemsetAsync(R.entries, 0, R.slots * bls::RC_WORDS * 4, c.stream));
+  if (R.lctr) HIP_TRY(hipMemsetAsync(R.lctr + bls::RL_CTR_NEXT, 0, sizeof(unsigned long long), c.stream));
   HIP_TRY(hipStreamSynchronize(c.stream));
   *R.h_ins = ins;
   R.gen_base = ins;
@@ -1037,6 +1096,7 @@
   int rc = rootcache_roll_if_due(c, ctx_locked);
   if (rc) return rc;
   std::lock_guard<std::mutex> rg(R.mu);
+  if (n <= 0xffffffffull) rootcache_lines_ensure(R, s);
   const bls::rootcache rcd = n <= 0xffffffffull ? R.dev() : bls::rootcache{};
   uint32_t *perm = nullptr, *pslot = nullptr;
   if (rcd.entries) {
@@ -1054,8 +1114,9 @@
   }
   rc = timed(c, "verify", s, [&] {
     KC_LAUNCH_GUARD(c);
-    hipLaunchKernelGGL(k_verify_fused, dim3((unsigned)grid_for(n)), dim3(kBlock), 0, s, d_pks, d_msgs, d_offs, d_sigs,
-                       n, d_status, c.kcache.dev(), rcd, (const uint32_t*)perm, (const uint32_t*)pslot);
+    hipLaunchKernelGGL(rcd.lines ? k_verify_fused_lines : k_verify_fused, dim3((unsigned)grid_for(n)), dim3(kBlock), 0,
+                       s, d_pks, d_msgs, d_offs, d_sigs, n, d_status, c.kcache.dev(), rcd, (const uint32_t*)perm,
+                       (const uint32_t*)pslot);
   });
   if (rc) return rc;
   if (rcd.entries) HIP_TRY(hipMemcpyAsync(R.h_ins, rcd.ctr + 2, sizeof(unsigned long long), hipMemcpyDeviceToHost, s));
@@ -3907,6 +3968,41 @@
   return HIPBLS_OK;
 }
 
+int hipbls_rootcache_lines_config(uint64_t blocks) {
+  if (blocks != RootCache::kLinesDefault && blocks > kRootCacheMaxLines)
+    return arg_err("root cache line pool above 2^22 blocks");
+  ENSURE_INIT();
+  return run_all([&](Context& c) -> int {
+    std::lock_guard<std::mutex> g(c.rcache.mu);
+    HIP_TRY(hipDeviceSynchronize());
+    c.rcache.lines_want = blocks;
+    return rootcache_setup(c.rcache, c.rcache.slots, c.stream);
+  });
+}
+
+int hipbls_rootcache_lines_stats(uint64_t* line_hits, uint64_t* blocks_published, uint64_t* pool_full,
+                                 uint64_t* check_failures) {
+  if (!line_hits || !blocks_published || !pool_full || !check_failures) return arg_err("null output");
+  *line_hits = *blocks_published = *pool_full = *check_failures = 0;
+  ENSURE_INIT();
+  const int n = nctx();
+  for (int k = 0; k < n; ++k) {
+    Context& c = ctx(k);
+    ENTER_CTX(c);
+    std::lock_guard<std::mutex> g(c.rcache.mu);
+    if (!c.rcache.lctr) continue;
+    unsigned long long v[bls::RL_CTRS] = {};
+    HIP_TRY(hipDeviceSynchronize());
+    HIP_TRY(hipMemcpyAsync(v, c.rcache.lctr, sizeof(v), hipMemcpyDeviceToHost, c.stream));
+    HIP_TRY(hipStreamSynchronize(c.stream));
+    *line_hits += v[bls::RL_CTR_HITS];
+    *blocks_published += v[bls::RL_CTR_PUBLISHED];
+    *pool_full += v[bls::RL_CTR_FULL];
+    *check_failures += v[bls::RL_CTR_BAD];
+  }
+  return HIPBLS_OK;
+}
+
 int hipbls_hcache_stats(uint64_t* hits, uint64_t* misses, uint64_t* entries) {
   if (!hits || !misses || !entries) return arg_err("null output");
   *hits = *misses = *entries = 0;
diff --git a/charon_amd/csrc/kernels.h b/charon_amd/csrc/kernels.h
--- a/charon_amd/csrc/kernels.h
+++ b/charon_amd/csrc/kernels.h
@@ -19,6 +19,26 @@
   __shared__ u32x4 s_f12_[36 * kBlock];      \
   const f12l<kBlock> F { (BLS_LDS u32x4*)&s_f12_[threadIdx.x] }
 
+template <bool LINES>
+__device__ __forceinline__ void verify_fused_lane(const uint8_t* __restrict__ pks, const uint8_t* __restrict__ msgs,
+                                                  const uint64_t* __restrict__ offs, const uint8_t* __restrict__ sigs,
+                                                  uint64_t n, int32_t* __restrict__ status, keycache kc, rootcache rc,
+                                                  const uint32_t* __restrict__ perm,
+                                                  const uint32_t* __restrict__ pslot) {
+  const uint64_t j = blockIdx.x * (uint64_t)blockDim.x + threadIdx.x;
+  if (j >= n) return;
+  const uint64_t i = perm ? perm[j] : j;
+  if (i >= n) return;
+  const uint64_t o0 = offs[i], o1 = offs[i + 1];
+#if BLS_VERIFY_LDS
+  BLS_LANE_F12(F);
+  if (!perm) rc.entries = nullptr;
+  status[i] = op_verify_l_kernel_rc<kBlock, LINES>(pks + 48 * i, msgs + o0, (uint32_t)(o1 - o0), sigs + 96 * i, F, kc,
+                                                   rc, perm ? pslot[j] : RC_NONE);
+#else
+  status[i] = op_verify(pks + 48 * i, msgs + o0, (uint32_t)(o1 - o0), sigs + 96 * i);
+#endif
+}
 __global__ void __launch_bounds__(kBlock) k_verify_fused(const uint8_t* __restrict__ pks,
                                                          const uint8_t* __restrict__ msgs,
                                                          const uint64_t* __restrict__ offs,
@@ -26,19 +46,16 @@
                                                          int32_t* __restrict__ status, keycache kc, rootcache rc,
                                                          const uint32_t* __restrict__ perm,
                                                          const uint32_t* __restrict__ pslot) {
-  const uint64_t j = blockIdx.x * (uint64_t)blockDim.x + threadIdx.x;
-  if (j >= n) return;
-  const uint64_t i = perm ? perm[j] : j;
-  if (i >= n) return;
-  const uint64_t o0 = offs[i], o1 = offs[i + 1];
-#if BLS_VERIFY_LDS
-  BLS_LANE_F12(F);
-  if (!perm) rc.entries = nullptr;
-  status[i] = op_verify_l_kernel_rc(pks + 48 * i, msgs + o0, (uint32_t)(o1 - o0), sigs + 96 * i, F, kc, rc,
-                                    perm ? pslot[j] : RC_NONE);
-#else
-  status[i] = op_verify(pks + 48 * i, msgs + o0, (uint32_t)(o1 - o0), sigs + 96 * i);
-#endif
+  verify_fused_lane<false>(pks, msgs, offs, sigs, n, status, kc, rc, perm, pslot);
+}
+__global__ void __launch_bounds__(kBlock) k_verify_fused_lines(const uint8_t* __restrict__ pks,
+                                                               const uint8_t* __restrict__ msgs,
+                                                               const uint64_t* __restrict__ offs,
+                                                               const uint8_t* __restrict__ sigs, uint64_t n,
+                                                               int32_t* __restrict__ status, keycache kc, rootcache rc,
+                                                               const uint32_t* __restrict__ perm,
+                                                               const uint32_t* __restrict__ pslot) {
+  verify_fused_lane<true>(pks, msgs, offs, sigs, n, status, kc, rc, perm, pslot);
 }
 
 __global__ void __launch_bounds__(kBlock) k_root_lookup(const uint8_t* __restrict__ msgs,
@@ -49,18 +66,19 @@
   if (i >= n) return;
   const uint64_t o0 = offs[i], o1 = offs[i + 1];
   const bool eligible = o1 - o0 == RC_MSG_BYTES;
-  uint32_t slot = RC_NONE;
+  uint32_t slot = RC_NONE, e_lines = 0;
   if (eligible) {
     uint32_t tag[8];
     rc_tag_from_msg(tag, msgs + o0);
-    slot = rc_find(rc, tag);
+    slot = rc_find(rc, tag, &e_lines);
   }
   const bool hit = slot != RC_NONE;
+  const bool front = hit && (!rc.lines || (e_lines != 0 && e_lines - 1 < rc.blocks));
   rc_count(rc, 0, hit);
   rc_count(rc, 1, eligible && !hit);
   uint64_t pos = i;
   if (partition) {
-    const uint64_t act = __ballot(1), mh = __ballot(hit), mr = act & ~mh;
+    const uint64_t act = __ballot(1), mh = __ballot(front), mr = act & ~mh;
     const uint32_t lane = __builtin_amdgcn_mbcnt_hi(~0u, __builtin_amdgcn_mbcnt_lo(~0u, 0u));
     uint32_t bh = 0, br = 0;
     if (lane == (uint32_t)(__ffsll((unsigned long long)act) - 1)) {
@@ -70,7 +88,7 @@
     bh = __builtin_amdgcn_readfirstlane(bh);
     br = __builtin_amdgcn_readfirstlane(br);
     const uint64_t below = ((uint64_t)1 << lane) - 1;
-    pos = hit ? (uint64_t)bh + __popcll(mh & below) : n - 1 - ((uint64_t)br + __popcll(mr & below));
+    pos = front ? (uint64_t)bh + __popcll(mh & below) : n - 1 - ((uint64_t)br + __popcll(mr & below));
   }
   if (pos >= n) return;
   perm[pos] = (uint32_t)i;
diff --git a/charon_amd/csrc/ops.h b/charon_amd/csrc/ops.h
--- a/charon_amd/csrc/ops.h
+++ b/charon_amd/csrc/ops.h
@@ -38,8 +38,9 @@
 #ifndef BLS_VERIFY_L_CALL
 #define BLS_VERIFY_L_CALL BLS_CALL
 #endif
-template <int S, bool INL>
-BLS_HD BLS_INLINE int pairing_check_verify_sig_l_body(const g1a& pk, const g2a& hm, const g2a& sig, const f12l<S> F) {
+template <int S, bool INL, bool LINES = false>
+BLS_HD BLS_INLINE int pairing_check_verify_sig_l_body(const g1a& pk, const g2a& hm, const g2a& sig, const f12l<S> F,
+                                                    const rl_plan* plan = nullptr) {
   g1a P1;
   P1.x = G1_GEN_X;
   P1.y = G1_NEG_GEN_Y;
@@ -47,7 +48,24 @@
   bool in_g2;
   {
     g2j T1;
-    if (INL)
+    if (LINES) {
+      bool done = false;
+      if (rl_wave_all(plan->replay != nullptr)) {
+        done = miller_loop_2_l_replay<S>(f, F, pk, sig, &T1, plan->replay, plan->seed);
+        rl_count(plan->lctr, RL_CTR_HITS, done);
+        rl_count(plan->lctr, RL_CTR_BAD, !done);
+      }
+      if (!done && rl_wave_any(plan->record != nullptr)) {
+        rl_recorder rec{plan->record, plan->seed};
+        miller_loop_2_l_body<S, true>(f, F, pk, hm, P1, sig, &T1, rec);
+        if (plan->record) {
+          rl_publish(*plan, rec.h);
+          rl_count(plan->lctr, RL_CTR_PUBLISHED, true);
+        }
+      } else if (!done) {
+        miller_loop_2_l_body<S, true>(f, F, pk, hm, P1, sig, &T1);
+      }
+    } else if (INL)
       miller_loop_2_l_body<S, true>(f, F, pk, hm, P1, sig, &T1);
     else
       miller_loop_2_l<S, true>(f, F, pk, hm, P1, sig, &T1);
diff --git a/charon_amd/csrc/pairing.h b/charon_amd/csrc/pairing.h
--- a/charon_amd/csrc/pairing.h
+++ b/charon_amd/csrc/pairing.h
@@ -11,7 +11,20 @@
 
 
 
-BLS_HD BLS_INLINE void miller_dbl_step_inl(g2j& T_in, fp2& g0, fp2& g1, fp2& h1, const fp& xp_in, const fp& yp_in) {
+#if defined(__HIPCC__)
+#define BLS_MEMBER __forceinline__
+#else
+#define BLS_MEMBER inline
+#endif
+
+struct line_sink_none {
+  BLS_HD BLS_MEMBER void put(int, const fp2&) const {}
+  BLS_HD BLS_MEMBER void next() const {}
+};
+
+template <class SINK = line_sink_none>
+BLS_HD BLS_INLINE void miller_dbl_step_inl(g2j& T_in, fp2& g0, fp2& g1, fp2& h1, const fp& xp_in, const fp& yp_in,
+                                         SINK&& sink = SINK()) {
   const fp xp = xp_in;
   const fp yp = yp_in;
   g2j T = T_in;
@@ -21,6 +34,7 @@
     fp2 J3;
     fp2_add(J3, t, t);
     fp2_add(J3, J3, t);
+    sink.put(1, J3);
     fp2_mul_fp(g1, J3, xp);
   }
   fp2_mul(A, T.x, T.y);
@@ -32,7 +46,9 @@
   fp2_sqr(B, T.y);
   fp2_sub(H, H, B);
   fp2_sub(H, H, C);
+  sink.put(2, H);
   fp2_sub(g0, E, B);
+  sink.put(0, g0);
   fp2_mul_fp(h1, H, yp);
   fp2_neg(h1, h1);
   fp2_mul(T.z, B, H);
@@ -53,19 +69,23 @@
 }
 BLS_HD BLS_MILLER_CALL void miller_dbl_step(g2j& T_in, fp2& g0, fp2& g1, fp2& h1, const fp& xp_in, const fp& yp_in) { miller_dbl_step_inl(T_in, g0, g1, h1, xp_in, yp_in); }
 
+template <class SINK = line_sink_none>
 BLS_HD BLS_INLINE void miller_add_step_inl(g2j& T_in, fp2& g0, fp2& g1, fp2& h1, const g2a& Q_in, const fp& xp_in,
-                                         const fp& yp_in) {
+                                         const fp& yp_in, SINK&& sink = SINK()) {
   const fp xp = xp_in;
   const fp yp = yp_in;
   g2j T = T_in;
   fp2 theta, lambda, t, u;
   fp2_mul(t, Q_in.y, T.z);
   fp2_sub(theta, T.y, t);
+  sink.put(1, theta);
   fp2_mul(t, Q_in.x, T.z);
   fp2_sub(lambda, T.x, t);
+  sink.put(2, lambda);
   fp2_mul(t, theta, Q_in.x);
   fp2_mul(u, lambda, Q_in.y);
   fp2_sub(g0, t, u);
+  sink.put(0, g0);
   fp2_mul_fp(g1, theta, xp);
   fp2_neg(g1, g1);
   fp2_mul_fp(h1, lambda, yp);
diff --git a/charon_amd/csrc/pairing_lds.h b/charon_amd/csrc/pairing_lds.h
--- a/charon_amd/csrc/pairing_lds.h
+++ b/charon_amd/csrc/pairing_lds.h
@@ -1,5 +1,6 @@
 #pragma once
 #include "pairing.h"
+#include "rootcache.h"
 
 namespace bls {
 
@@ -10,12 +11,6 @@
 #endif
 
 typedef uint32_t u32x4 __attribute__((vector_size(16)));
-
-#if defined(__HIPCC__)
-#define BLS_MEMBER __forceinline__
-#else
-#define BLS_MEMBER inline
-#endif
 
 template <int S>
 struct f12l {
@@ -343,9 +338,22 @@
 #ifndef BLS_MILLER_L_CALL
 #define BLS_MILLER_L_CALL BLS_CALL
 #endif
-template <int S, bool P1_NEG_GEN = false>
+struct rl_recorder {
+  uint32_t* p;
+  uint64_t h;
+  BLS_HD BLS_MEMBER void put(int k, const fp2& v) {
+    if (!p) return;
+    rl_store_words(p + 24 * k, &v.c0.v[0], 24);
+    h = rl_fold(h, &v.c0.v[0], 24);
+  }
+  BLS_HD BLS_MEMBER void next() {
+    if (p) p += RL_LINE_WORDS;
+  }
+};
+
+template <int S, bool P1_NEG_GEN = false, class SINK = line_sink_none>
 BLS_HD BLS_INLINE void miller_loop_2_l_body(fp12& f_out, const f12l<S> F, const g1a& P0_in, const g2a& Q0,
-                                          const g1a& P1_in, const g2a& Q1, g2j* T1_out) {
+                                          const g1a& P1_in, const g2a& Q1, g2j* T1_out, SINK&& sink = SINK()) {
   g1a P0 = P0_in;
   g1a P1;
   if (P1_NEG_GEN) {
@@ -364,11 +372,13 @@
   {
     fp12 f;
     fp2 a0, a1, ah, g0, g1, h1;
-    miller_dbl_step_inl(T0, a0, a1, ah, P0.x, P0.y);
+    miller_dbl_step_inl(T0, a0, a1, ah, P0.x, P0.y, sink);
+    sink.next();
     miller_dbl_step_inl(T1, g0, g1, h1, P1.x, P1.y);
     fp12_line_pair(f, a0, a1, ah, g0, g1, h1);
     F.st12(f);
-    miller_add_step_inl(T0, a0, a1, ah, Q0, P0.x, P0.y);
+    miller_add_step_inl(T0, a0, a1, ah, Q0, P0.x, P0.y, sink);
+    sink.next();
     miller_add_step_inl(T1, g0, g1, h1, Q1, P1.x, P1.y);
     fp12_mul_line2_l(F, a0, a1, ah, g0, g1, h1);
   }
@@ -382,7 +392,8 @@
 #endif
     fp12_sqr_l(F);
     fp2 a0, a1, ah, g0, g1, h1;
-    BLS_ML_DBL(T0, a0, a1, ah, P0.x, P0.y);
+    BLS_ML_DBL(T0, a0, a1, ah, P0.x, P0.y, sink);
+    sink.next();
 #if BLS_ML_PARK & 2
     park_agpr(T0);
     park_agpr(a0);
@@ -392,7 +403,8 @@
     BLS_ML_DBL(T1, g0, g1, h1, P1.x, P1.y);
     fp12_mul_line2_l(F, a0, a1, ah, g0, g1, h1);
     if ((X_ABS >> bit) & 1ull) {
-      miller_add_step_inl(T0, a0, a1, ah, Q0, P0.x, P0.y);
+      miller_add_step_inl(T0, a0, a1, ah, Q0, P0.x, P0.y, sink);
+      sink.next();
       miller_add_step_inl(T1, g0, g1, h1, Q1, P1.x, P1.y);
       fp12_mul_line2_l(F, a0, a1, ah, g0, g1, h1);
     }
@@ -401,6 +413,94 @@
   F.ld12(f);
   fp12_conj(f_out, f);
   if (T1_out) *T1_out = T1;
+}
+
+BLS_HD BLS_INLINE void rl_line_dbl(fp2& a0, fp2& a1, fp2& ah, const uint32_t w[RL_LINE_WORDS], const g1a& P0) {
+  fp2 J3, H;
+  for (int k = 0; k < 12; ++k) {
+    a0.c0.v[k] = w[k], a0.c1.v[k] = w[12 + k];
+    J3.c0.v[k] = w[24 + k], J3.c1.v[k] = w[36 + k];
+    H.c0.v[k] = w[48 + k], H.c1.v[k] = w[60 + k];
+  }
+  fp2_mul_fp(a1, J3, P0.x);
+  fp2_mul_fp(ah, H, P0.y);
+  fp2_neg(ah, ah);
+}
+BLS_HD BLS_INLINE void rl_line_add(fp2& a0, fp2& a1, fp2& ah, const uint32_t w[RL_LINE_WORDS], const g1a& P0) {
+  fp2 theta, lambda;
+  for (int k = 0; k < 12; ++k) {
+    a0.c0.v[k] = w[k], a0.c1.v[k] = w[12 + k];
+    theta.c0.v[k] = w[24 + k], theta.c1.v[k] = w[36 + k];
+    lambda.c0.v[k] = w[48 + k], lambda.c1.v[k] = w[60 + k];
+  }
+  fp2_mul_fp(a1, theta, P0.x);
+  fp2_neg(a1, a1);
+  fp2_mul_fp(ah, lambda, P0.y);
+}
+
+template <int S>
+BLS_HD BLS_INLINE bool miller_loop_2_l_replay(fp12& f_out, const f12l<S> F, const g1a& P0_in, const g2a& Q1,
+                                            g2j* T1_out, const uint32_t* blk, uint64_t seed) {
+  g1a P0 = P0_in;
+  g1a P1;
+  P1.x = G1_GEN_X;
+  P1.y = G1_NEG_GEN_Y;
+  g2j T1;
+  T1.x = Q1.x;
+  T1.y = Q1.y;
+  fp2_set_one(T1.z);
+  uint64_t h = seed;
+  const uint32_t* p = blk;
+  uint32_t chk[4];
+  rl_load_check(chk, blk);
+  {
+    fp12 f;
+    fp2 a0, a1, ah, g0, g1, h1;
+    uint32_t w[RL_LINE_WORDS];
+    miller_dbl_step_inl(T1, g0, g1, h1, P1.x, P1.y);
+    rl_load_line(w, p);
+    p += RL_LINE_WORDS;
+    h = rl_fold_line(h, w);
+    rl_line_dbl(a0, a1, ah, w, P0);
+    fp12_line_pair(f, a0, a1, ah, g0, g1, h1);
+    F.st12(f);
+    miller_add_step_inl(T1, g0, g1, h1, Q1, P1.x, P1.y);
+    rl_load_line(w, p);
+    p += RL_LINE_WORDS;
+    h = rl_fold_line(h, w);
+    rl_line_add(a0, a1, ah, w, P0);
+    fp12_mul_line2_l(F, a0, a1, ah, g0, g1, h1);
+  }
+  for (int bit = 61; bit >= 0; --bit) {
+#if BLS_ML_PARK & 1
+    park_agpr(T1);
+#endif
+#if BLS_ML_PARK & 4
+    park_agpr(P0);
+#endif
+    fp12_sqr_l(F);
+    fp2 a0, a1, ah, g0, g1, h1;
+    uint32_t w[RL_LINE_WORDS];
+    BLS_ML_DBL(T1, g0, g1, h1, P1.x, P1.y);
+    rl_load_line(w, p);
+    p += RL_LINE_WORDS;
+    h = rl_fold_line(h, w);
+    rl_line_dbl(a0, a1, ah, w, P0);
+    fp12_mul_line2_l(F, a0, a1, ah, g0, g1, h1);
+    if ((X_ABS >> bit) & 1ull) {
+      miller_add_step_inl(T1, g0, g1, h1, Q1, P1.x, P1.y);
+      rl_load_line(w, p);
+      p += RL_LINE_WORDS;
+      h = rl_fold_line(h, w);
+      rl_line_add(a0, a1, ah, w, P0);
+      fp12_mul_line2_l(F, a0, a1, ah, g0, g1, h1);
+    }
+  }
+  fp12 f;
+  F.ld12(f);
+  fp12_conj(f_out, f);
+  if (T1_out) *T1_out = T1;
+  return rl_check_ok(h, chk[0], chk[1]);
 }
 template <int S, bool P1_NEG_GEN = false>
 BLS_HD BLS_MILLER_L_CALL void miller_loop_2_l(fp12& f_out, const f12l<S> F, const g1a& P0_in, const g2a& Q0, const g1a& P1_in,
diff --git a/charon_amd/csrc/rlc.h b/charon_amd/csrc/rlc.h
--- a/charon_amd/csrc/rlc.h
+++ b/charon_amd/csrc/rlc.h
@@ -245,22 +245,34 @@
   return RLC_PENDING;
 }
 
-BLS_HD BLS_CALL void verify_hm_rc(g2a& hm, const uint8_t* msg, uint32_t msg_len, const rootcache& rc, uint32_t slot) {
+BLS_HD BLS_CALL void verify_hm_rc(g2a& hm, const uint8_t* msg, uint32_t msg_len, const rootcache& rc, uint32_t slot,
+                                  rl_plan* plan = nullptr) {
   const bool eligible = rc.entries && msg_len == RC_MSG_BYTES;
   uint32_t tag[8];
   if (eligible) rc_tag_from_msg(tag, msg);
-  bool ins = false;
-  if (!(eligible && slot != RC_NONE && rc_get_slot(rc, slot, tag, &hm.x.c0.v[0]))) {
+  bool ins = false, full = false;
+  uint32_t e_lines = 0;
+  if (eligible && slot != RC_NONE && rc_get_slot(rc, slot, tag, &hm.x.c0.v[0], &e_lines)) {
+    if (plan) rl_plan_hit(*plan, rc, e_lines, rc_tag_hash(tag));
+  } else {
     g2j hj;
     hash_to_g2(hj, msg, msg_len, DST_POP, 43);
     const bool inf = jac_is_inf(hj);
     jac_to_aff(hm, hj);
-    if (eligible && !inf) ins = rc_insert(rc, tag, &hm.x.c0.v[0]);
+    if (eligible && !inf) {
+      const uint32_t s = rc_insert_slot(rc, tag, &hm.x.c0.v[0]);
+      ins = s != RC_NONE;
+      if (ins && plan && rc.lines) {
+        rl_plan_insert(*plan, rc, s, rc_tag_hash(tag));
+        full = !plan->record;
+      }
+    }
   }
   if (rc.entries) rc_count(rc, 2, ins);
-}
-
-template <int S>
+  if (rc.entries && rc.lines && plan) rl_count(rc.lctr, RL_CTR_FULL, full);
+}
+
+template <int S, bool LINES = true>
 BLS_HD BLS_INLINE int op_verify_l_kernel_rc(const uint8_t* pk48, const uint8_t* msg, uint32_t msg_len,
                                             const uint8_t* sig96, const f12l<S> F, const keycache& kc,
                                             const rootcache& rc, uint32_t slot) {
@@ -272,8 +284,13 @@
   if (ds == DEC_BAD) return HIPBLS_ERR_SIGNATURE;
   if (dp == DEC_INF || ds == DEC_INF) return verify_inf_status(ds, sig);
   g2a hm;
-  verify_hm_rc(hm, msg, msg_len, rc, slot);
-  return pairing_check_verify_sig_l_body<S, true>(pk, hm, sig, F);
+  if (!LINES) {
+    verify_hm_rc(hm, msg, msg_len, rc, slot);
+    return pairing_check_verify_sig_l_body<S, true>(pk, hm, sig, F);
+  }
+  rl_plan plan{};
+  verify_hm_rc(hm, msg, msg_len, rc, slot, &plan);
+  return pairing_check_verify_sig_l_body<S, true, true>(pk, hm, sig, F, &plan);
 }
 
 template <int S>
diff --git a/charon_amd/csrc/rootcache.h b/charon_amd/csrc/rootcache.h
--- a/charon_amd/csrc/rootcache.h
+++ b/charon_amd/csrc/rootcache.h
@@ -4,7 +4,7 @@
 namespace bls {
 
 constexpr int RC_WORDS = 64;
-constexpr int RC_TAG = 0, RC_H = 8, RC_CHK = 56, RC_USED = 60;
+constexpr int RC_TAG = 0, RC_H = 8, RC_CHK = 56, RC_LINES = 58, RC_USED = 60;
 constexpr uint32_t RC_MSG_BYTES = 32;
 constexpr uint32_t RC_NONE = 0xffffffffu;
 
@@ -13,7 +13,9 @@
   uint32_t* claim;
   unsigned long long* ctr;
   uint32_t mask;
-  uint32_t pad_;
+  uint32_t blocks;
+  uint32_t* lines;
+  unsigned long long* lctr;
 };
 
 KC_HD void rc_tag_from_msg(uint32_t tag[8], const uint8_t* m32) {
@@ -54,7 +56,7 @@
   return (home + (uint32_t)(j % KC_WINDOW)) & mask;
 }
 
-KC_HD uint32_t rc_find(const rootcache& rc, const uint32_t tag[8]) {
+KC_HD uint32_t rc_find(const rootcache& rc, const uint32_t tag[8], uint32_t* e_lines = nullptr) {
   const uint64_t th = rc_tag_hash(tag);
   const uint32_t fpr = kc_fingerprint(th);
   for (int j = 0; j < RC_SEQ; ++j) {
@@ -64,32 +66,41 @@
     if (c != fpr) continue;
     uint32_t e[RC_WORDS];
     kc_load_words(e, rc.entries + (uint64_t)s * RC_WORDS, 0, RC_USED);
-    if (rc_entry_get(e, tag, nullptr)) return s;
+    if (rc_entry_get(e, tag, nullptr)) {
+      if (e_lines) *e_lines = e[RC_LINES];
+      return s;
+    }
   }
   return RC_NONE;
 }
 
-KC_HD bool rc_get_slot(const rootcache& rc, uint32_t slot, const uint32_t tag[8], uint32_t h[48]) {
+KC_HD bool rc_get_slot(const rootcache& rc, uint32_t slot, const uint32_t tag[8], uint32_t h[48],
+                       uint32_t* e_lines = nullptr) {
   uint32_t e[RC_WORDS];
   kc_load_words(e, rc.entries + (uint64_t)(slot & rc.mask) * RC_WORDS, 0, RC_USED);
+  if (e_lines) *e_lines = e[RC_LINES];
   return rc_entry_get(e, tag, h);
 }
 
-KC_HD bool rc_insert(const rootcache& rc, const uint32_t tag[8], const uint32_t h[48]) {
+KC_HD uint32_t rc_insert_slot(const rootcache& rc, const uint32_t tag[8], const uint32_t h[48]) {
   const uint64_t th = rc_tag_hash(tag);
   const uint32_t fpr = kc_fingerprint(th);
   for (int j = 0; j < RC_SEQ; ++j) {
     const uint32_t s = rc_seq_slot(th, j, rc.mask);
     uint32_t c = kc_load_claim(rc.claim + s);
     if (!c) c = kc_cas_claim(rc.claim + s, fpr);
-    if (c == fpr) return false;
+    if (c == fpr) return RC_NONE;
     if (c) continue;
     uint32_t e[RC_WORDS];
     rc_pack(e, tag, h);
     kc_store_entry(rc.entries + (uint64_t)s * RC_WORDS, e);
-    return true;
+    return s;
   }
-  return false;
+  return RC_NONE;
+}
+
+KC_HD bool rc_insert(const rootcache& rc, const uint32_t tag[8], const uint32_t h[48]) {
+  return rc_insert_slot(rc, tag, h) != RC_NONE;
 }
 
 #if defined(__HIP_DEVICE_COMPILE__)
@@ -107,4 +118,109 @@
 }
 #endif
 
-}
+constexpr int RL_LINES = 68;
+constexpr int RL_LINE_WORDS = 72;
+constexpr int RL_CHK = RL_LINES * RL_LINE_WORDS;
+constexpr int RL_BLOCK_WORDS = 4928;
+static_assert(RL_CHK % 4 == 0 && RL_CHK + 4 <= RL_BLOCK_WORDS && RL_BLOCK_WORDS % 64 == 0, "line block layout");
+enum { RL_CTR_NEXT = 0, RL_CTR_HITS, RL_CTR_PUBLISHED, RL_CTR_FULL, RL_CTR_BAD, RL_CTRS };
+
+struct rl_plan {
+  const uint32_t* replay;
+  uint32_t* record;
+  uint32_t* entry_word;
+  uint32_t index1;
+  uint64_t seed;
+  unsigned long long* lctr;
+};
+
+KC_HD uint64_t rl_seed(uint64_t tag_hash) { return tag_hash ^ 0xC0AC29B7C97C50DDull; }
+KC_HD uint64_t rl_mix2(uint64_t h, uint32_t lo, uint32_t hi) {
+  h = (h ^ (((uint64_t)hi << 32) | lo)) * 0x9E3779B97F4A7C15ull;
+  return h ^ (h >> 29);
+}
+KC_HD uint64_t rl_fold(uint64_t h, const uint32_t* w, int n) {
+  for (int i = 0; i < n; i += 2) h = rl_mix2(h, w[i], w[i + 1]);
+  return h;
+}
+KC_HD uint64_t rl_fold_line(uint64_t h, const uint32_t w[RL_LINE_WORDS]) {
+  return rl_fold(rl_fold(h, w + 24, 48), w, 24);
+}
+KC_HD bool rl_check_ok(uint64_t h, uint32_t c0, uint32_t c1) {
+  const uint64_t c = kc_check_final(h);
+  return c0 == (uint32_t)c && c1 == (uint32_t)(c >> 32);
+}
+KC_HD bool rl_block_ok(const uint32_t* b, uint64_t seed) {
+  uint64_t h = seed;
+  for (int l = 0; l < RL_LINES; ++l) h = rl_fold_line(h, b + l * RL_LINE_WORDS);
+  return rl_check_ok(h, b[RL_CHK], b[RL_CHK + 1]);
+}
+
+#if defined(__HIP_DEVICE_COMPILE__)
+KC_HD void rl_load_line(uint32_t w[RL_LINE_WORDS], const uint32_t* src) { kc_load_words(w, src, 0, RL_LINE_WORDS); }
+KC_HD void rl_load_check(uint32_t c[4], const uint32_t* blk) { kc_load_words(c, blk + RL_CHK, 0, 4); }
+KC_HD void rl_store_words(uint32_t* dst, const uint32_t* v, int n) {
+  kc_gu128* d = (kc_gu128*)__builtin_assume_aligned(dst, 16);
+  for (int k = 0; k < n / 4; ++k) d[k] = make_uint4(v[4 * k], v[4 * k + 1], v[4 * k + 2], v[4 * k + 3]);
+}
+KC_HD void rl_store_word(uint32_t* dst, uint32_t v) { *(kc_gu32*)dst = v; }
+KC_HD unsigned long long rl_take_block(const rootcache& rc) {
+  return __hip_atomic_fetch_add((kc_gu64*)rc.lctr + RL_CTR_NEXT, 1ull, __ATOMIC_RELAXED, __HIP_MEMORY_SCOPE_AGENT);
+}
+KC_HD void rl_count(unsigned long long* lctr, int which, bool flag) {
+  const uint64_t act = __ballot(1), m = __ballot(flag);
+  if (!m) return;
+  const uint32_t lane = __builtin_amdgcn_mbcnt_hi(~0u, __builtin_amdgcn_mbcnt_lo(~0u, 0u));
+  if (lane != (uint32_t)(__ffsll((unsigned long long)act) - 1)) return;
+  __hip_atomic_fetch_add((kc_gu64*)lctr + which, (unsigned long long)__popcll(m), __ATOMIC_RELAXED,
+                         __HIP_MEMORY_SCOPE_AGENT);
+}
+#else
+KC_HD void rl_load_line(uint32_t w[RL_LINE_WORDS], const uint32_t* src) {
+  for (int k = 0; k < RL_LINE_WORDS; ++k) w[k] = src[k];
+}
+KC_HD void rl_load_check(uint32_t c[4], const uint32_t* blk) {
+  for (int k = 0; k < 4; ++k) c[k] = blk[RL_CHK + k];
+}
+KC_HD void rl_store_words(uint32_t* dst, const uint32_t* v, int n) {
+  for (int k = 0; k < n; ++k) dst[k] = v[k];
+}
+KC_HD void rl_store_word(uint32_t* dst, uint32_t v) { *dst = v; }
+KC_HD unsigned long long rl_take_block(const rootcache& rc) { return rc.lctr[RL_CTR_NEXT]++; }
+KC_HD void rl_count(unsigned long long* lctr, int which, bool flag) {
+  if (flag) lctr[which] += 1;
+}
+#endif
+
+#if defined(__HIP_DEVICE_COMPILE__)
+KC_HD bool rl_wave_all(bool flag) { return __ballot(flag) == __ballot(1); }
+KC_HD bool rl_wave_any(bool flag) { return __ballot(flag) != 0; }
+#else
+KC_HD bool rl_wave_all(bool flag) { return flag; }
+KC_HD bool rl_wave_any(bool flag) { return flag; }
+#endif
+
+KC_HD void rl_plan_hit(rl_plan& plan, const rootcache& rc, uint32_t e_lines, uint64_t tag_hash) {
+  if (!rc.lines || e_lines == 0 || e_lines - 1 >= rc.blocks) return;
+  plan.replay = rc.lines + (uint64_t)(e_lines - 1) * RL_BLOCK_WORDS;
+  plan.seed = rl_seed(tag_hash);
+  plan.lctr = rc.lctr;
+}
+KC_HD void rl_plan_insert(rl_plan& plan, const rootcache& rc, uint32_t slot, uint64_t tag_hash) {
+  if (!rc.lines) return;
+  const unsigned long long b = rl_take_block(rc);
+  if (b >= rc.blocks) return;
+  plan.record = rc.lines + b * RL_BLOCK_WORDS;
+  plan.entry_word = rc.entries + (uint64_t)(slot & rc.mask) * RC_WORDS + RC_LINES;
+  plan.index1 = (uint32_t)b + 1;
+  plan.seed = rl_seed(tag_hash);
+  plan.lctr = rc.lctr;
+}
+KC_HD void rl_publish(const rl_plan& plan, uint64_t h) {
+  const uint64_t c = kc_check_final(h);
+  const uint32_t tail[4] = {(uint32_t)c, (uint32_t)(c >> 32), 0, 0};
+  rl_store_words(plan.record + RL_CHK, tail, 4);
+  rl_store_word(plan.entry_word, plan.index1);
+}
+
+}
diff --git a/charon_amd/tbls.py b/charon_amd/tbls.py
--- a/charon_amd/tbls.py
+++ b/charon_amd/tbls.py
@@ -81,6 +81,8 @@
         "hipbls_keycache_stats": ([u64p, u64p, u64p], ctypes.c_int),
         "hipbls_rootcache_config": ([u64], ctypes.c_int),
         "hipbls_rootcache_stats": ([u64p, u64p, u64p, u64p], ctypes.c_int),
+        "hipbls_rootcache_lines_config": ([u64], ctypes.c_int),
+        "hipbls_rootcache_lines_stats": ([u64p, u64p, u64p, u64p], ctypes.c_int),
         "hipbls_abi_version": ([], ctypes.c_int),
         "hipbls_init": ([ctypes.c_int], ctypes.c_int),
         "hipbls_device_count": ([], ctypes.c_int),
@@ -162,6 +164,7 @@
         "hipbls_keycache_config", "hipbls_keycache_stats", "hipbls_hcache_prefetch",
         "hipbls_verify_aggregate_batch_keys", "hipbls_verify_aggregate_batch_keys_device",
         "hipbls_rootcache_config", "hipbls_rootcache_stats",
+        "hipbls_rootcache_lines_config", "hipbls_rootcache_lines_stats",
         "hipbls_sign_batch_ct", "hipbls_secret_to_public_key_batch_ct", "hipbls_sign_batch_ct_device",
         "hipbls_secret_to_public_key_batch_ct_device",
         "hipbls_threshold_split_batch_ct", "hipbls_recover_secret_batch_ct",
@@ -738,6 +741,15 @@
                self.lib)
         return a.value, b.value, c.value, d.value
 
+    def rootcache_lines_config(self, blocks: Optional[int] = None) -> None:
+        _check(self.lib.hipbls_rootcache_lines_config(2 ** 64 - 1 if blocks is None else blocks), self.lib)
+
+    def rootcache_lines_stats(self) -> Tuple[int, int, int, int]:
+        a, b, c, d = ctypes.c_uint64(), ctypes.c_uint64(), ctypes.c_uint64(), ctypes.c_uint64()
+        _check(self.lib.hipbls_rootcache_lines_stats(ctypes.byref(a), ctypes.byref(b), ctypes.byref(c),
+                                                     ctypes.byref(d)), self.lib)
+        return a.value, b.value, c.value, d.value
+
     def set_pair_mode(self, mode: int) -> int:
         rc = self.lib.hipbls_set_pair_mode(mode)
         if rc not in (PAIR_AUTO, PAIR_SINGLE, PAIR_LANES, PAIR_QUADS, PAIR_OCTETS):
diff --git a/include/hipbls.h b/include/hipbls.h
--- a/include/hipbls.h
+++ b/include/hipbls.h
@@ -127,6 +127,10 @@
 
 int hipbls_rootcache_config(uint64_t slots);
 int hipbls_rootcache_stats(uint64_t* hits, uint64_t* misses, uint64_t* inserts, uint64_t* rollovers);
+
+int hipbls_rootcache_lines_config(uint64_t blocks);
+int hipbls_rootcache_lines_stats(uint64_t* line_hits, uint64_t* blocks_published, uint64_t* pool_full,
+                                 uint64_t* check_failures);
 
 int hipbls_verify_batch_device(const uint8_t* d_pks, const uint8_t* d_msgs, const uint64_t* d_msg_offsets,
                                const uint8_t* d_sigs, uint64_t n, int32_t* d_status, void* stream);
```

Measured after the change: 2.892 million (median of 6 runs). 1.07x the previous value.
